# MPF-Optimization-Laboratory/ConicIP.jl

Measured on AMD Instinct MI355X. Metric: KKT solves/sec + wall-clock to converge, dense QP n=8192, 1 GPU, higher is better.
Workload: dtype f64

## Files before the change

conicip.jl_amd/cipkkt/_lib.py:

```python
import ctypes as C
import os

_HERE = os.path.dirname(os.path.abspath(__file__))
LIB_PATH = os.environ.get("CIPKKT_LIB", os.path.join(_HERE, "libcipkkt.so"))

CONE_R, CONE_Q, CONE_S = 0, 1, 2
ROUTE_SCHUR, ROUTE_FULL3X3 = 0, 1
OP_F, OP_FT, OP_FINV, OP_FINVT = 0, 1, 2, 3
MAT_Q, MAT_A, MAT_G = 0, 1, 2
FLAG_DEVICE_PTRS = 1
FLAG_CSR_HOST = 2
FLAG_Q_CSR = 4
E_SINGULAR = -5
E_UNSUPPORTED = -6
E_RETRY = -7

c_double_p = C.POINTER(C.c_double)
c_int_p = C.POINTER(C.c_int)


class CipProblem(C.Structure):
    _fields_ = [("n", C.c_int), ("m", C.c_int), ("p", C.c_int), ("ncones", C.c_int),
                ("cone_type", c_int_p), ("cone_dim", c_int_p),
                ("Q", C.c_void_p), ("ldq", C.c_int),
# ... 24 lines not shown
                             C.c_void_p, C.c_int, C.POINTER(C.c_void_p)]),
    "cip_create_ex": (C.c_int, [C.POINTER(CipProblem), C.POINTER(C.c_void_p)]),
    "cip_update_problem": (C.c_int, [C.c_void_p, C.POINTER(CipProblem)]),
    "cip_destroy": (C.c_int, [C.c_void_p]),
    "cip_last_error": (C.c_char_p, []),
    "cip_set_stream": (C.c_int, [C.c_void_p, C.c_void_p]),
    "cip_scaling_packed_len": (C.c_size_t, [C.c_void_p]),
    "cip_set_scaling_packed": (C.c_int, [C.c_void_p, C.c_void_p]),
    "cip_set_scaling_identity": (C.c_int, [C.c_void_p]),
    "cip_set_scaling_from_iterate_dev": (C.c_int, [C.c_void_p, C.c_void_p, C.c_void_p, C.c_void_p]),
    "cip_get_scaling_packed": (C.c_int, [C.c_void_p, C.c_void_p]),
    "cip_factor": (C.c_int, [C.c_void_p]),
    "cip_check_factor": (C.c_int, [C.c_void_p]),
    "cip_set_regularization": (C.c_int, [C.c_void_p, C.c_double, C.c_int]),
    "cip_get_regularization": (C.c_int, [C.c_void_p, c_double_p, c_int_p]),
    "cip_solve3x3": (C.c_int, [C.c_void_p] + [C.c_void_p] * 6),
    "cip_solve3x3_dev": (C.c_int, [C.c_void_p] + [C.c_void_p] * 6),
    "cip_solve2x2": (C.c_int, [C.c_void_p] + [C.c_void_p] * 4),
    "cip_solve2x2_dev": (C.c_int, [C.c_void_p] + [C.c_void_p] * 4),
    "cip_solve3x3_many": (C.c_int, [C.c_void_p, C.c_int] + [C.c_void_p] * 6),
    "cip_solve3x3_many_dev": (C.c_int, [C.c_void_p, C.c_int] + [C.c_void_p] * 6),
    "cip_solve2x2_many": (C.c_int, [C.c_void_p, C.c_int] + [C.c_void_p] * 4),
    "cip_solve2x2_many_dev": (C.c_int, [C.c_void_p, C.c_int] + [C.c_void_p] * 4),
    "cip_solve4x4_dev": (C.c_int, [C.c_void_p, C.c_void_p, C.c_void_p, C.c_void_p]),
    "cip_apply_F_dev": (C.c_int, [C.c_void_p, C.c_int, C.c_void_p, C.c_void_p]),
    "cip_cone_prod_dev": (C.c_int, [C.c_void_p, C.c_void_p, C.c_void_p, C.c_void_p]),
    "cip_cone_div_dev": (C.c_int, [C.c_void_p, C.c_void_p, C.c_void_p, C.c_void_p]),
    "cip_maxstep_dev": (C.c_int, [C.c_void_p, C.c_void_p, C.c_void_p, C.c_double, c_double_p]),
    "cip_maxstep_pair_dev": (C.c_int, [C.c_void_p, C.c_void_p, C.c_void_p, C.c_void_p, C.c_void_p, C.c_double, c_double_p]),
    "cip_cone_identity_dev": (C.c_int, [C.c_void_p, C.c_void_p]),
    "cip_gemv_dev": (C.c_int, [C.c_void_p, C.c_int, C.c_int, C.c_double, C.c_void_p, C.c_double, C.c_void_p]),
    "cip_dots_dev": (C.c_int, [C.c_void_p, C.c_int, C.POINTER(C.c_void_p), C.POINTER(C.c_void_p), c_int_p,
                               c_double_p]),
    "cip_axpby_dev": (C.c_int, [C.c_void_p, C.c_int, C.c_double, C.c_void_p, C.c_double, C.c_void_p]),
    "cip_conicip": (C.c_int, [C.c_void_p, C.c_void_p, C.c_void_p, C.c_void_p, C.POINTER(CipOptions), C.c_void_p,
                              C.c_void_p, C.c_void_p, C.POINTER(CipResult), C.c_void_p, C.c_int]),
    "cip_batch_create": (C.c_int, [C.c_int, C.POINTER(CipProblem), C.POINTER(C.c_void_p)]),
    "cip_batch_destroy": (C.c_int, [C.c_void_p]),
    "cip_batch_size": (C.c_int, [C.c_void_p]),
    "cip_batch_handle": (C.c_void_p, [C.c_void_p, C.c_int]),
    "cip_batch_conicip": (C.c_int, [C.c_void_p] + [C.POINTER(C.c_void_p)] * 3 + [C.POINTER(CipOptions)] +
                          [C.POINTER(C.c_void_p)] * 3 + [C.POINTER(CipResult), C.c_int]),
    "cip_conicip_problems": (C.c_int, [C.c_int, C.POINTER(CipProblem)] + [C.POINTER(C.c_void_p)] * 3 +
                             [C.POINTER(CipOptions)] + [C.POINTER(C.c_void_p)] * 3 + [C.POINTER(CipResult), C.c_int]),
    "cip_conicip_lockstep": (C.c_int, [C.c_int, C.POINTER(CipProblem)] + [C.POINTER(C.c_void_p)] * 3 +
                             [C.POINTER(CipOptions)] + [C.POINTER(C.c_void_p)] * 3 + [C.POINTER(CipResult)]),
    "cip_conicip_mixed": (C.c_int, [C.c_int, C.POINTER(CipProblem)] + [C.POINTER(C.c_void_p)] * 3 +
                          [C.POINTER(CipOptions)] + [C.POINTER(C.c_void_p)] * 3 + [C.POINTER(CipResult), C.c_int]),
    "cip_release_cached_memory": (C.c_int, []),
    "cip_lockstep_stats": (C.c_int, [c_int_p]),
    "cip_set_lockstep_regularize": (C.c_int, [C.c_int]),
    "cip_set_lockstep_ragged": (C.c_int, [C.c_int]),
    "cip_lockstep_regularized": (C.c_int, [c_int_p]),
    "cip_conicip_many": (C.c_int, [C.POINTER(C.c_void_p), C.c_int] + [C.POINTER(C.c_void_p)] * 3 +
                         [C.POINTER(CipOptions)] + [C.POINTER(C.c_void_p)] * 3 + [C.POINTER(CipResult), C.c_int]),
    "cip_ldlt_workspace_bytes": (C.c_int, [C.c_int, C.POINTER(C.c_size_t)]),
    "cip_ldlt_factor_dev": (C.c_int, [C.c_void_p, C.c_void_p, C.c_int, C.c_int, C.c_void_p, c_int_p]),
    "cip_ldlt_solve_dev": (C.c_int, [C.c_void_p, C.c_void_p, C.c_int, C.c_int, C.c_void_p, C.c_void_p]),
    "cip_ldlt_solve_many_scratch_bytes": (C.c_int, [C.c_int, C.c_int, C.POINTER(C.c_size_t)]),
    "cip_ldlt_solve_many_dev": (C.c_int, [C.c_void_p, C.c_void_p, C.c_int, C.c_int, C.c_void_p, C.c_void_p, C.c_void_p, C.c_int,
                                          C.c_int]),
    "cip_gemm_nt_dev": (C.c_int, [C.c_void_p, C.c_int, C.c_int, C.c_int, C.c_double, C.c_void_p, C.c_int,
                                  C.c_void_p, C.c_int, C.c_void_p, C.c_int, C.c_int]),
    "cip_qrcp_workspace_bytes": (C.c_int, [C.c_int, C.c_int, C.POINTER(C.c_size_t)]),
    "cip_imcols_workspace_bytes": (C.c_int, [C.c_int, C.c_int, C.POINTER(C.c_size_t)]),
    "cip_qrcp_dev": (C.c_int, [C.c_void_p, C.c_void_p, C.c_int, C.c_int, C.c_int, C.c_double, C.c_void_p, C.c_void_p, c_int_p,
                               c_double_p, c_int_p]),
    "cip_imcols_dev": (C.c_int, [C.c_void_p, C.c_void_p, C.c_int, C.c_int, C.c_int, C.c_void_p, C.c_double, C.c_void_p, c_int_p,
                                 c_int_p, c_int_p, c_double_p]),
    "cip_kkt_order": (C.c_int, [C.c_void_p, c_int_p, c_int_p]),
    "cip_get_kkt_matrix": (C.c_int, [C.c_void_p, C.c_void_p]),
    "cip_assemble_only": (C.c_int, [C.c_void_p]),
    "cip_stats": (C.c_int, [C.c_void_p, c_double_p]),
    "cip_set_timing": (C.c_int, [C.c_void_p, C.c_int]),
    "cip_set_ldlt_outer_block": (C.c_int, [C.c_int]),
    "cip_set_solve_block_max": (C.c_int, [C.c_int]),
    "cip_set_solve_fused": (C.c_int, [C.c_int]),
    "cip_lockstep_solve_block_for": (C.c_int, [C.c_int]),
    "cip_profile_trailing_thread": (C.c_int, [C.c_int]),
    "cip_profile_thread_get": (C.c_int, [c_double_p]),
    "cip_profile_kernel_thread": (C.c_int, [C.c_int, C.c_int]),
    "cip_profile_kernel_thread_get": (C.c_int, [C.c_int, c_double_p]),
    "cip_set_lazy_copy": (C.c_int, [C.c_int]),
    "cip_set_sdp_lanczos": (C.c_int, [C.c_int]),
    "cip_set_lockstep_split": (C.c_int, [C.c_int]),
    "cip_debug_chain_giveup": (C.c_int, [C.c_int]),
    "cip_get_chain_fallbacks": (C.c_int, [C.c_void_p]),
    "cip_sdp_lanczos_fallbacks": (C.c_int, [C.c_void_p, c_int_p]),
    "cip_set_ldlt_fused_chain": (C.c_int, [C.c_int]),
    "cip_set_ldlt_side_prep": (C.c_int, [C.c_int]),
    "cip_profile_trailing": (C.c_int, [C.c_void_p, C.c_int]),
    "cip_profile_get": (C.c_int, [C.c_void_p, c_double_p]),
}

_lib = None


class CipError(RuntimeError):
    def __init__(self, code, msg):
        super().__init__("libcipkkt error %d: %s" % (code, msg))
        self.code = code


def load():
    global _lib
    if _lib is not None:
        return _lib
    if not os.path.exists(LIB_PATH):
        raise ImportError("libcipkkt.so not built (%s): run `python -c 'import __graft_entry__ as g; g.build()'` "
                          "-- there is no CPU fallback" % LIB_PATH)
    lib = C.CDLL(LIB_PATH)
    for name, (res, args) in SIGNATURES.items():
        fn = getattr(lib, name)
        fn.restype = res
        fn.argtypes = args
    _lib = lib
    return lib


def check(rc):
    if rc != 0:
        msg = load().cip_last_error()
        raise CipError(rc, msg.decode() if msg else "?")
```

conicip.jl_amd/csrc/api.hip:

```cpp
#include "cip_handle.h"
#include <thread>
#include <stdlib.h>
#include "../../include/cipkkt.h"
#include <stdarg.h>
#include <stdio.h>
#include <string.h>
#include <math.h>
#include <new>

static thread_local char g_err[512] = "";
void cip_set_error(const char *fmt, ...) {
    va_list ap;
    va_start(ap, fmt);
    vsnprintf(g_err, sizeof(g_err), fmt, ap);
    va_end(ap);
}
extern "C" const char *cip_last_error(void) { return g_err; }

int cip_env_int(const char *name, int dflt) { const char *e = getenv(name); return e ? atoi(e) : dflt; }
long cip_env_long(const char *name, long dflt) { const char *e = getenv(name); return e ? atol(e) : dflt; }
double cip_env_double(const char *name, double dflt) { const char *e = getenv(name); return e ? atof(e) : dflt; }
bool cip_env_set(const char *name) { return getenv(name) != nullptr; }

#include <dlfcn.h>
// ... 556 lines not shown
    return 0;
}

extern "C" int cip_set_stream(cip_handle *h, void *stream) {
    if (!h) return CIP_E_INVALID;
    CIP_HIP_CHECK(hipStreamSynchronize(h->stream));
    h->stream = (hipStream_t)stream;
    h->graph_state = 0;
    return 0;
}

extern "C" size_t cip_scaling_packed_len(const cip_handle *h) { return h ? h->cs.scal_len : 0; }

extern "C" int cip_set_scaling_packed(cip_handle *h, const double *packedF) {
    if (!h || !packedF) { cip_set_error("NULL argument"); return CIP_E_INVALID; }
    CIP_HIP_CHECK(hipMemcpyAsync(h->cs.d_scal, packedF, sizeof(double) * h->cs.scal_len, hipMemcpyHostToDevice, h->stream));
    CIP_HIP_CHECK(hipStreamSynchronize(h->stream));
    h->assembled = h->factored = false;
    return cip_sdp_scaling_changed(h->stream, h->cs);
}
extern "C" int cip_get_scaling_packed(cip_handle *h, double *packedF) {
    if (!h || !packedF) { cip_set_error("NULL argument"); return CIP_E_INVALID; }
    CIP_HIP_CHECK(hipMemcpyAsync(packedF, h->cs.d_scal, sizeof(double) * h->cs.scal_len, hipMemcpyDeviceToHost, h->stream));
    CIP_HIP_CHECK(hipStreamSynchronize(h->stream));
    return 0;
}
extern "C" int cip_set_scaling_identity(cip_handle *h) {
    if (!h) return CIP_E_INVALID;
    h->assembled = h->factored = false;
    CIP_TRY(cip_cones_identity_scaling(h->stream, h->cs));
    return cip_sdp_scaling_changed(h->stream, h->cs);
}
extern "C" int cip_set_scaling_from_iterate_dev(cip_handle *h, const double *v, const double *s, double *lambda_out) {
    if (!h || (h->m > 0 && (!v || !s))) { cip_set_error("NULL argument"); return CIP_E_INVALID; }
    h->assembled = h->factored = false;
    CipRange rg("cip:scaling");
    return cip_cones_nt_scaling(h->stream, h->cs, v, s, lambda_out);
}

extern "C" int cip_assemble_only(cip_handle *h) {
    if (!h) return CIP_E_INVALID;
    return cip_assemble(h);
}

bool cip_graph_wanted(cip_handle *h) {
    if (h->graph_state == 0) {
        const int npmax = cip_env_int("CIP_GRAPH_NMAX", 4096);
        h->graph_state = (h->Npad <= npmax && cip_env_int("CIP_GRAPH", 0) == 1 && !h->timing && !h->ws.prof) ? 1 : -1;
    }
    return h->graph_state == 1;
}
thread_local CipGraphBuilder *cip_tl_builder = nullptr;

__global__ void k_publish_info(const int *info, int *host, int seq) {
    if (threadIdx.x == 0) {
        host[0] = info[0]; host[1] = info[1]; host[2] = info[2]; host[3] = info[3];
        __hip_atomic_store(host + 4, seq, __ATOMIC_RELEASE, __HIP_MEMORY_SCOPE_SYSTEM);
    }
}
static int info_landed(cip_handle *h, bool wait, bool *landed) {
    volatile int *seqp = h->info_host + 4;
    *landed = __atomic_load_n(seqp, __ATOMIC_ACQUIRE) == h->info_seq;
    if (*landed || !wait) return 0;
    for (long spin = 0;; ++spin) {
        if (__atomic_load_n(seqp, __ATOMIC_ACQUIRE) == h->info_seq) { *landed = true; return 0; }
        if ((spin & 0xfff) == 0xfff) {
            std::this_thread::yield();
            const hipError_t q = hipStreamQuery(h->stream);
            if (q == hipSuccess) {
                *landed = __atomic_load_n(seqp, __ATOMIC_ACQUIRE) == h->info_seq;
                if (*landed) return 0;
                cip_set_error("LDL': the pivot flags of factorisation %d never arrived", h->info_seq);
                return CIP_E_HIP;
            }
            if (q != hipErrorNotReady) { cip_set_error("hipStreamQuery failed: %s", hipGetErrorString(q)); return CIP_E_HIP; }
        }
    }
}
static int factor_enqueue(cip_handle *h) {
    { CipRange rg("cip:assemble"); CIP_TRY(cip_assemble(h, true)); }
    if (h->timing) CIP_HIP_CHECK(hipEventRecord(h->ev1, h->stream));
    {
        CipRange rg("cip:ldlt");
        if (h->gx_factor && (h->gx_factor_lazyC != h->ws.lazyC || h->gx_factor_unfused != h->ws.unfused)) {
            (void)hipGraphExecDestroy(h->gx_factor); h->gx_factor = nullptr;
        }
        h->gx_factor_lazyC = h->ws.lazyC;
        h->gx_factor_unfused = h->ws.unfused;
        bool replayed = false;
        CIP_TRY(graph_run(h, &h->gx_factor, [&]() {
            const int r = cip_ldlt_factor(h->stream, h->K, h->Npad, h->ldk, h->ws);
            if (cip_tl_builder) h->gx_factor_fused = cip_ldlt_last_factor_fused();
            return r;
        }, &replayed));
        if (replayed) CIP_TRY(cip_ldlt_debug_giveup(h->stream, h->K, h->Npad, h->ldk, h->ws, h->gx_factor_fused));
    }
    h->n_factor += 1;
    if (!h->info_host) {
        CIP_HIP_CHECK(hipHostMalloc((void **)&h->info_host, 8 * sizeof(int), hipHostMallocMapped | hipHostMallocCoherent));
        memset(h->info_host, 0, 8 * sizeof(int));
    }
    {
        int *info_dev = nullptr;
        CIP_HIP_CHECK(hipHostGetDevicePointer((void **)&info_dev, h->info_host, 0));
        h->info_seq = (h->info_seq == 0x7fffffff) ? 1 : h->info_seq + 1;
        hipLaunchKernelGGL(k_publish_info, dim3(1), dim3(64), 0, h->stream, (const int *)h->ws.info, info_dev, h->info_seq);
        CIP_HIP_CHECK(hipGetLastError());
    }
    h->info_pending = true;
    h->spec_solves = 0;
    h->factored = true;
    return 0;
}

static int refactor_and_wait(cip_handle *h) {
    for (;;) {
        CIP_TRY(factor_enqueue(h));
        { bool landed = false; CIP_TRY(info_landed(h, true, &landed)); }
        h->info_pending = false;
        if (h->info_host[3] == 0 || h->info_host[1] != 0 || h->ws.unfused) return 0;
        h->ws.unfused = 1;
        h->n_chain_fallbacks += 1;
    }
}
static int chain_gave_up(cip_handle *h) {
    if (h->info_host[3] == 0 && h->info_host[1] == 0) return 0;
    cip_set_error("LDL': in-launch wait of the panel chain gave up (%d)", h->info_host[3]);
    h->factored = false;
    return CIP_E_HIP;
}
static int solves_to_repeat(int spec, const char *why) {
    if (spec <= 0) return 0;
    cip_set_error("LDL': %d solve(s) were enqueued on a factorisation %s -- repeat them", spec, why);
    return CIP_E_RETRY;
}
int cip_factor_resolve(cip_handle *h, bool wait) {
    if (!h->info_pending) return 0;
    bool landed = false;
    CIP_TRY(info_landed(h, wait, &landed));
    if (!landed) return 0;
    h->info_pending = false;
    const int spec = h->spec_solves;
    bool redone = false;
    if (h->info_host[3] != 0 && h->info_host[1] == 0 && !h->ws.unfused) {
        h->ws.unfused = 1;
        h->n_chain_fallbacks += 1;
        CIP_TRY(refactor_and_wait(h));
        redone = true;
    }
    CIP_TRY(chain_gave_up(h));
    int info = h->info_host[0];
    if (info == 0 || (h->reg_rel > 0.0 && h->info_host[2] == 0)) {
        h->pivots_verified = true;
        return redone ? solves_to_repeat(spec, "whose panel chain gave up an in-launch wait; the handle has switched to the three-launch chain") : 0;
    }
    if (h->reg_rel > 0.0) {
        info = h->info_host[2];
    } else if (h->auto_reg) {
        h->reg_rel = cip_env_double("CIP_AUTO_REG", CIP_AUTO_REG);
        h->n_regularized += 1;
        CIP_TRY(refactor_and_wait(h));
        CIP_TRY(chain_gave_up(h));
        if (h->info_host[2] == 0) {
            h->pivots_verified = true;
            return solves_to_repeat(spec, "that met a bad pivot; the handle has switched to the regularised factorisation");
        }
        info = h->info_host[2];
    }
    h->factored = false;
    h->pivots_verified = false;
// ... 132 lines not shown
    return cip_ldlt_solve((hipStream_t)stream, K, N, ld, ws, rhs);
}
extern "C" int cip_ldlt_solve_many_scratch_bytes(int N, int nrhs, size_t *bytes) {
    if (N <= 0 || N % CIP_NB || nrhs < 0 || !bytes) { cip_set_error("N must be a positive multiple of 128, nrhs >= 0"); return CIP_E_INVALID; }
    *bytes = sizeof(double) * (size_t)cip_ldlt_solve_many_scratch_block(N) * (size_t)(nrhs < 64 ? nrhs : 64);
    return 0;
}
extern "C" int cip_ldlt_solve_many_dev(void *stream, const double *K, int N, int ld, const void *workspace, void *scratch, double *B,
                                       int ldb, int nrhs) {
    if (!ldlt_dims_ok(K, N, ld, workspace) || nrhs < 0 || ldb < N) {
        cip_set_error("cip_ldlt_solve_many_dev: bad argument (K, workspace non-NULL; N > 0 and ld >= N multiples of 128; nrhs >= 0; "
                      "ldb >= N)");
        return CIP_E_INVALID;
    }
    if (nrhs == 0) return 0;
    if (!B || !scratch) { cip_set_error("cip_ldlt_solve_many_dev: B and scratch must be non-NULL"); return CIP_E_INVALID; }
    LdltWorkspace ws{};
    cip_ldlt_ws_carve((void *)workspace, N, &ws, cip_ldlt_fused_for(N));
    return cip_ldlt_solve_many((hipStream_t)stream, K, N, ld, ws, (double *)scratch, B, ldb, nrhs, true);
}
extern "C" int cip_gemm_nt_dev(void *stream, int M, int N, int K, double alpha, const double *A, int lda, const double *B,
                               int ldb, double *C, int ldc, int lower_only) {
    if (!A || !B || !C || M <= 0 || N <= 0 || K <= 0 || M % CIP_NB || N % CIP_NB || K % 16 || lda < M || ldb < N || ldc < M ||
        (lower_only && M != N)) {
        cip_set_error("cip_gemm_nt_dev: bad argument (A, B, C non-NULL; M, N > 0 multiples of 128, K > 0 a multiple of 16, "
                      "lda >= M, ldb >= N, ldc >= M; M == N with lower_only)");
        return CIP_E_INVALID;
    }
    if (lower_only) return cip_gemm_lower((hipStream_t)stream, M, K, alpha, A, lda, B, ldb, C, ldc);
    return cip_gemm_rect((hipStream_t)stream, M, N, K, alpha, A, lda, B, ldb, C, ldc);
}

extern "C" int cip_kkt_order(const cip_handle *h, int *N, int *N_padded) {
    if (!h) return CIP_E_INVALID;
    if (N) *N = h->N;
    if (N_padded) *N_padded = h->Npad;
    return 0;
}
extern "C" int cip_get_kkt_matrix(cip_handle *h, double *K_host) {
    if (!h || !K_host) return CIP_E_INVALID;
    CIP_TRY(cip_ldlt_side_join(h->stream, h->ws, -1));
    CIP_HIP_CHECK(hipStreamSynchronize(h->stream));
    CIP_HIP_CHECK(hipMemcpy(K_host, h->K, sizeof(double) * (size_t)h->ldk * h->Npad, hipMemcpyDeviceToHost));
    return 0;
}
extern "C" int cip_stats(cip_handle *h, double *out8) {
    if (!h || !out8) return CIP_E_INVALID;
    out8[0] = h->n_factor; out8[1] = h->n_solve; out8[2] = h->ms_assemble; out8[3] = h->ms_ldlt; out8[4] = h->flops_ldlt;
    out8[5] = cip_ldlt_outer_block_for(h->Npad); out8[6] = h->N; out8[7] = h->Npad;
    return 0;
}
extern "C" int cip_set_timing(cip_handle *h, int enabled) {
    if (!h) return CIP_E_INVALID;
    h->timing = enabled != 0;
    return 0;
}
extern "C" int cip_profile_trailing(cip_handle *h, int enabled) {
    if (!h) return CIP_E_INVALID;
    if (enabled && !h->ws.prof) h->ws.prof = cip_ldlt_profile_create();
    if (enabled) cip_ldlt_profile_stride(h->ws.prof, enabled);
    if (!enabled && h->ws.prof) { cip_ldlt_profile_destroy(h->ws.prof); h->ws.prof = nullptr; }
    return 0;
}
extern "C" int cip_profile_get(cip_handle *h, double *out3) {
    if (!h || !out3 || !h->ws.prof) { cip_set_error("profiling not enabled"); return CIP_E_INVALID; }
    return cip_ldlt_profile_collect(h->ws.prof, &out3[0], &out3[1], &out3[2]);
}
extern "C" int cip_profile_kernel_thread(int slot, int enabled) {
    if (cip_prof_slot_enable(slot, enabled)) { cip_set_error("cip_profile_kernel_thread: no slot %d", slot); return CIP_E_INVALID; }
    return 0;
}
extern "C" int cip_profile_kernel_thread_get(int slot, double *out3) {
    if (!out3) return CIP_E_INVALID;
    if (cip_prof_slot_collect(slot, &out3[0], &out3[1], &out3[2])) { cip_set_error("slot %d: profiling not enabled", slot); return CIP_E_INVALID; }
    return 0;
}
extern "C" int cip_profile_trailing_thread(int enabled) { return cip_ldlt_profile_thread(enabled); }
extern "C" int cip_profile_thread_get(double *out3) {
    if (!out3) return CIP_E_INVALID;
    if (cip_ldlt_profile_thread_collect(&out3[0], &out3[1], &out3[2])) { cip_set_error("thread profiling not enabled"); return CIP_E_INVALID; }
    return 0;
}
extern "C" int cip_set_lazy_copy(int on) { return cip_lazy_copy_set(on); }
extern "C" int cip_set_sdp_lanczos(int on) { return cip_sdp_large_lanczos(on); }
extern "C" int cip_debug_chain_giveup(int n) { return cip_debug_chain_giveup_set(n); }
extern "C" int cip_get_chain_fallbacks(cip_handle *h) { return h ? h->n_chain_fallbacks : -1; }
extern "C" int cip_sdp_lanczos_fallbacks(cip_handle *h, int *count) {
    if (!h || !count) { cip_set_error("bad argument"); return CIP_E_INVALID; }
    int out2[2] = {0, 0};
    const int rc = cip_sdp_large_cert_stats(h->stream, h->cs.lg, out2);
    *count = out2[0];
    return rc;
}
extern "C" int cip_set_ldlt_fused_chain(int on) { return cip_ldlt_set_fused_chain(on); }
extern "C" int cip_set_ldlt_side_prep(int on) { return cip_ldlt_set_side_prep(on); }
extern "C" int cip_set_solve_block_max(int b) { return cip_solve_block_max_set(b); }
extern "C" int cip_set_solve_fused(int mode) { return cip_solve_fused_set(mode); }
extern "C" int cip_set_ldlt_outer_block(int nbo) { cip_ldlt_set_outer_block(nbo); return cip_ldlt_outer_block(); }
```

conicip.jl_amd/csrc/assemble.hip:

```cpp
#include "cip_handle.h"
#include <atomic>
#include "../../include/cipkkt.h"

__global__ __launch_bounds__(256) void k_fill_rest(double *K, long ldk, int n, int p, int Npad, const double *G, long ldg, CipBatch cb) {
    CIP_BATCH_GUARD(cb);
    CIP_BO2(cb, K, G);
    const int j = blockIdx.x * 256 + threadIdx.x;
    if (j >= Npad) return;
    for (int i = n + blockIdx.y; i < Npad; i += gridDim.y) {
        if (j > i) continue;
        double v;
        if (i < n + p) v = (j < n) ? G[(i - n) + (long)j * ldg] : 0.0;
        else v = (i == j) ? 1.0 : 0.0;
        K[i + (long)j * ldk] = v;
    }
}

__global__ __launch_bounds__(256) void k_copy_block(double *K, long ldk, int r0, int c0, const double *M, long ldm,
                                                     int rows, int cols, double sign, CipBatch cb) {
    CIP_BATCH_GUARD(cb);
    CIP_BO2(cb, K, M);
    const int i = blockIdx.x * 256 + threadIdx.x;
    if (i >= rows) return;
    for (int j = blockIdx.y; j < cols; j += gridDim.y)
// ... 38 lines not shown
        cip_launch_b(k_copy_block_lower, dim3((n + 255) / 256, n < 32768 ? n : 32768), dim3(256), 0, s, K, ldk, r0, M, ldm, n, sign);
    }
}

__global__ __launch_bounds__(256) void k_qcsr_fill_cols(double *K, long ldk, int n, const int *rp, const int *ci, const double *v, int vec,
                                                         CipBatch cb) {
    CIP_BATCH_GUARD(cb);
    CIP_BO4(cb, K, rp, ci, v);
    const int j = blockIdx.x, tid = threadIdx.x;
    if (j >= n) return;
    double *col = K + (long)j * ldk;
    const int z0 = j & ~127;
    if (vec) {
        const int nv = (n - z0) >> 1;
        for (int t = tid; t < nv; t += 256) *(v2d *)(col + z0 + 2 * t) = (v2d){0.0, 0.0};
        if (((n - z0) & 1) && tid == 0) col[n - 1] = 0.0;
    } else {
        for (int i = z0 + tid; i < n; i += 256) col[i] = 0.0;
    }
    __syncthreads();
    const int q1 = rp[j + 1];
    for (int q = rp[j] + tid; q < q1; q += 256) {
        const int i = ci[q];
        if ((i >> 7) >= (j >> 7)) col[i] = v[q];
    }
}
template <bool ADD>
__global__ __launch_bounds__(256) void k_qcsr_scatter(double *K, long ldk, int r0, int n, const int *rp, const int *ci, const double *v,
                                                       int shift, CipBatch cb) {
    CIP_BATCH_GUARD(cb);
    CIP_BO4(cb, K, rp, ci, v);
    const int lane = threadIdx.x & 63;
    const int j = blockIdx.x * 4 + (threadIdx.x >> 6);
    if (j >= n) return;
    double *col = K + r0 + (long)(r0 + j) * ldk;
    const int q1 = rp[j + 1];
    for (int q = rp[j] + lane; q < q1; q += 64) {
        const int i = ci[q];
        if (((r0 + i) >> shift) < ((r0 + j) >> shift)) continue;
        if (ADD) col[i] += v[q];
        else col[i] = v[q];
    }
}

__device__ __forceinline__ double schur_row_weight(const ConeDesc &cd, const double *scal, int r) {
    if (cd.type == CIP_CONE_R) { const double d = scal[cd.soff + (r - cd.off)]; return 1.0 / (d * d); }
    if (cd.type == CIP_CONE_S) return 0.0;
    const double beta = scal[cd.soff];
    return ((r == cd.off) ? -1.0 : 1.0) / (beta * beta);
}
__global__ __launch_bounds__(256) void k_schur_rows(int n, const int *trp, const int *tci, const double *tv, const int *rp,
                                                     const int *ci, const double *av, const int *row_cone,
                                                     const ConeDesc *cones, const double *scal, double *K, long ldk, int base, CipBatch cb) {
    CIP_BATCH_GUARD(cb);
    CIP_BO8(cb, trp, tci, tv, rp, ci, av, scal, K);
    const int lane = threadIdx.x & 63;
    const int i = blockIdx.x * 4 + (threadIdx.x >> 6);
    if (i >= n) return;
    double *Ki = K + (base + i) + (long)base * ldk;
    for (int q = trp[i]; q < trp[i + 1]; ++q) {
        const int r = tci[q];
        const ConeDesc rc = cones[row_cone[r]];
        if (rc.type == CIP_CONE_S) continue;
        const double wa = schur_row_weight(rc, scal, r) * tv[q];
        const int b1 = rp[r + 1];
        bool wrote = false;
        for (int b = rp[r] + lane; b < b1; b += 64) {
            const int j = ci[b];
            if (j <= i) {
                double *kp = Ki + (long)j * ldk;
                double x = __hip_atomic_load(kp, __ATOMIC_RELAXED, __HIP_MEMORY_SCOPE_AGENT);
                x += wa * av[b];
                __hip_atomic_store(kp, x, __ATOMIC_RELAXED, __HIP_MEMORY_SCOPE_AGENT);
                wrote = true;
            }
        }
        (void)wrote;
        asm volatile("s_waitcnt vmcnt(0)" ::: "memory");
    }
}
__global__ __launch_bounds__(256) void k_schur_diag_lazy(int n, int nb0, const int *trp, const int *tci, const double *tv, const int *rp,
                                                          const int *ci, const double *av, const int *row_cone, const ConeDesc *cones,
                                                          const double *scal, const double *Q, long ldq, double *K, long ldk, double *kdiag,
                                                          CipBatch cb) {
    CIP_BATCH_GUARD(cb);
    CIP_BO8(cb, trp, tci, tv, rp, ci, av, scal, Q);
    CIP_BO2(cb, K, kdiag);
    const int i = blockIdx.x * 256 + threadIdx.x;
    if (i >= n) return;
    double d = i < nb0 ? K[i + (long)i * ldk] : Q[i + (long)i * ldq];
    for (int q = trp[i]; q < trp[i + 1]; ++q) {
        const int r = tci[q];
        const double wa = schur_row_weight(cones[row_cone[r]], scal, r) * tv[q];
        for (int b = rp[r]; b < rp[r + 1]; ++b)
            if (ci[b] == i) d += wa * av[b];
    }
    if (i < nb0) K[i + (long)i * ldk] = d;
    else kdiag[i] = d;
}
__global__ __launch_bounds__(256) void k_schur_qcols(int n, const int *trp, const int *tci, const double *tv,
                                                      const int *row_cone, const ConeDesc *cones, const double *scal,
                                                      double *Gm, long ldgm, CipBatch cb) {
    CIP_BATCH_GUARD(cb);
    CIP_BO5(cb, trp, tci, tv, scal, Gm);
    const int i = blockIdx.x * 256 + threadIdx.x;
    if (i >= n) return;
    int cur = -1;
    double acc = 0.0;
    for (int q = trp[i]; q < trp[i + 1]; ++q) {
        const int r = tci[q];
        const ConeDesc cd = cones[row_cone[r]];
        if (cd.type != CIP_CONE_Q) continue;
        if (cd.qidx != cur) {
            if (cur >= 0) Gm[i + (long)cur * ldgm] = acc;
            cur = cd.qidx; acc = 0.0;
        }
        const double beta = scal[cd.soff];
        const double *w = scal + cd.soff + 1;
        const int e = r - cd.off;
        const double jw = (e == 0) ? (w[0] * w[0] / beta - 1.0) : -(w[0] * w[e] / beta);
        acc += (jw * 1.4142135623730951 / beta) * tv[q];
    }
    if (cur >= 0) Gm[i + (long)cur * ldgm] = acc;
}

__global__ __launch_bounds__(256) void k_scatter_AtS(int n, const int *trp, const int *tci, const double *tv, const int *row_cone,
                                                      const ConeDesc *cones, double *AtS, long ld, CipBatch cb) {
    CIP_BATCH_GUARD(cb);
    CIP_BO4(cb, trp, tci, tv, AtS);
    const int i = blockIdx.x * 256 + threadIdx.x;
    if (i >= n) return;
    for (int q = trp[i]; q < trp[i + 1]; ++q) {
        const int r = tci[q];
        const ConeDesc cd = cones[row_cone[r]];
        if (cd.type == CIP_CONE_S) AtS[i + (long)(cd.aoff + (r - cd.off)) * ld] = tv[q];
    }
}
int cip_scatter_AtS(cip_handle *h) {
    if (!h->AtS || h->n == 0) return 0;
    CIP_HIP_CHECK(hipMemsetAsync(h->AtS, 0, sizeof(double) * (size_t)h->npad * h->mSpad, h->stream));
    hipLaunchKernelGGL(k_scatter_AtS, dim3((h->n + 255) / 256), dim3(256), 0, h->stream, h->n, h->T_rp, h->T_ci, h->T_v, h->row_cone,
                       h->cs.d_cones, h->AtS, (long)h->npad, CipBatch{0, 1ull});
    CIP_HIP_CHECK(hipGetLastError());
    return 0;
}

__global__ __launch_bounds__(256) void k_fill_ftf(const ConeDesc *cones, const WorkItem *items, const double *scal,
                                                   double *K, long ldk, CipBatch cb) {
    CIP_BATCH_GUARD(cb);
    CIP_BO2(cb, scal, K);
    const WorkItem it = items[blockIdx.x];
    const ConeDesc cd = cones[it.cone];
    const int tid = threadIdx.x;
    if (cd.type == CIP_CONE_R) {
        for (int e = it.start + tid; e < it.start + it.len; e += 256) {
            const double d = scal[cd.soff + e];
            const long g = cd.off + e;
            K[g + g * ldk] = -d * d;
        }
    } else if (cd.type == CIP_CONE_Q) {
        if (!it.width) return;
        const int ncone = it.len;
        for (int q = 0; q < ncone; ++q) {
            const ConeDesc qc = cones[it.cone + q];
            const int k = qc.dim;
            const double beta = scal[qc.soff];
            const double *w = scal + qc.soff + 1;
            const double b2 = beta * beta, w0 = w[0];
            for (long e = tid; e < (long)k * k; e += 256) {
                const int i = (int)(e % k), j = (int)(e / k);
                if (i < j) continue;
                const double wi = (i == 0) ? (w0 * w0 / beta - 1.0) : (w0 * w[i] / beta);
                const double wj = (j == 0) ? (w0 * w0 / beta - 1.0) : (w0 * w[j] / beta);
                double v = 2.0 * wi * wj;
                if (i == j) v -= (i == 0) ? 1.0 : -1.0;
                K[(qc.off + i) + (long)(qc.off + j) * ldk] = -b2 * v;
            }
        }
    }
}
__global__ __launch_bounds__(256) void k_fill_ftf_qbig(const ConeDesc *cones, const WorkItem *items, const int *bigq, const double *scal,
                                                        double *K, long ldk, CipBatch cb) {
    CIP_BATCH_GUARD(cb);
    CIP_BO2(cb, scal, K);
    const WorkItem it = items[bigq[blockIdx.x]];
    const ConeDesc qc = cones[it.cone];
    const int k = qc.dim;
    const double beta = scal[qc.soff];
    const double *w = scal + qc.soff + 1;
    const double b2 = beta * beta, w0 = w[0];
    for (int j = blockIdx.y; j < k; j += gridDim.y) {
        const double wj = (j == 0) ? (w0 * w0 / beta - 1.0) : (w0 * w[j] / beta);
        for (int i = j + threadIdx.x; i < k; i += 256) {
            const double wi = (i == 0) ? (w0 * w0 / beta - 1.0) : (w0 * w[i] / beta);
            double v = 2.0 * wi * wj;
            if (i == j) v -= (i == 0) ? 1.0 : -1.0;
            K[(qc.off + i) + (long)(qc.off + j) * ldk] = -b2 * v;
        }
    }
}
__global__ __launch_bounds__(256) void k_scatter_negA(int nrowsT, const int *trp, const int *tci, const double *tv,
                                                       double *K, long ldk, int r0, CipBatch cb) {
    CIP_BATCH_GUARD(cb);
    CIP_BO4(cb, trp, tci, tv, K);
    const int i = blockIdx.x * 256 + threadIdx.x;
    if (i >= nrowsT) return;
    for (int q = trp[i]; q < trp[i + 1]; ++q) K[(r0 + i) + (long)tci[q] * ldk] = -tv[q];
}
__global__ __launch_bounds__(256) void k_pad_identity(double *K, long ldk, int N, int Npad, CipBatch cb) {
    CIP_BATCH_GUARD(cb);
    CIP_BO1(cb, K);
    const int i = N + blockIdx.x * 256 + threadIdx.x;
    if (i < Npad) K[i + (long)i * ldk] = 1.0;
}

int cip_ldlt_outer_block_for(int Npad);
static std::atomic<int> g_lazy_copy{-1};
int cip_lazy_copy_set(int on) {
    int prev = g_lazy_copy.load(std::memory_order_relaxed);
    if (prev < 0) {
        const int env = cip_env_int("CIP_LAZY_COPY", 1) != 0;
        int expect = -1;
        g_lazy_copy.compare_exchange_strong(expect, env);
        prev = g_lazy_copy.load(std::memory_order_relaxed);
    }
    if (on == 0 || on == 1) g_lazy_copy.store(on);
    return prev;
}
static int assemble_schur(cip_handle *h, bool lazy_ok) {
    hipStream_t s = h->stream;
    int rc;
    const int n = h->n, p = h->p;
    h->ws.lazyC = nullptr;
    if (!h->A_sparse) {
        if ((rc = cip_cones_scale_At(s, h->cs, n, h->At, h->npad, h->Wt, h->npad))) return rc;
        if ((rc = cip_prof_slot_begin(CIP_PROF_SYRK, s, (double)h->m * (double)n * (double)n * (cip_in_batch() ? (double)__builtin_popcountll(cip_tl_bz.mask) : 1.0)))) return rc;
        if ((rc = cip_syrk_schur(s, h->npad, h->mpad, n, 1.0, h->Wt, h->npad, h->Q, n, h->K, h->ldk, h->syrk_ws, h->syrk_n, h->syrk_len))) return rc;
        if ((rc = cip_prof_slot_end(CIP_PROF_SYRK, s))) return rc;
        if (h->Q_sparse && cip_grp_Q_nonempty(h))
            cip_launch_b(k_qcsr_scatter<true>, dim3((n + 3) / 4), dim3(256), 0, s, h->K, h->ldk, 0, n, h->Q_rp, h->Q_ci, h->Q_v, 6);
    } else {
        const int lazy_now = g_lazy_copy.load(std::memory_order_relaxed);
        const int lazy_on = lazy_now < 0 ? cip_lazy_copy_set(-1) : lazy_now;
        bool all_r = cip_all_r(h);
        const int nb0 = cip_ldlt_outer_block_for(h->Npad);
        if (!h->Q_sparse && lazy_on && lazy_ok && all_r && cip_grp_A_one_per_row(h) && p == 0 && h->Npad == n && n > nb0 && h->reg_rel <= 0.0 && h->kdiag &&
            copy_lower_vectorisable(h->K, h->ldk, 0, h->Q, (long)n, n)) {
            launch_copy_block_lower(s, h->K, h->ldk, 0, h->Q, (long)n, n, 1.0, nb0);
            cip_launch_b(k_schur_diag_lazy, dim3((n + 255) / 256), dim3(256), 0, s, n, nb0, h->T_rp, h->T_ci, h->T_v, h->A_rp, h->A_ci, h->A_v,
                         h->row_cone, h->cs.d_cones, h->cs.d_scal, h->Q, (long)n, h->K, h->ldk, h->kdiag);
            CIP_HIP_CHECK(hipGetLastError());
            h->ws.lazyC = h->Q; h->ws.lazy_ld = n; h->ws.lazy_diag = h->kdiag;
            return 0;
        }
        if (h->Q_sparse) {
            const int vec = !(h->ldk & 1) && !(((uintptr_t)h->K) & 15);
            cip_launch_b(k_qcsr_fill_cols, dim3(n), dim3(256), 0, s, h->K, h->ldk, n, h->Q_rp, h->Q_ci, h->Q_v, vec);
        } else if (n > 0) {
            launch_copy_block_lower(s, h->K, h->ldk, 0, h->Q, (long)n, n, 1.0);
        }
        if (h->m > 0) {
            cip_launch_b(k_schur_rows, dim3((n + 3) / 4), dim3(256), 0, s, n, h->T_rp, h->T_ci, h->T_v, h->A_rp, h->A_ci,
                               h->A_v, h->row_cone, h->cs.d_cones, h->cs.d_scal, h->K, h->ldk, 0);
            if (h->nq > 0) {
                if ((rc = cip_zero(s, (long)h->npad * h->nqpad, h->Gm))) return rc;
                cip_launch_b(k_schur_qcols, dim3((n + 255) / 256), dim3(256), 0, s, n, h->T_rp, h->T_ci, h->T_v,
                                   h->row_cone, h->cs.d_cones, h->cs.d_scal, h->Gm, (long)h->npad);
            }
        }
    }
    if (h->Npad > n) {
        cip_launch_b(k_fill_rest, dim3((h->Npad + 255) / 256, (h->Npad - n) < 32768 ? (h->Npad - n) : 32768), dim3(256), 0, s, h->K, h->ldk, n, p,
                           h->Npad, h->G, (long)p);
    }
    if (h->A_sparse && h->AtS) {
        if ((rc = cip_sdp_scale_At(s, h->cs, n, h->AtS, (long)h->npad, h->WtS, (long)h->npad))) return rc;
        if ((rc = cip_gemm_lower(s, h->npad, h->mSpad, 1.0, h->WtS, h->npad, h->WtS, h->npad, h->K, h->ldk))) return rc;
    }
    if (h->A_sparse && h->nq > 0 && h->m > 0) {
        if ((rc = cip_gemm_lower(s, h->npad, h->nqpad, 1.0, h->Gm, h->npad, h->Gm, h->npad, h->K, h->ldk))) return rc;
    }
    CIP_HIP_CHECK(hipGetLastError());
    return 0;
}

int cip_sdp_fill_ftf(hipStream_t s, const ConeSet &cs, double *K, long ldk);

static int assemble_full(cip_handle *h) {
    hipStream_t s = h->stream;
    const int n = h->n, m = h->m, p = h->p;
    { int rcz = cip_zero(s, (long)h->ldk * h->Npad, h->K); if (rcz) return rcz; }
    if (h->cs.nitems > 0)
        cip_launch_b(k_fill_ftf, dim3(h->cs.nitems), dim3(256), 0, s, h->cs.d_cones, h->cs.d_items, h->cs.d_scal,
                           h->K, h->ldk);
    if (h->cs.nbigq > 0)
        cip_launch_b(k_fill_ftf_qbig, dim3(h->cs.nbigq, 128), dim3(256), 0, s, h->cs.d_cones, h->cs.d_items, (const int *)h->cs.d_bigq, h->cs.d_scal, h->K, h->ldk);
    if (h->cs.has_S) { int rc = cip_sdp_fill_ftf(s, h->cs, h->K, h->ldk); if (rc) return rc; }
    if (m > 0 && n > 0) {
        if (!h->A_sparse)
            cip_launch_b(k_copy_block, dim3((n + 255) / 256, m < 32768 ? m : 32768), dim3(256), 0, s, h->K, h->ldk, m, 0, h->At,
                               (long)h->npad, n, m, -1.0);
        else
            cip_launch_b(k_scatter_negA, dim3((n + 255) / 256), dim3(256), 0, s, n, h->T_rp, h->T_ci, h->T_v,
                               h->K, h->ldk, m);
    }
    if (h->Q_sparse) {
        if (cip_grp_Q_nonempty(h))
            cip_launch_b(k_qcsr_scatter<false>, dim3((n + 3) / 4), dim3(256), 0, s, h->K, h->ldk, m, n, h->Q_rp, h->Q_ci, h->Q_v, 7);
    } else if (n > 0)
        launch_copy_block_lower(s, h->K, h->ldk, m, h->Q, (long)n, n, 1.0);
    if (p > 0)
        cip_launch_b(k_copy_block, dim3((p + 255) / 256, n < 32768 ? n : 32768), dim3(256), 0, s, h->K, h->ldk, m + n, m, h->G,
                           (long)p, p, n, 1.0);
    if (h->Npad > h->N)
        cip_launch_b(k_pad_identity, dim3((h->Npad - h->N + 255) / 256), dim3(256), 0, s, h->K, h->ldk, h->N, h->Npad);
    CIP_HIP_CHECK(hipGetLastError());
    return 0;
}

#define REG_TILE 128
#define REG_COLS 16
__global__ __launch_bounds__(256) void k_regmax_tiles(const double *K, long ldk, int N, double *mx_d, CipBatch cb) {
    CIP_BATCH_GUARD(cb);
    CIP_BO2(cb, K, mx_d);
    unsigned long long *mx = (unsigned long long *)mx_d;
    __shared__ double sh[2][REG_COLS][REG_TILE + 1];
    __shared__ double shrow[REG_TILE];
    const int t = blockIdx.x;
    int ti = (int)((sqrt(8.0 * (double)t + 1.0) - 1.0) * 0.5);
    while ((long)(ti + 1) * (ti + 2) / 2 <= t) ++ti;
    while ((long)ti * (ti + 1) / 2 > t) --ti;
    const int tj = t - (int)((long)ti * (ti + 1) / 2);
    const int r = threadIdx.x & (REG_TILE - 1), hh = threadIdx.x >> 7;
    const int cc = threadIdx.x >> 4, sg = threadIdx.x & 15;
    const int gi = ti * REG_TILE + r;
    double rmx = 0.0;
    for (int q = 0; q < REG_TILE / REG_COLS; ++q) {
        double (*buf)[REG_TILE + 1] = sh[q & 1];
        double a[8];
#pragma unroll
        for (int k = 0; k < 8; ++k) {
            const int gj = tj * REG_TILE + q * REG_COLS + hh * 8 + k;
            a[k] = (gi < N && gj <= gi) ? fmax(0.0, fabs(K[gi + (long)gj * ldk])) : 0.0;
        }
#pragma unroll
        for (int k = 0; k < 8; ++k) {
            const int gj = tj * REG_TILE + q * REG_COLS + hh * 8 + k;
            rmx = fmax(rmx, a[k]);
            buf[hh * 8 + k][r] = gj < gi ? a[k] : 0.0;
        }
        __syncthreads();
        double v = 0.0;
#pragma unroll
        for (int e = 0; e < 8; ++e) v = fmax(v, buf[cc][sg + 16 * e]);
        for (int o = 8; o > 0; o >>= 1) v = fmax(v, __shfl_xor(v, o));
        const int gc = tj * REG_TILE + q * REG_COLS + cc;
        if (sg == 0 && gc < N && v > 0.0) atomicMax(&mx[gc], (unsigned long long)__double_as_longlong(v));
    }
    if (hh == 1) shrow[r] = rmx;
    __syncthreads();
    if (hh == 0) {
        rmx = fmax(rmx, shrow[r]);
        if (gi < N && rmx > 0.0) atomicMax(&mx[gi], (unsigned long long)__double_as_longlong(rmx));
    }
}
__global__ __launch_bounds__(256) void k_regularize_diag(double *K, long ldk, int N, int p0, int p1, double rel, const double *mx, CipBatch cb) {
    CIP_BATCH_GUARD(cb);
    CIP_BO2(cb, K, mx);
    const int i = blockIdx.x * 256 + threadIdx.x;
    if (i >= N) return;
    const double delta = rel * mx[i];
    K[i + (long)i * ldk] += (i >= p0 && i < p1) ? delta : -delta;
}
int cip_regularize(cip_handle *h, double rel) {
    if (h->N <= 0) return 0;
    const int T = (h->N + REG_TILE - 1) / REG_TILE;
    { const int rc = cip_zero(h->stream, h->N, h->rhs); if (rc) return rc; }
    cip_launch_b(k_regmax_tiles, dim3((unsigned)((long)T * (T + 1) / 2)), dim3(256), 0, h->stream, (const double *)h->K, h->ldk, h->N, h->rhs);
    cip_launch_b(k_regularize_diag, dim3((h->N + 255) / 256), dim3(256), 0, h->stream, h->K, h->ldk, h->N, h->ws.signs.p0, h->ws.signs.p1, rel,
                 (const double *)h->rhs);
    CIP_HIP_CHECK(hipGetLastError());
    return 0;
}

int cip_assemble(cip_handle *h, bool lazy_ok) {
    h->ws.lazyC = nullptr;
    { const int rj = cip_ldlt_side_join(h->stream, h->ws, -1); if (rj) return rj; }
    int rc = (h->route == CIP_ROUTE_SCHUR) ? assemble_schur(h, lazy_ok) : assemble_full(h);
    if (rc == 0 && h->reg_rel > 0.0) rc = cip_regularize(h, h->reg_rel);
    if (rc == 0) { h->assembled = true; h->factored = false; }
    return rc;
}
```

conicip.jl_amd/csrc/cip_gemm_tile.h:

```cpp
#pragma once
#include "cip_internal.h"

enum { EPI_ACCUM = 0, EPI_SYRKQ = 2, EPI_STORE = 3, EPI_LAZYC = 4, EPI_SYRK0 = 5 };

struct GemmArgs {
    const double *A; long lda;
    const double *B; long ldb;
    double *C; long ldc;
    int M, N, K;
    double alpha;
    int tiles;
    const double *Qin; long ldq; int nvalid;
    const double *Cdiag;
    int bz;
    long sAy, sAz, sBy, sBz, sCy, sCz;
    double *Ct; long ldct, sCty, sCtz;
    double *ksplit_ws; int ksplit_n, ksplit_len;
};

__device__ __forceinline__ unsigned gemm_batch_prologue(GemmArgs &g, const CipBatch &cb, bool &live) {
    const unsigned gz = g.bz > 0 ? (unsigned)g.bz : 1u;
    const unsigned pz = blockIdx.z / gz;
    live = ((cb.mask >> pz) & 1ull) != 0;
    const long off = (long)pz * cb.stride;
// ... 76 lines not shown
            acc[0][1] = __builtin_amdgcn_mfma_f64_16x16x4f64(fj.y, fi.x, acc[0][1], 0, 0, 0);
            acc[1][1] = __builtin_amdgcn_mfma_f64_16x16x4f64(fj.y, fi.y, acc[1][1], 0, 0, 0);
        }
        if (!GLDS && kt + 1 < KT) lstore(buf ^ 1);
        __syncthreads();
    }
#pragma unroll
    for (int tj = 0; tj < 2; ++tj)
#pragma unroll
        for (int q = 0; q < 4; ++q) {
            const long col = j0 + wn * 32 + 2 * (l4 + 4 * q) + tj;
            const long row = i0 + wm * 32 + 2 * l15;
            double *cp = g.C + row + col * g.ldc;
            const v2d val = (v2d){acc[0][tj][q], acc[1][tj][q]};
            if (EPI == EPI_ACCUM) {
                v2d c = *(v2d *)cp;
                c += g.alpha * val;
                *(v2d *)cp = c;
            } else if (EPI == EPI_LAZYC) {
                v2d c = *(const v2d *)(g.Qin + row + col * g.ldq);
                if (row == col) c.x = g.Cdiag[row];
                if (row + 1 == col) c.y = g.Cdiag[col];
                c += g.alpha * val;
                *(v2d *)cp = c;
            } else if (EPI == EPI_STORE) {
                const v2d c = g.alpha * val;
                *(v2d *)cp = c;
                if (g.Ct) { g.Ct[col + row * g.ldct] = c.x; g.Ct[col + (row + 1) * g.ldct] = c.y; }
            } else if (EPI == EPI_SYRK0) {
                if (col < g.nvalid) {
                    if (row + 1 < g.nvalid) *(v2d *)cp = g.alpha * val;
                    else if (row < g.nvalid) *cp = g.alpha * val.x;
                }
            } else if (col < g.nvalid) {
                if (row + 1 < g.nvalid) {
                    const double *qp = g.Qin + row + col * g.ldq;
                    *(v2d *)cp = (v2d){qp[0], qp[1]} + g.alpha * val;
                } else if (row < g.nvalid) {
                    *cp = g.Qin[row + col * g.ldq] + g.alpha * val.x;
                }
            }
        }
}

template <class FetchB, class Store>
__device__ __forceinline__ void gemm_tile_16_splitk(const double *a, long lda, int K, FetchB fetch_b, Store store) {
    __shared__ double red[3][4][64];
    const int lane = threadIdx.x & 63, wave = threadIdx.x >> 6;
    const int kq = K >> 2;
    v4d acc0 = (v4d){0.0, 0.0, 0.0, 0.0}, acc1 = acc0;
    for (int k = 0; k < kq; k += 32) {
        double av[8], bv[8];
#pragma unroll
        for (int u = 0; u < 8; ++u) {
            av[u] = a[(long)(k + 4 * u) * lda];
            bv[u] = fetch_b(k + 4 * u);
        }
#pragma unroll
        for (int u = 0; u < 8; u += 2) {
            acc0 = __builtin_amdgcn_mfma_f64_16x16x4f64(bv[u], av[u], acc0, 0, 0, 0);
            acc1 = __builtin_amdgcn_mfma_f64_16x16x4f64(bv[u + 1], av[u + 1], acc1, 0, 0, 0);
        }
    }
    acc0 += acc1;
    if (wave > 0) {
#pragma unroll
        for (int q = 0; q < 4; ++q) red[wave - 1][q][lane] = acc0[q];
    }
    __syncthreads();
    if (wave == 0) {
#pragma unroll
        for (int q = 0; q < 4; ++q) store(q, ((acc0[q] + red[0][q][lane]) + red[1][q][lane]) + red[2][q][lane]);
    }
}

struct GrpBar { unsigned *ctr; unsigned gen; };
__device__ __forceinline__ void grp_barrier(GrpBar &b) {
    b.gen += 4u;
    asm volatile("s_waitcnt lgkmcnt(0)" ::: "memory");
    if ((threadIdx.x & 63) == 0) __hip_atomic_fetch_add(b.ctr, 1u, __ATOMIC_RELAXED, __HIP_MEMORY_SCOPE_WORKGROUP);
    while (__hip_atomic_load(b.ctr, __ATOMIC_RELAXED, __HIP_MEMORY_SCOPE_WORKGROUP) < b.gen) __builtin_amdgcn_s_sleep(1);
    asm volatile("" ::: "memory");
}
template <bool QUEUE>
__device__ __forceinline__ unsigned gemm_tile_64_k128_grp(const GemmArgs &g, double *lds, long i0, long j0, int gt, GrpBar &bar,
                                                          unsigned *tileq, unsigned *slot) {
    const int lane = gt & 63;
    const int wave = gt >> 6;
    const int wm = wave & 1, wn = wave >> 1;
    const int l15 = lane & 15, l4 = lane >> 4;
    const int k_ld = gt >> 5, rp = gt & 31;
    const double *Ap = g.A + i0 + 2 * rp;
    const double *Bp = g.B + j0 + 2 * rp;
    const long rowo = i0 + wm * 32 + 2 * l15;
    v2d cpre[2][4];
    v2d ra[16], rb[16];
#pragma unroll
    for (int q = 0; q < 16; ++q) {
        const long k = q * 8 + k_ld;
        ra[q] = *(const v2d *)(Ap + k * g.lda);
        rb[q] = *(const v2d *)(Bp + k * g.ldb);
    }
    unsigned nxt = 0u;
    if (QUEUE && gt == 0) nxt = __hip_atomic_fetch_add(tileq, 1u, __ATOMIC_RELAXED, __HIP_MEMORY_SCOPE_AGENT);
    v4d acc[2][2];
#pragma unroll
    for (int a = 0; a < 2; ++a)
#pragma unroll
        for (int b = 0; b < 2; ++b) acc[a][b] = (v4d){0.0, 0.0, 0.0, 0.0};
#pragma unroll
    for (int qt = 0; qt < 4; ++qt) {
        double *la = lds + (qt & 1) * (64 * SB), *lb = la + 32 * SB;
        if (qt == 0) {
#pragma unroll
            for (int q = 0; q < 4; ++q) {
                *(v2d *)(la + (q * 8 + k_ld) * SB + 2 * rp) = ra[q];
                *(v2d *)(lb + (q * 8 + k_ld) * SB + 2 * rp) = rb[q];
            }
        }
        if (QUEUE && qt == 3 && gt == 0) *(volatile unsigned *)slot = nxt;
        grp_barrier(bar);
        if (qt == 1) {
#pragma unroll
            for (int tj = 0; tj < 2; ++tj)
#pragma unroll
                for (int q = 0; q < 4; ++q) cpre[tj][q] = *(const v2d *)(g.C + rowo + (j0 + wn * 32 + 2 * (l4 + 4 * q) + tj) * g.ldc);
        }
        if (qt < 3) {
            double *na = lds + ((qt + 1) & 1) * (64 * SB), *nb = na + 32 * SB;
#pragma unroll
            for (int q = 0; q < 4; ++q) {
                *(v2d *)(na + (q * 8 + k_ld) * SB + 2 * rp) = ra[4 * (qt + 1) + q];
                *(v2d *)(nb + (q * 8 + k_ld) * SB + 2 * rp) = rb[4 * (qt + 1) + q];
            }
        }
        const double *pa = la + wm * 32 + 2 * l15, *pb = lb + wn * 32 + 2 * l15;
#pragma unroll
        for (int ks = 0; ks < 8; ++ks) {
            const int kk = ks * 4 + l4;
            const v2d fi = *(const v2d *)(pa + kk * SB);
            const v2d fj = *(const v2d *)(pb + kk * SB);
            acc[0][0] = __builtin_amdgcn_mfma_f64_16x16x4f64(fj.x, fi.x, acc[0][0], 0, 0, 0);
            acc[1][0] = __builtin_amdgcn_mfma_f64_16x16x4f64(fj.x, fi.y, acc[1][0], 0, 0, 0);
            acc[0][1] = __builtin_amdgcn_mfma_f64_16x16x4f64(fj.y, fi.x, acc[0][1], 0, 0, 0);
            acc[1][1] = __builtin_amdgcn_mfma_f64_16x16x4f64(fj.y, fi.y, acc[1][1], 0, 0, 0);
        }
    }
#pragma unroll
    for (int tj = 0; tj < 2; ++tj)
#pragma unroll
        for (int q = 0; q < 4; ++q) {
            double *cp = g.C + rowo + (j0 + wn * 32 + 2 * (l4 + 4 * q) + tj) * g.ldc;
            v2d c = cpre[tj][q];
            c += g.alpha * (v2d){acc[0][tj][q], acc[1][tj][q]};
            *(v2d *)cp = c;
        }
    if (QUEUE) nxt = *(volatile unsigned *)slot;
    return nxt;
}
```

conicip.jl_amd/csrc/cip_handle.h:

```cpp
#pragma once
#include "cip_internal.h"
#include <vector>

struct cip_handle {
    int n = 0, m = 0, p = 0, ncones = 0, route = 0;
    int N = 0, Npad = 0;
    int npad = 0, mpad = 0;
    int nq = 0, nqpad = 0;
    hipStream_t stream = nullptr;
    int device = 0;
    std::vector<void *> owned;
    bool in_slab = false;
    int ldlt_fused = 0;

    double *Q = nullptr;
    bool Q_sparse = false;
    int Q_nnz = 0, Q_wave = 0;
    int *Q_rp = nullptr, *Q_ci = nullptr; double *Q_v = nullptr;
    double *symv_ws = nullptr;
    bool A_sparse = false;
    bool A_one_per_row = false;
    double *kdiag = nullptr;
    int s4_fused = -1;
    double *A = nullptr;
    double *At = nullptr;
    int A_nnz = 0;
    int *A_rp = nullptr, *A_ci = nullptr; double *A_v = nullptr;
    int *T_rp = nullptr, *T_ci = nullptr; double *T_v = nullptr;
    int *row_cone = nullptr;
    double *AtS = nullptr, *WtS = nullptr; int mS = 0, mSpad = 0;
    double *G = nullptr;
    double *Gt = nullptr;

    std::vector<int> st_rp, st_ci, st_trp, st_tci, st_rowcone, st_sidx, st_small, st_bigq, st_ritems, st_packq;
    std::vector<double> st_av, st_tv;
    std::vector<int> st_qrp, st_qci; std::vector<double> st_qv;
    bool staging_live = false;

    std::vector<ConeDesc> h_cones;
    std::vector<WorkItem> h_items;
    ConeSet cs = {};

    double *K = nullptr; long ldk = 0;
    double *Wt = nullptr;
    double *syrk_ws = nullptr; int syrk_n = 1, syrk_len = 0;
    double *Gm = nullptr;
    void *ws_base = nullptr; LdltWorkspace ws = {};
    struct LdltSide *ldlt_side = nullptr;
    bool assembled = false, factored = false;
    double reg_rel = 0.0;
    bool auto_reg = true;
    int n_regularized = 0;
    int n_chain_fallbacks = 0;
    int x_zeroed = 0;
    int *info_host = nullptr;
    int info_seq = 0;
    bool info_pending = false;
    int spec_solves = 0;
    bool pivots_verified = false;

    double *rhs = nullptr;
    double *mt1 = nullptr, *mt2 = nullptr, *mt3 = nullptr;
    double *nt1 = nullptr;
    double *pt1 = nullptr;
    double *dot_scratch = nullptr;
    double *stage = nullptr;
    double *ref = nullptr;
    double *c2x2 = nullptr;
    double *many = nullptr, *many_stage = nullptr;
    double *drv = nullptr;

    hipGraphExec_t gx_factor = nullptr, gx_solve = nullptr;
    const double *gx_factor_lazyC = nullptr;
    int gx_factor_unfused = 0;
    bool gx_factor_fused = false;
    int graph_state = 0;

    double n_factor = 0, n_solve = 0, ms_assemble = 0, ms_ldlt = 0, flops_ldlt = 0;
    bool timing = false;
    hipEvent_t ev0 = nullptr, ev1 = nullptr, ev2 = nullptr;
};

int cip_lazy_copy_set(int on);
int cip_scatter_AtS(cip_handle *h);
int cip_assemble(cip_handle *h, bool lazy_ok = false);
#define CIP_AUTO_REG 1e-13

int cip_regularize(cip_handle *h, double rel);
int cip_mul_Q(cip_handle *h, double alpha, const double *x, double beta, double *y, bool symv = true);
int cip_mul_A(cip_handle *h, double alpha, const double *x, double beta, double *y);
int cip_mul_At(cip_handle *h, double alpha, const double *x, double beta, double *y);
inline bool cip_all_r(const cip_handle *h) { return h->m > 0 && h->nq == 0 && !h->cs.has_S; }
int cip_handle_alloc(cip_handle *h, void **out, size_t bytes);
#define CIP_EXTRA_DRIVER 1u
#define CIP_EXTRA_REFINE 2u
int cip_plan(const struct cip_problem *pr, hipStream_t stream, cip_handle **out);
struct CipCsrCap { size_t A_nnz, Q_nnz; };
size_t cip_handle_layout(CipLayout L, cip_handle *h, unsigned extras, const CipCsrCap *cap = nullptr);
int cip_create_in_slab(cip_handle *h, const struct cip_problem *pr, char *slab, size_t cap, unsigned extras, const CipCsrCap *csr_cap = nullptr);
inline bool cip_grp_A_one_per_row(const cip_handle *h) {
    return cip_in_batch() ? (cip_tl_bz.mask & ~cip_tl_bz.a_one_per_row) == 0 : h->A_one_per_row;
}
inline bool cip_grp_Q_nonempty(const cip_handle *h) {
    return cip_in_batch() ? (cip_tl_bz.mask & cip_tl_bz.q_nonempty) != 0 : h->Q_nnz > 0;
}
size_t cip_driver_bytes(const cip_handle *h);
int cip_factor_resolve(cip_handle *h, bool wait);

void cip_range_push(const char *name);
void cip_range_pop(void);
struct CipRange { explicit CipRange(const char *n) { cip_range_push(n); } ~CipRange() { cip_range_pop(); } };

#define CIP_MANY_CHUNK 64
struct Vec3 { double *x, *y, *z; };
inline Vec3 cip_take3(CipLayout &L, const cip_handle *h, size_t k = 1, size_t g = 8) { return Vec3{L.take<double>(h->n * k, g), L.take<double>(h->p * k, g), L.take<double>(h->m * k, g)}; }
struct StageView { Vec3 in, out; };
inline size_t stage_layout(CipLayout L, const cip_handle *h, size_t cap, StageView *v) {
    v->in = cip_take3(L, h, cap, 16);
    v->out = cip_take3(L, h, cap, 16);
    return L.bytes();
}
struct RefView { Vec3 rhs, res, cor; };
inline size_t ref_layout(CipLayout L, const cip_handle *h, RefView *v) {
    for (Vec3 *b : {&v->rhs, &v->res, &v->cor}) { *b = cip_take3(L, h); L.take<double>(8, 8); }
    return L.bytes();
}
struct ManyView { double *R, *T, *U, *S; };
inline size_t many_layout(CipLayout L, const cip_handle *h, ManyView *v) {
    const size_t c = CIP_MANY_CHUNK;
    *v = ManyView{L.take<double>(c * h->Npad, 8), L.take<double>(c * h->m, 8), L.take<double>(c * h->m, 8), L.take<double>(c * h->ws.Bs, 8)};
    return L.bytes();
}

bool cip_graph_wanted(cip_handle *h);
template <class F>
static int graph_run(cip_handle *h, hipGraphExec_t *exec, F &&enqueue, bool *replayed = nullptr) {
    if (cip_in_batch() || !cip_graph_wanted(h) || h->timing || h->ws.prof) return enqueue();
    if (!*exec) {
        CipGraphBuilder b = {nullptr, nullptr, false, true};
        if (hipGraphCreate(&b.graph, 0) != hipSuccess) { (void)hipGetLastError(); h->graph_state = -1; return enqueue(); }
        cip_tl_builder = &b;
        const int rc = enqueue();
        cip_tl_builder = nullptr;
        hipError_t ei = hipErrorUnknown;
        if (rc == 0 && b.ok && b.have_last) ei = hipGraphInstantiate(exec, b.graph, nullptr, nullptr, 0);
        (void)hipGraphDestroy(b.graph);
        if (ei != hipSuccess) { (void)hipGetLastError(); *exec = nullptr; h->graph_state = -1; return enqueue(); }
    }
    CIP_HIP_CHECK(hipGraphLaunch(*exec, h->stream));
    if (replayed) *replayed = true;
    return 0;
}
```

conicip.jl_amd/csrc/cip_internal.h:

```cpp
#pragma once
#include <hip/hip_runtime.h>
#include <stddef.h>
#include <stdint.h>

typedef double v4d __attribute__((ext_vector_type(4)));
typedef double v2d __attribute__((ext_vector_type(2)));

#define CIP_NB 128
#define CIP_KT 16

void cip_set_error(const char *fmt, ...);
#define CIP_HIP_CHECK(expr)                                                       \
    do {                                                                          \
        hipError_t e__ = (expr);                                                  \
        if (e__ != hipSuccess) {                                                  \
            cip_set_error("%s failed: %s (%s:%d)", #expr, hipGetErrorString(e__), \
                          __FILE__, __LINE__);                                    \
            return -3;                                                            \
        }                                                                         \
    } while (0)
#define CIP_TRY(expr)                                                             \
    do {                                                                          \
        const int rc__ = (expr);                                                  \
        if (rc__) return rc__;                                                    \
// ... 46 lines not shown
#define CIP_BATCH_MAX 64
struct CipScal64 { double v[CIP_BATCH_MAX]; };
extern thread_local CipBatchCtx cip_tl_bz;
inline bool cip_in_batch() { return cip_tl_bz.B > 1; }
struct CipMaskScope {
    const unsigned long long saved = cip_tl_bz.mask;
    ~CipMaskScope() { cip_tl_bz.mask = saved; }
    void set(unsigned long long mask) { cip_tl_bz.mask = mask; }
};
template <typename T>
__device__ __forceinline__ T *cip_bo(T *p, const CipBatch &cb) { return p ? (T *)((char *)p + (long)blockIdx.z * cb.stride) : p; }
#define CIP_BATCH_GUARD(cb) do { if (!(((cb).mask >> blockIdx.z) & 1ull)) return; } while (0)
#define CIP_BO1(cb, a) a = cip_bo(a, cb)
#define CIP_BO2(cb, a, b) CIP_BO1(cb, a); CIP_BO1(cb, b)
#define CIP_BO3(cb, a, b, c) CIP_BO2(cb, a, b); CIP_BO1(cb, c)
#define CIP_BO4(cb, a, b, c, d) CIP_BO2(cb, a, b); CIP_BO2(cb, c, d)
#define CIP_BO5(cb, a, b, c, d, e) CIP_BO4(cb, a, b, c, d); CIP_BO1(cb, e)
#define CIP_BO6(cb, a, b, c, d, e, f) CIP_BO4(cb, a, b, c, d); CIP_BO2(cb, e, f)
#define CIP_BO7(cb, a, b, c, d, e, f, g) CIP_BO4(cb, a, b, c, d); CIP_BO3(cb, e, f, g)
#define CIP_BO8(cb, a, b, c, d, e, f, g, h) CIP_BO4(cb, a, b, c, d); CIP_BO4(cb, e, f, g, h)
template <typename... KArgs, typename... Args>
inline void cip_launch_b(void (*kernel)(KArgs...), dim3 grid, dim3 block, size_t shmem, hipStream_t s, Args... args) {
    const CipBatchCtx &c = cip_tl_bz;
    CipBatch cb{c.B > 1 ? c.stride : 0, c.B > 1 ? c.mask : 1ull};
    if (c.B > 1) grid.z *= (unsigned)c.B;
    cip_launch(kernel, grid, block, shmem, s, args..., cb);
}

int cip_gemm_lower(hipStream_t s, int M, int K, double alpha, const double *A, long lda, const double *B, long ldb, double *C, long ldc);
int cip_gemm_lower_lazyc(hipStream_t s, int M, int K, double alpha, const double *A, long lda, const double *B, long ldb, double *C, long ldc,
                         const double *Qin, long ldq, const double *Cdiag);
int cip_gemm_rect(hipStream_t s, int M, int N, int K, double alpha, const double *A, long lda, const double *B, long ldb, double *C, long ldc);
int cip_syrk_schur(hipStream_t s, int M, int K, int nvalid, double alpha, const double *W, long ldw, const double *Qin, long ldq, double *C, long ldc,
                   double *split_ws, int split_n, int split_len);
int cip_syrk_split(int M, int K, int *len);
struct GemmBatchIn { const double *p; long ld, sy, sz; };
struct GemmBatchOut { double *p; long ld, sy, sz; };
enum { GEMM_TILES_ALL = 0, GEMM_TILES_TOUCH_UPPER = 1, GEMM_TILES_TOUCH_LOWER = 2 };
int cip_gemm_batched_64(hipStream_t s, int M, int N, int K, double alpha, const GemmBatchIn &A, const GemmBatchIn &B, const GemmBatchOut &C,
                        const GemmBatchOut &Ct, int by, int bz, int tiles);
int cip_gemm_batched_16(hipStream_t s, int M, int N, int K, double alpha, const GemmBatchIn &A, const GemmBatchIn &B, const GemmBatchOut &C,
                        const GemmBatchOut &Ct, int by, int bz);

struct CipHostScratch { double *host; double *dev; };
int cip_host_scratch(CipHostScratch *out);
int cip_wait(hipStream_t s);

struct LdltProfile;
LdltProfile *cip_ldlt_profile_create(void);
void cip_ldlt_profile_destroy(LdltProfile *p);
void cip_ldlt_profile_stride(LdltProfile *p, int stride);
int cip_ldlt_profile_collect(LdltProfile *p, double *launches, double *ms, double *flops);
int cip_ldlt_profile_thread(int enabled);
int cip_ldlt_profile_thread_collect(double *launches, double *ms, double *flops);
#define CIP_PROF_SLOTS 3
#define CIP_PROF_SYRK 1
#define CIP_PROF_JACOBI 2
int cip_prof_slot_enable(int slot, int enabled);
int cip_prof_slot_collect(int slot, double *launches, double *ms, double *work);
int cip_prof_slot_begin(int slot, hipStream_t s, double work);
int cip_prof_slot_end(int slot, hipStream_t s);

struct PivotSigns { int p0, p1, N; };

struct LdltWorkspace {
    double *Wbuf;
    double *Linv;
    double *LinvT;
    double *Xm;
    int Bs;
    double *X, *XT;
    double *Tt;
    double *MT, *PT;
    int fused;
    double *zbuf;
    int *x_zeroed;
    double *dinv;
    double *dvec;
    double *tmp;
    int *info;
    PivotSigns signs;
    LdltProfile *prof;
    const double *lazyC; long lazy_ld; const double *lazy_diag;
    struct LdltSide **side;
    int no_prep;
    int unfused;
};
struct LdltSide;
void cip_ldlt_side_destroy(struct LdltSide *sd);
int cip_ldlt_side_join(hipStream_t s, const struct LdltWorkspace &ws, int J);
int cip_kernels_init(void);
int cip_ldlt_set_side_prep(int on);
int cip_debug_chain_giveup_set(int n);
int cip_ldlt_debug_giveup(hipStream_t s, double *K, int Npad, long ld, const struct LdltWorkspace &ws, bool fused);
bool cip_ldlt_last_factor_fused(void);
int cip_ldlt_set_fused_chain(int on);
int cip_solve_block(int Npad);
int cip_solve_block_max_set(int b);
int cip_solve_fused_set(int mode);
extern thread_local int cip_tl_solve_block_max;
int cip_ldlt_fused_for(int Npad);
size_t cip_ldlt_ws_bytes(int Npad, int fused);
void cip_ldlt_ws_carve(void *base, int Npad, LdltWorkspace *ws, int fused);
int cip_ldlt_factor(hipStream_t s, double *K, int Npad, long ld, const LdltWorkspace &ws);
int cip_ldlt_solve(hipStream_t s, const double *K, int Npad, long ld, const LdltWorkspace &ws, double *rhs);
int cip_ldlt_solve_many_scratch_block(int Npad);
int cip_ldlt_solve_many(hipStream_t s, const double *K, int Npad, long ld, const LdltWorkspace &ws, double *scratch, double *B, long ldb,
                        int k, bool one_is_single);
int cip_gemm_tn(hipStream_t s, int M, int k, int Kr, double alpha, const double *A, long lda, const double *B, long ldb,
                double beta, double *C, long ldc);
int cip_block_copy(hipStream_t s, int rows, int cols, double alpha, const double *src, long lds, const double *d, double *dst, long ldd);
int cip_ldlt_outer_block(void);
int cip_ldlt_outer_block_for(int Npad);
void cip_ldlt_set_outer_block(int nbo);

struct ConeDesc {
    int type;
    int off;
    int dim;
    int soff;
    int r;
    int qidx;
    int item;
    int aoff;
};
struct WorkItem {
    int cone;
    int start;
    int len;
    int slot;
    int width;
};
struct ConeSet {
    int ncones, nitems, nslots, m;
    ConeDesc *d_cones;
    WorkItem *d_items;
    double *d_scal;
    size_t scal_len;
    double *d_partial;
    double *d_scalar;
    int has_S;
    int nbigq;
    int nritems; int *d_ritems;
    int *d_bigq;
    int npackq; int *d_packq;
    int ns, rmax, kmax;
    int *d_sidx;
    int sdp_slots;
    double *d_sdpws;
    double *d_sdpvec;
    int *d_sdpflag;
    int ns_small;
    int rmax_small;
    int *d_sidx_small;
    int nlarge;
    int large_cone[1024];
    const ConeDesc *h_cones;
    struct LargeWs *lg;
};
#define CIP_MAX_LARGE_S 1024
#define CIP_LARGE_S_MIN 133
#define CIP_SDP_WS_MATS 6
struct LargeWs;
int cip_sdp_large_create(int rmax_large, int nlarge, int ncols, LargeWs **out);
void cip_sdp_large_invalidate(LargeWs *w);
void cip_sdp_large_destroy(LargeWs *w);
int cip_sdp_large_nt(hipStream_t s, LargeWs *w, const ConeDesc &cd, int li, const double *v, const double *sv, double *scal,
                     double *lambda, int *flag);
int cip_sdp_large_refresh(hipStream_t s, LargeWs *w, const ConeDesc &cd, int li, const double *scal);
int cip_sdp_large_apply(hipStream_t s, LargeWs *w, const ConeDesc &cd, int li, int mode, const double *x, double *out);
int cip_sdp_large_prod(hipStream_t s, LargeWs *w, const ConeDesc &cd, const double *x, const double *y, double *out);
int cip_sdp_large_div(hipStream_t s, LargeWs *w, const ConeDesc &cd, const double *x, const double *y, double *out, int *flag);
int cip_sdp_large_lanczos(int on);
int cip_sdp_large_cert_stats(hipStream_t s, struct LargeWs *w, int *out2);
int cip_sdp_large_maxstep(hipStream_t s, LargeWs *w, const ConeDesc &cd, const double *x, const double *d, double scale,
                          double *partial, int side = 0);
bool cip_sdp_large_pairable(const LargeWs *w);
int cip_sdp_large_fork(hipStream_t s, LargeWs *w, hipStream_t *s2);
int cip_sdp_large_join(hipStream_t s, LargeWs *w);
int cip_sdp_large_scale_At(hipStream_t s, LargeWs *w, const ConeDesc &cd, int li, int n, const double *At, long ldat, double *Wt,
                           long ldwt);
int cip_cones_nt_scaling(hipStream_t s, const ConeSet &cs, const double *v, const double *sv, double *lambda);
int cip_cones_identity_scaling(hipStream_t s, const ConeSet &cs);
int cip_sdp_scaling_changed(hipStream_t s, const ConeSet &cs);
// ... 83 lines not shown
```

conicip.jl_amd/csrc/diag.hip:

```cpp
#include "cip_internal.h"
#include "cip_gemm_tile.h"
#include <stdlib.h>

#define DP 144
#define PANEL_WAVES 8
#define XM_OFF (CIP_NB * DP)
#define DIAG2_LDS_BYTES ((CIP_NB * DP + 8 * 256) * 8)

__device__ __forceinline__ double fast_rcp(double d) {
    double r = __builtin_amdgcn_rcp(d);
    double e = fma(-d, r, 1.0);
    r = fma(r, e, r);
    e = fma(-d, r, 1.0);
    r = fma(r, e, r);
    return r;
}
#define MFMA(a, b, c) __builtin_amdgcn_mfma_f64_16x16x4f64((a), (b), (c), 0, 0, 0)

__host__ __device__ constexpr int diag_perm(int x) { return 4 * (x & 3) + (x >> 2); }
template <int N>
__device__ __forceinline__ double row_bcast_t(double x) {
    return __builtin_amdgcn_update_dpp(0.0, x, 0x150 + N, 0xf, 0xf, true);
}
template <int N>
// ... 192 lines not shown
#pragma unroll
                    for (int s = 0; s < 4; ++s) acc = MFMA(lp[4 * s], XT[kt][s], acc);
                }
            }
            const double *xp = xm + jt * (16 * XR) + l15 * XR + g;
            v4d r = (v4d){0.0, 0.0, 0.0, 0.0};
#pragma unroll
            for (int s = 0; s < 4; ++s) r = MFMA(xp[4 * s], acc[s], r);
#pragma unroll
            for (int s = 0; s < 4; ++s) XT[jt][s] = -r[s];
        }
    }
#pragma unroll
    for (int t = 0; t < 8; ++t)
        if (t < it) {
#pragma unroll
            for (int s = 0; s < 4; ++s) a[(t * 16 + g + 4 * s) + (it * 16 + l15) * P] = XT[t][s];
        }
}

template <int P = DP>
__device__ __forceinline__ void diag_load_block(double *a, const double *Kb, long ld, int tid) {
    v2d tmp[32];
#pragma unroll
    for (int q = 0; q < 32; ++q) {
        const int e = q * 256 + tid;
        tmp[q] = *(const v2d *)(Kb + 2 * (e & 63) + (long)(e >> 6) * ld);
    }
#pragma unroll
    for (int q = 0; q < 32; ++q) {
        const int e = q * 256 + tid;
        const int i = 2 * (e & 63), j = e >> 6;
        v2d v = tmp[q];
        if (i < j) v.x = 0.0;
        if (i + 1 < j) v.y = 0.0;
        *(v2d *)(a + i + j * P) = v;
    }
}

#define PANEL_STAGE_LAST 0x10000u
__device__ __forceinline__ void st_pub(double *p, double v) { __hip_atomic_store(p, v, __ATOMIC_RELAXED, __HIP_MEMORY_SCOPE_AGENT); }
__device__ __forceinline__ double ld_pub(const double *p) { return __hip_atomic_load(p, __ATOMIC_RELAXED, __HIP_MEMORY_SCOPE_AGENT); }
template <bool PUB = false>
__device__ __forceinline__ void diag_store_panel(const double *a, double *Kb, long ld, int c, int t, int nt) {
    typedef int v4i_t __attribute__((ext_vector_type(4)));
    const __amdgpu_buffer_rsrc_t rs = __builtin_amdgcn_make_buffer_rsrc((void *)Kb, 0, 0x7fffffff, 0x00020000);
    for (int e = t; e < 16 * 64; e += nt) {
        const int i = 2 * (e & 63), j = c + (e >> 6);
        if (i >= j) {
            const v2d v = *(const v2d *)(a + i + j * DP);
            if (PUB) __builtin_amdgcn_raw_buffer_store_b128(__builtin_bit_cast(v4i_t, v), rs, (int)((i + (long)j * ld) * 8), 0, 16);
            else *(v2d *)(Kb + i + (long)j * ld) = v;
        } else if (i + 1 == j) {
            if (PUB) st_pub(Kb + i + 1 + (long)j * ld, a[i + 1 + j * DP]);
            else Kb[i + 1 + (long)j * ld] = a[i + 1 + j * DP];
        }
    }
}
__device__ __forceinline__ void wave_store_T(double *scr, const double (&v)[4], double *dst, long ld, int lane) {
    const int l15 = lane & 15, g = lane >> 4;
#pragma unroll
    for (int q = 0; q < 4; ++q) scr[l15 * 17 + 4 * q + g] = v[q];
    __builtin_amdgcn_fence(__ATOMIC_RELEASE, "wavefront");
    __builtin_amdgcn_wave_barrier();
    __builtin_amdgcn_fence(__ATOMIC_ACQUIRE, "wavefront");
    const int r = lane >> 2, cq = lane & 3;
    const double *sp = scr + r * 17 + 4 * cq;
    const double t0 = sp[0], t1 = sp[1], t2 = sp[2], t3 = sp[3];
    double *d = dst + 4 * cq + (long)r * ld;
    *(v2d *)d = (v2d){t0, t1};
    *(v2d *)(d + 2) = (v2d){t2, t3};
    __builtin_amdgcn_fence(__ATOMIC_RELEASE, "wavefront");
    __builtin_amdgcn_wave_barrier();
}
__device__ __forceinline__ void diag_publish_micro(const double *a, const double *xm, double *xm_out, double *dvec, double *dinv,
                                                   int kb, int t, int nt) {
    for (int i = t; i < 256; i += nt) st_pub(xm_out + kb * 256 + i, xm[kb * 256 + i]);
    if (t < 16) {
        st_pub(dvec + kb * 16 + t, a[128 + (kb * 16 + t) * DP]);
        st_pub(dinv + kb * 16 + t, a[129 + (kb * 16 + t) * DP]);
    }
}

template <bool WAIT, bool PUB = false>
__device__ __forceinline__ void diag_body(double *sm, double *Kb, long ld, double *xm_out, double *dvec, double *dinv,
                                          int *info, int col0, PivotSigns sg, const unsigned *ready, unsigned *stage,
                                          unsigned ready_target) {
    double *a = sm;
    double *xm = sm + XM_OFF;
    const int tid = threadIdx.x, lane = tid & 63, wave = __builtin_amdgcn_readfirstlane(tid >> 6);
    const int l15 = lane & 15, g = lane >> 4;

    constexpr int NW = PANEL_WAVES, NH = NW - NW / 4;
    const bool idle = wave != 0 && (wave & 3) == 0;
    const int hid = wave - 1 - (wave >> 2);
    __builtin_amdgcn_s_setprio(3);
    if (WAIT) {
        if (tid == 0) {
            cip_bounded_wait<1>([&] { return __hip_atomic_load(ready, __ATOMIC_RELAXED, __HIP_MEMORY_SCOPE_AGENT) >= ready_target; },
                                info + 3, CIP_GIVEUP_XWG);
            __builtin_amdgcn_fence(__ATOMIC_ACQUIRE, "wavefront");
        }
        __syncthreads();
        typedef int v4i_t __attribute__((ext_vector_type(4)));
        const __amdgpu_buffer_rsrc_t rs = __builtin_amdgcn_make_buffer_rsrc((void *)Kb, 0, 0x7fffffff, 0x00020000);
        auto put = [&](int e, v4i_t t) {
            const int i = 2 * (e & 63), j = e >> 6;
            v2d v = __builtin_bit_cast(v2d, t);
            if (i < j) v.x = 0.0;
            if (i + 1 < j) v.y = 0.0;
            *(v2d *)(a + i + j * DP) = v;
        };
        auto get = [&](int e) -> v4i_t {
            const int i = 2 * (e & 63), j = e >> 6;
            if (i + 1 >= j) return __builtin_amdgcn_raw_buffer_load_b128(rs, (int)((i + (long)j * ld) * 8), 0, 16);
            return (v4i_t){0, 0, 0, 0};
        };
        {
            v4i_t t0 = get(tid), t1 = get(512 + tid);
            put(tid, t0); put(512 + tid, t1);
        }
        if (tid < 3) *(unsigned *)(a + 130 + tid) = 0u;
        __syncthreads();
        if (wave != 0) {
            constexpr int REST = 64 * (NW - 1), PER = (8192 - 1024 + REST - 1) / REST;
            v4i_t t[PER];
#pragma unroll
            for (int q = 0; q < PER; ++q) { const int e = 1024 + q * REST + (tid - 64); t[q] = e < 8192 ? get(e) : (v4i_t){0, 0, 0, 0}; }
#pragma unroll
            for (int q = 0; q < PER; ++q) { const int e = 1024 + q * REST + (tid - 64); if (e < 8192) put(e, t[q]); }
        }
    } else {
        auto put = [&](int e, v2d v) {
            const int i = 2 * (e & 63), j = e >> 6;
            if (i < j) v.x = 0.0;
            if (i + 1 < j) v.y = 0.0;
            *(v2d *)(a + i + j * DP) = v;
        };
        auto get = [&](int e) -> v2d {
            const int i = 2 * (e & 63), j = e >> 6;
            return (i + 1 >= j) ? *(const v2d *)(Kb + i + (long)j * ld) : (v2d){0.0, 0.0};
        };
        {
            v2d t0 = get(tid), t1 = get(512 + tid);
            put(tid, t0); put(512 + tid, t1);
        }
        if (tid < 3) *(unsigned *)(a + 130 + tid) = 0u;
        __syncthreads();
        if (wave != 0) {
            constexpr int REST = 64 * (NW - 1), PER = (8192 - 1024 + REST - 1) / REST;
            v2d t[PER];
#pragma unroll
            for (int q = 0; q < PER; ++q) { const int e = 1024 + q * REST + (tid - 64); t[q] = e < 8192 ? get(e) : (v2d){0.0, 0.0}; }
#pragma unroll
            for (int q = 0; q < PER; ++q) { const int e = 1024 + q * REST + (tid - 64); if (e < 8192) put(e, t[q]); }
        }
    }

    if (wave == 0) diag_step_a(a, xm, 0, lane, info, col0, sg);
    __syncthreads();
    unsigned *bflag = (unsigned *)(a + 130), *tflag = (unsigned *)(a + 131), *aflag = (unsigned *)(a + 132);
    auto count = [&](unsigned *f) {
        __builtin_amdgcn_fence(__ATOMIC_RELEASE, "wavefront");
        if (lane == 0) __hip_atomic_fetch_add(f, 1u, __ATOMIC_RELAXED, __HIP_MEMORY_SCOPE_WORKGROUP);
    };
    auto wait_for = [&](unsigned *f, unsigned want) {
        if (__hip_atomic_load(f, __ATOMIC_RELAXED, __HIP_MEMORY_SCOPE_WORKGROUP) < want)
            cip_bounded_wait<1>([&] { return __hip_atomic_load(f, __ATOMIC_RELAXED, __HIP_MEMORY_SCOPE_WORKGROUP) >= want; },
                                info + 3, CIP_GIVEUP_INWG);
        __builtin_amdgcn_fence(__ATOMIC_ACQUIRE, "wavefront");
    };
    if (!idle) {
        for (int kb = 0; kb < 7; ++kb) {
            const int c = kb * 16;
            double xa[4], di4[4], d4[4];
            if (wave == 0) {
                const unsigned tf = __hip_atomic_load(tflag, __ATOMIC_RELAXED, __HIP_MEMORY_SCOPE_WORKGROUP);
                asm volatile("" ::: "memory");
#pragma unroll
                for (int s = 0; s < 4; ++s) {
                    xa[s] = xm[kb * 256 + (g + 4 * s) * 16 + l15];
                    di4[s] = a[129 + (c + g + 4 * s) * DP];
                    d4[s] = a[128 + (c + g + 4 * s) * DP];
                }
                BcOperands bo = diag_step_bc_load(a, kb, l15, g);
                if (tf < (unsigned)(kb * NH)) {
                    wait_for(tflag, (unsigned)(kb * NH));
                    bo = diag_step_bc_load(a, kb, l15, g);
                } else __builtin_amdgcn_fence(__ATOMIC_ACQUIRE, "wavefront");
                const v4d U1 = diag_step_bc_perm(a, kb, l15, g, bo, xa, di4, d4);
                count(bflag);
                diag_step_a<true>(a, xm, kb + 1, lane, info, col0, sg, U1);
                count(aflag);
                if (PUB && kb == 6) {
#pragma unroll
                    for (int q = 0; q < 4; ++q) st_pub(xm_out + 7 * 256 + lane + 64 * q, xm[7 * 256 + lane + 64 * q]);
                    if (lane < 16) {
                        st_pub(dvec + 112 + lane, a[128 + (112 + lane) * DP]);
                        st_pub(dinv + 112 + lane, a[129 + (112 + lane) * DP]);
                    }
                    asm volatile("s_waitcnt vmcnt(0)" ::: "memory");
                    if (lane == 0) atomicAdd(stage, PANEL_STAGE_LAST);
                }
            } else {
                wait_for(aflag, (unsigned)kb);
                wait_for(tflag, (unsigned)(kb * NH));
#pragma unroll
                for (int s = 0; s < 4; ++s) {
                    xa[s] = xm[kb * 256 + (g + 4 * s) * 16 + l15];
                    di4[s] = a[129 + (c + g + 4 * s) * DP];
                    d4[s] = a[128 + (c + g + 4 * s) * DP];
                }
                for (int it = kb + 2 + hid; it < 8; it += NH) diag_step_b(a, it, c, l15, g, xa, di4);
                count(bflag);
                if (PUB && kb > 0) {
                    asm volatile("s_waitcnt vmcnt(0)" ::: "memory");
                    if (lane == 0) atomicAdd(stage, 1u);
                }
                wait_for(bflag, (unsigned)((kb + 1) * (NH + 1)));
                const int ncol = 6 - kb;
                const int ntl = ncol + (kb + 2 <= 7 ? 1 : 0);
                for (int t = hid; t < ntl; t += NH) {
                    const int it = t < ncol ? kb + 2 + t : kb + 2, jt = t < ncol ? kb + 1 : kb + 2;
                    diag_tile_left(a, it, jt, kb + 1, l15, g);
                }
                count(tflag);
#ifdef DIAG_DEBUG_SLOW_HELPERS
                if (PUB && kb == 6) { const long t0 = __builtin_amdgcn_s_memtime(); while (__builtin_amdgcn_s_memtime() - t0 < (long)(DIAG_DEBUG_SLOW_HELPERS)) __builtin_amdgcn_s_sleep(8); }
#endif
                diag_store_panel<PUB>(a, Kb, ld, c, hid * 64 + lane, 64 * NH);
                if (PUB) diag_publish_micro(a, xm, xm_out, dvec, dinv, kb, hid * 64 + lane, 64 * NH);
            }
        }
        if (PUB && wave != 0) {
            wait_for(tflag, 7u * NH);
            asm volatile("s_waitcnt vmcnt(0)" ::: "memory");
            if (lane == 0) atomicAdd(stage, 1u);
        }
    }
    __syncthreads();
    if (PUB) {
        diag_store_panel<true>(a, Kb, ld, 112, tid, 64 * NW);
        return;
    }

    diag_store_panel(a, Kb, ld, 112, tid, 64 * NW);
    if (tid < CIP_NB) {
        dvec[tid] = a[128 + tid * DP];
        dinv[tid] = a[129 + tid * DP];
    }
#pragma unroll
    for (int q = 0; q < 8; ++q)
        if (tid < 256) xm_out[q * 256 + tid] = xm[q * 256 + tid];
}

__global__ __launch_bounds__(64 * PANEL_WAVES) void k_ldlt_diag128_v2(double *Kb, long ld, double *xm_out, double *dvec, double *dinv,
                                                                      int *info, int col0, PivotSigns sg, CipBatch cb) {
    CIP_BATCH_GUARD(cb);
    CIP_BO5(cb, Kb, xm_out, dvec, dinv, info);
    extern __shared__ __attribute__((aligned(16))) double sm[];
    diag_body<false>(sm, Kb, ld, xm_out, dvec, dinv, info, col0, sg, nullptr, nullptr, 0u);
}

#define PANEL_NH (PANEL_WAVES - PANEL_WAVES / 4)
struct TrsmStrips {
    double *Ap; long ld;
    const double *L11;
    const double *xm, *dinv;
    double *W; long ldw;
    int strips;
    int nprod;
};
__device__ __forceinline__ bool stage_reached(unsigned x, int kb) {
    return kb < 7 ? (x & 0xffffu) >= (unsigned)PANEL_NH * (unsigned)(kb + 1) : (x >> 16) != 0u;
}
__device__ __forceinline__ unsigned strip_wait(unsigned v, int kb, const unsigned *stage, unsigned *slot, int *info) {
    if (stage_reached(v, kb)) return v;
    if (threadIdx.x == 0) {
        unsigned x;
        if (!cip_bounded_wait<2>([&] { return stage_reached(x = __hip_atomic_load(stage, __ATOMIC_RELAXED, __HIP_MEMORY_SCOPE_AGENT), kb); },
                                 info + 3, CIP_GIVEUP_XWG))
            x = 0xffffffffu;
        *slot = x;
    }
    __syncthreads();
    const unsigned r = *slot;
    __syncthreads();
    return r;
}
__device__ __forceinline__ unsigned strip_wait_wave(unsigned v, int kb, const unsigned *stage, int *info) {
    if (stage_reached(v, kb)) return v;
    unsigned x = 0u;
    if ((threadIdx.x & 63) == 0 &&
        !cip_bounded_wait<2>([&] { return stage_reached(x = __hip_atomic_load(stage, __ATOMIC_RELAXED, __HIP_MEMORY_SCOPE_AGENT), kb); },
                             info + 3, CIP_GIVEUP_XWG))
        x = 0xffffffffu;
    return (unsigned)__builtin_amdgcn_readfirstlane((int)x);
}
template <bool WAVEWAIT>
__device__ __forceinline__ void trsm_strip_pipelined(const TrsmStrips &tr, int strip, const unsigned *stage, unsigned *slot, int *info, double *tscr) {
    const int tid = threadIdx.x & 255, lane = tid & 63, wave = tid >> 6;
    const int l15 = lane & 15, g = lane >> 4;
    const long row = (long)strip * 64 + wave * 16 + l15;
    double *scr = tscr + wave * 272;
    double *ut = const_cast<double *>(tr.L11) + (long)(CIP_NB + strip * 64 + wave * 16) * tr.ld;
    double *ap = tr.Ap + row + (long)g * tr.ld;
    double *wp = tr.W + row + (long)g * tr.ldw;
    v4d T[8];
    unsigned v = 0;
#pragma unroll
    for (int r = 0; r < 8; ++r)
#pragma unroll
        for (int q = 0; q < 4; ++q) T[r][q] = ap[(long)(r * 16 + 4 * q) * tr.ld];
#pragma unroll
    for (int kb = 0; kb < 8; ++kb) {
        v = WAVEWAIT ? strip_wait_wave(v, kb, stage, info) : strip_wait(v, kb, stage, slot, info);
        double xo[4], dv[4], lo[7][4];
#pragma unroll
        for (int s = 0; s < 4; ++s) {
            xo[s] = ld_pub(tr.xm + kb * 256 + (g + 4 * s) * 16 + l15);
            dv[s] = ld_pub(tr.dinv + kb * 16 + 4 * s + g);
        }
#pragma unroll
        for (int r = 1; r < 8; ++r)
            if (r > kb) {
#pragma unroll
                for (int s = 0; s < 4; ++s) lo[r - 1][s] = ld_pub(tr.L11 + r * 16 + l15 + (long)(kb * 16 + 4 * s + g) * tr.ld);
            }
        v4d w = (v4d){0.0, 0.0, 0.0, 0.0};
#pragma unroll
        for (int s = 0; s < 4; ++s) w = MFMA(xo[s], T[kb][s], w);
        double wneg[4], lq[4];
#pragma unroll
        for (int q = 0; q < 4; ++q) {
            const long col = kb * 16 + 4 * q;
            wneg[q] = -w[q];
            lq[q] = w[q] * dv[q];
            wp[col * tr.ldw] = w[q];
            ap[col * tr.ld] = lq[q];
        }
#pragma unroll
        for (int s = 0; s < 4; ++s)
#pragma unroll
            for (int r = 1; r < 8; ++r)
                if (r > kb) T[r] = MFMA(lo[r - 1][s], wneg[s], T[r]);
        wave_store_T(scr, lq, ut + kb * 16, tr.ld, lane);
    }
}
__device__ __forceinline__ void diag_block_producer(const GemmArgs &g, int tile, unsigned *ready, int col0 = 0) {
    const int lane = threadIdx.x & 63, l15 = lane & 15, l4 = lane >> 4;
    int it = 0;
    while ((it + 1) * (it + 2) / 2 <= tile) ++it;
    const int jt = tile - it * (it + 1) / 2;
    const double *ap = g.A + it * 16 + l15 + (long)l4 * g.lda;
    const double *bp = g.B + jt * 16 + l15 + (long)l4 * g.ldb;
    double *cp = g.C + (it * 16 + l15) + (long)(jt * 16 + l4) * g.ldc;
    double wa[32], lb[32], cpre[4];
#pragma unroll
    for (int q = 0; q < 4; ++q) cpre[q] = cp[(long)(4 * q) * g.ldc];
#pragma unroll
    for (int ks = 0; ks < 32; ++ks) {
        wa[ks] = ap[(long)(4 * ks) * g.lda];
        lb[ks] = bp[(long)(4 * ks) * g.ldb];
    }
    v4d acc = (v4d){0.0, 0.0, 0.0, 0.0};
#pragma unroll
    for (int ks = 0; ks < 32; ++ks) acc = MFMA(lb[ks], wa[ks], acc);
#pragma unroll
    for (int q = 0; q < 4; ++q) st_pub(cp + (long)(4 * q) * g.ldc, cpre[q] + g.alpha * acc[q]);
    asm volatile("s_waitcnt vmcnt(0)" ::: "memory");
    if (lane == 0) atomicAdd(ready, 1u);
}
#define PANEL_PRODUCERS 36
#define PANEL_PRODUCER_CUS 9
#define PANEL_GRP_DOUBLES 8192
#define PANEL_NONE 0xffffffffu
__device__ __forceinline__ void panel_tile_jobs(const GemmArgs &g, double *lds, int gt, GrpBar &bar, unsigned *tileq, unsigned *slot,
                                                unsigned first_tile, unsigned nstatic) {
    const int tm = g.M / SB, tn = g.N / SB;
    const unsigned ntiles = (unsigned)(tm * (tn - 2) - (tn * (tn - 1) / 2 - 1));
    unsigned t = first_tile;
    if (t == PANEL_NONE) {
        if (gt == 0) *(volatile unsigned *)slot = __hip_atomic_fetch_add(tileq, 1u, __ATOMIC_RELAXED, __HIP_MEMORY_SCOPE_AGENT);
        grp_barrier(bar);
        t = nstatic + *(volatile unsigned *)slot;
    }
    while (t < ntiles) {
        const int npair = (tn - 2) / 2;
        int r = (int)t, ti = 0, tj = 0, p = 0;
        for (; p < npair; ++p) {
            const int j = 2 + 2 * p, n = 2 * (tm - j - 1);
            if (r < n) { ti = j + 1 + (r >> 1); tj = j + (r & 1); break; }
            r -= n;
        }
        if (p == npair) { tj = 2 + 2 * r; ti = tj; }
        t = nstatic + gemm_tile_64_k128_grp<true>(g, lds, (long)ti * SB, (long)tj * SB, gt, bar, tileq, slot);
    }
}
template <bool UPD>
__global__ __launch_bounds__(64 * PANEL_WAVES) void k_ldlt_panel(double *Kb, long ld, double *xm_out, double *dvec, double *dinv,
                                                                  int *info, int col0, PivotSigns sg, unsigned *ready, unsigned *stage,
                                                                  unsigned *tileq, GemmArgs g, TrsmStrips tr, int bt, CipBatch cb) {
    extern __shared__ __attribute__((aligned(16))) double sm[];
    const unsigned bz = bt > 0 ? blockIdx.x % (unsigned)bt : blockIdx.z;
    if (!((cb.mask >> bz) & 1ull)) return;
    {
        const long off = (long)bz * cb.stride;
        Kb = (double *)((char *)Kb + off); xm_out = (double *)((char *)xm_out + off); dvec = (double *)((char *)dvec + off);
        dinv = (double *)((char *)dinv + off); info = (int *)((char *)info + off); ready = (unsigned *)((char *)ready + off);
        stage = (unsigned *)((char *)stage + off); if (tileq) tileq = (unsigned *)((char *)tileq + off);
        g.A = (const double *)((const char *)g.A + off); g.B = (const double *)((const char *)g.B + off); g.C = (double *)((char *)g.C + off);
        tr.Ap = (double *)((char *)tr.Ap + off); tr.L11 = (const double *)((const char *)tr.L11 + off);
        tr.xm = (const double *)((const char *)tr.xm + off); tr.dinv = (const double *)((const char *)tr.dinv + off);
        tr.W = (double *)((char *)tr.W + off);
    }
    const int b = bt > 0 ? (int)(blockIdx.x / (unsigned)bt) : (int)blockIdx.x;
    const int nblocks = bt > 0 ? (int)(gridDim.x / (unsigned)bt) : (int)gridDim.x;
    if (b == 0) {
        diag_body<UPD, true>(sm, Kb, ld, xm_out, dvec, dinv, info, col0, sg, ready, stage, 36u);
        return;
    }
    if (!UPD) {
        __builtin_amdgcn_s_setprio(3);
        if (threadIdx.x >= 256) return;
        trsm_strip_pipelined<false>(tr, b - 1, stage, (unsigned *)sm, info, sm + 64);
        return;
    }
    if (b <= tr.nprod) {
        __builtin_amdgcn_s_setprio(3);
        const int pw = 36 / tr.nprod;
        if ((int)threadIdx.x < 64 * pw) diag_block_producer(g, (b - 1) * pw + (int)(threadIdx.x >> 6), ready, col0);
        return;
    }
    const int first = 1 + tr.nprod;
    const int grp = (int)(threadIdx.x >> 8), gt = (int)(threadIdx.x & 255);
    unsigned *ctl = (unsigned *)(sm + 2 * PANEL_GRP_DOUBLES);
    if (threadIdx.x < 5) ctl[threadIdx.x] = 0u;
    __syncthreads();
    GrpBar bar = {ctl + grp, 0u};
    double *lds = sm + grp * PANEL_GRP_DOUBLES;
    const int w = b - first - tr.strips, nworkers = nblocks - first - tr.strips;
    const unsigned first_tile = w >= 0 ? (unsigned)(2 * w + grp) : PANEL_NONE;
    if (w < 0) {
        const int strip = b - first;
        __builtin_amdgcn_s_setprio(3);
        gemm_tile_64_k128_grp<false>(g, lds, (long)(2 + strip) * SB, (long)grp * SB, gt, bar, nullptr, nullptr);
        asm volatile("s_waitcnt vmcnt(0)" ::: "memory");
        grp_barrier(bar);
        if (gt == 0) __hip_atomic_fetch_add(ctl + 4, 1u, __ATOMIC_RELAXED, __HIP_MEMORY_SCOPE_WORKGROUP);
        if (grp == 0) {
            while (__hip_atomic_load(ctl + 4, __ATOMIC_RELAXED, __HIP_MEMORY_SCOPE_WORKGROUP) < 2u) __builtin_amdgcn_s_sleep(1);
            asm volatile("" ::: "memory");
            trsm_strip_pipelined<true>(tr, strip, stage, nullptr, info, lds);
        }
        __builtin_amdgcn_s_setprio(0);
    }
    panel_tile_jobs(g, lds, gt, bar, tileq, ctl + 2 + grp, first_tile, (unsigned)(2 * nworkers));
}

__global__ __launch_bounds__(256) void k_diag_inverse_batched(const double *K, long ld, const double *xm_all, double *Linv,
                                                               double *LinvT, int Bs, CipBatch cb) {
    CIP_BATCH_GUARD(cb);
    CIP_BO4(cb, K, xm_all, Linv, LinvT);
    extern __shared__ __attribute__((aligned(16))) double sm[];
    constexpr int P = 130, XR = 17;
    static_assert((CIP_NB * P + 8 * 16 * XR) * 8 <= DIAG2_LDS_BYTES, "the re-pitched images must fit the launch's LDS");
    double *a = sm;
    double *xm = sm + CIP_NB * P;
    const int tid = threadIdx.x, lane = tid & 63, wave = tid >> 6;
    const int l15 = lane & 15, g = lane >> 4;
    const int jb = blockIdx.x;
    diag_load_block<P>(a, K + (long)jb * CIP_NB * (ld + 1), ld, tid);
#pragma unroll
    for (int q = 0; q < 8; ++q) xm[q * (16 * XR) + (tid >> 4) * XR + (tid & 15)] = xm_all[(size_t)jb * 2048 + q * 256 + tid];
    __syncthreads();
    diag_inverse_row<P, XR>(a, xm, wave, l15, g);
    diag_inverse_row<P, XR>(a, xm, 7 - wave, l15, g);
    __syncthreads();
    const int per = Bs / CIP_NB;
    const size_t ob = (size_t)(jb / per) * Bs * Bs + (size_t)(jb % per) * CIP_NB * (Bs + 1);
    double *Li = Linv + ob, *Lt = LinvT + ob;
    for (int e = tid; e < CIP_NB * CIP_NB; e += 256) {
        const int r = e & 127, cc = e >> 7;
        const int tr = r >> 4, tc = cc >> 4;
        double x, xt;
        if (tr == tc) {
            x = xm[tr * (16 * XR) + (cc & 15) * XR + (r & 15)];
            xt = xm[tr * (16 * XR) + (r & 15) * XR + (cc & 15)];
        } else {
            x = (tr > tc) ? a[cc + r * P] : 0.0;
            xt = (tc > tr) ? a[r + cc * P] : 0.0;
        }
        Li[r + (size_t)cc * Bs] = x;
        Lt[r + (size_t)cc * Bs] = xt;
    }
}

#define TRSM_LDS_DOUBLES (28 * 256 + 8 * 256 + 128)
__device__ __forceinline__ int trsm_tile_index(int kb, int qq) { return kb * (kb - 1) / 2 + qq; }
__global__ __launch_bounds__(256) void k_trsm_subst(double *__restrict__ Ap, long ld, const double *__restrict__ L11,
                                                        const double *__restrict__ xm, const double *__restrict__ dinv,
                                                        double *__restrict__ W, long ldw, CipBatch cb) {
    CIP_BATCH_GUARD(cb);
    CIP_BO5(cb, Ap, L11, xm, dinv, W);
    extern __shared__ __attribute__((aligned(16))) double sm[];
    double *lt = sm, *xs = sm + 28 * 256, *ds = xs + 8 * 256;
    __builtin_amdgcn_s_setprio(3);
    const int tid = threadIdx.x, lane = tid & 63, wave = tid >> 6;
    const int l15 = lane & 15, g = lane >> 4;
    const long row = (long)blockIdx.x * 64 + wave * 16 + l15;
    double *ap = Ap + row + (long)g * ld;
    double *wp = W + row + (long)g * ldw;
    double areg[8][4];
#pragma unroll
    for (int kb = 0; kb < 8; ++kb)
#pragma unroll
        for (int q = 0; q < 4; ++q) areg[kb][q] = ap[(long)(kb * 16 + 4 * q) * ld];
    {
        const int r = tid & 15, c = tid >> 4;
        double tl[28];
#pragma unroll
        for (int kb = 1; kb < 8; ++kb)
#pragma unroll
            for (int qq = 0; qq < kb; ++qq) tl[trsm_tile_index(kb, qq)] = L11[kb * 16 + r + (long)(qq * 16 + c) * ld];
        double xv[8];
#pragma unroll
        for (int kb = 0; kb < 8; ++kb) xv[kb] = xm[kb * 256 + tid];
        const double dv = tid < CIP_NB ? dinv[tid] : 0.0;
#pragma unroll
        for (int t = 0; t < 28; ++t) lt[t * 256 + c * 16 + r] = tl[t];
#pragma unroll
        for (int kb = 0; kb < 8; ++kb) xs[kb * 256 + tid] = xv[kb];
        if (tid < CIP_NB) ds[tid] = dv;
    }
    __syncthreads();
    double wneg[8][4];
    double lreg[8][4];
#pragma unroll
    for (int kb = 0; kb < 8; ++kb) {
        v4d acc = (v4d){areg[kb][0], areg[kb][1], areg[kb][2], areg[kb][3]};
#pragma unroll
        for (int qq = 0; qq < kb; ++qq) {
            const double *t = lt + trsm_tile_index(kb, qq) * 256 + g * 16 + l15;
#pragma unroll
            for (int s = 0; s < 4; ++s) acc = MFMA(t[64 * s], wneg[qq][s], acc);
        }
        v4d w = (v4d){0.0, 0.0, 0.0, 0.0};
#pragma unroll
        for (int s = 0; s < 4; ++s) w = MFMA(xs[kb * 256 + (g + 4 * s) * 16 + l15], acc[s], w);
#pragma unroll
        for (int q = 0; q < 4; ++q) {
            const long col = kb * 16 + 4 * q;
            wneg[kb][q] = -w[q];
            lreg[kb][q] = w[q] * ds[col + g];
            wp[col * ldw] = w[q];
            ap[col * ld] = lreg[kb][q];
        }
    }
    __syncthreads();
    {
        double *scr = lt + wave * 272;
        double *ut = const_cast<double *>(L11) + (long)(CIP_NB + blockIdx.x * 64 + wave * 16) * ld;
#pragma unroll
        for (int kb = 0; kb < 8; ++kb) wave_store_T(scr, lreg[kb], ut + kb * 16, ld, lane);
    }
}

#include <mutex>
static std::once_flag g_attr_once;
static hipError_t g_attr_err = hipSuccess;
static void diag_attr_init(void) {
    hipError_t e = hipFuncSetAttribute((const void *)k_ldlt_diag128_v2, hipFuncAttributeMaxDynamicSharedMemorySize, DIAG2_LDS_BYTES);
    if (e == hipSuccess) e = hipFuncSetAttribute((const void *)k_ldlt_panel<true>, hipFuncAttributeMaxDynamicSharedMemorySize, DIAG2_LDS_BYTES);
    if (e == hipSuccess) e = hipFuncSetAttribute((const void *)k_ldlt_panel<false>, hipFuncAttributeMaxDynamicSharedMemorySize, DIAG2_LDS_BYTES);
    if (e == hipSuccess) e = hipFuncSetAttribute((const void *)k_diag_inverse_batched, hipFuncAttributeMaxDynamicSharedMemorySize, DIAG2_LDS_BYTES);
    if (e == hipSuccess) e = hipFuncSetAttribute((const void *)k_trsm_subst, hipFuncAttributeMaxDynamicSharedMemorySize, (int)(TRSM_LDS_DOUBLES * sizeof(double)));
    g_attr_err = e;
}
int cip_kernels_init(void) {
    std::call_once(g_attr_once, diag_attr_init);
    if (g_attr_err != hipSuccess) { cip_set_error("hipFuncSetAttribute failed: %s", hipGetErrorString(g_attr_err)); return -3; }
    return 0;
}
int cip_launch_diag_v2(hipStream_t s, double *Kb, long ld, double *xm_out, double *dvec, double *dinv, int *info, int col0,
                       PivotSigns sg) {
    if (cip_kernels_init()) return -3;
    cip_launch_b(k_ldlt_diag128_v2, dim3(1), dim3(64 * PANEL_WAVES), DIAG2_LDS_BYTES, s, Kb, ld, xm_out, dvec, dinv, info, col0, sg);
    CIP_HIP_CHECK(hipGetLastError());
    return 0;
}
int cip_launch_panel(hipStream_t s, double *Kb, long ld, double *xm_out, double *dvec, double *dinv, int *info, int col0,
                     PivotSigns sg, unsigned *ready, unsigned *stage, unsigned *tileq, const GemmArgs *g, int rows, double *W, long ldw) {
    if (cip_kernels_init()) return -3;
    TrsmStrips tr = {Kb + CIP_NB, ld, Kb, xm_out, dinv, W, ldw, rows / 64, PANEL_PRODUCER_CUS};
    const int Bn = cip_in_batch() ? cip_tl_bz.B : 1;
    const bool transposed = Bn > 1;
    if (g) {
        const int tm = g->M / SB, tn = g->N / SB;
        if (tm != tr.strips + 2 || tn < 2) { cip_set_error("panel launch: update / TRSM shapes disagree"); return -1; }
        static const int ncu = [] {
            int dev = 0, cus = 256;
            if (hipGetDevice(&dev) == hipSuccess) (void)hipDeviceGetAttribute(&cus, hipDeviceAttributeMultiprocessorCount, dev);
            return cus;
        }();
        const long ntiles = (long)tm * (tn - 2) - ((long)tn * (tn - 1) / 2 - 1);
        long workers = ncu / Bn - 1 - PANEL_PRODUCER_CUS - tr.strips;
        if (workers > (ntiles + 1) / 2) workers = (ntiles + 1) / 2;
        if (workers < 1 && ntiles > 0 && tr.strips == 0) workers = 1;
        if (workers < 0) workers = 0;
        tr.nprod = Bn > 1 ? PANEL_PRODUCER_CUS : PANEL_PRODUCERS;
        const long grid = 1 + tr.nprod + tr.strips + workers;
        if (transposed) cip_launch(k_ldlt_panel<true>, dim3((unsigned)(grid * Bn)), dim3(64 * PANEL_WAVES), DIAG2_LDS_BYTES, s, Kb, ld, xm_out, dvec, dinv, info,
                                   col0, sg, ready, stage, tileq, *g, tr, Bn, CipBatch{cip_tl_bz.stride, cip_tl_bz.mask});
        else cip_launch_b(k_ldlt_panel<true>, dim3((unsigned)grid), dim3(64 * PANEL_WAVES), DIAG2_LDS_BYTES, s, Kb, ld, xm_out, dvec, dinv, info, col0, sg,
                          ready, stage, tileq, *g, tr, 0);
    } else {
        if (transposed) cip_launch(k_ldlt_panel<false>, dim3((unsigned)((1 + tr.strips) * Bn)), dim3(64 * PANEL_WAVES), DIAG2_LDS_BYTES, s, Kb, ld, xm_out, dvec,
                                   dinv, info, col0, sg, ready, stage, tileq, GemmArgs{}, tr, Bn, CipBatch{cip_tl_bz.stride, cip_tl_bz.mask});
        else cip_launch_b(k_ldlt_panel<false>, dim3((unsigned)(1 + tr.strips)), dim3(64 * PANEL_WAVES), DIAG2_LDS_BYTES, s, Kb, ld, xm_out, dvec, dinv,
                          info, col0, sg, ready, stage, tileq, GemmArgs{}, tr, 0);
    }
    CIP_HIP_CHECK(hipGetLastError());
    return 0;
}
int cip_launch_diag_inverse(hipStream_t s, const double *K, long ld, int nblk, const double *xm_all, double *Linv,
                            double *LinvT, int Bs) {
    if (cip_kernels_init()) return -3;
    cip_launch_b(k_diag_inverse_batched, dim3(nblk), dim3(256), DIAG2_LDS_BYTES, s, K, ld, xm_all, Linv, LinvT, Bs);
    CIP_HIP_CHECK(hipGetLastError());
    return 0;
}
int cip_launch_trsm_subst(hipStream_t s, double *Ap, long ld, int rows, const double *L11, const double *xm,
                          const double *dinv, double *W, long ldw) {
    if (rows <= 0) return 0;
    if (cip_kernels_init()) return -3;
    cip_launch_b(k_trsm_subst, dim3(rows / 64), dim3(256), TRSM_LDS_DOUBLES * sizeof(double), s, Ap, ld, L11, xm, dinv, W, ldw);
    CIP_HIP_CHECK(hipGetLastError());
    return 0;
}
```

conicip.jl_amd/csrc/ldlt.hip:

```cpp
#include "cip_internal.h"
#include "cip_gemm_tile.h"
#include <stdlib.h>
#include <string.h>

#include <atomic>
#include <mutex>
#include <vector>
static std::atomic<int> g_nbo{0};
static std::atomic<int> g_fuse_diag{-1};
static std::once_flag g_fuse_once;
static void fuse_env(void) {
    std::call_once(g_fuse_once, [] {
        g_fuse_diag = cip_env_int("CIP_FUSE_DIAG", 3) == 0 ? 0 : 3;
    });
}
int cip_ldlt_outer_block_for(int Npad) {
    { const int v = g_nbo.load(std::memory_order_relaxed); if (v > 0) return v; }
    fuse_env();
    static const int nbo_auto = [] { const int v = cip_env_int("CIP_LDLT_NBO_AUTO", 896); return (v >= 256 && v <= 1024 && v % CIP_NB == 0) ? v : 896; }();
    return (Npad >= 4096 && g_fuse_diag) ? nbo_auto : 512;
}
#define CIP_NBO_MAX 1024
#define CIP_TAIL_MAX 3072
static size_t wbuf_cols(int Npad) { return Npad >= 4096 ? (Npad < CIP_TAIL_MAX ? Npad : CIP_TAIL_MAX) : CIP_NBO_MAX; }
// ... 39 lines not shown
    if (!p) return -1;
    if (p->used) CIP_HIP_CHECK(hipEventSynchronize(p->pool[p->used - 1]));
    for (size_t i = 0; i + 1 < p->used; i += 2) {
        float t = 0;
        CIP_HIP_CHECK(hipEventElapsedTime(&t, p->pool[i], p->pool[i + 1]));
        p->tot_ms += t;
        p->tot_flops += p->flops[i / 2];
        p->tot_launches += 1;
    }
    p->used = 0;
    p->flops.clear();
    if (launches) *launches = p->tot_launches;
    if (ms) *ms = p->tot_ms;
    if (flops) *flops = p->tot_flops;
    return 0;
}

static thread_local LdltProfile *g_tl_prof = nullptr;
int cip_ldlt_profile_thread(int enabled) {
    if (enabled && !g_tl_prof) g_tl_prof = cip_ldlt_profile_create();
    if (!enabled && g_tl_prof) { cip_ldlt_profile_destroy(g_tl_prof); g_tl_prof = nullptr; }
    return 0;
}
int cip_ldlt_profile_thread_collect(double *launches, double *ms, double *flops) {
    return cip_ldlt_profile_collect(g_tl_prof, launches, ms, flops);
}

static thread_local LdltProfile *g_tl_aux[CIP_PROF_SLOTS] = {nullptr, nullptr, nullptr};
int cip_prof_slot_enable(int slot, int enabled) {
    if (slot == 0) return cip_ldlt_profile_thread(enabled);
    if (slot < 0 || slot >= CIP_PROF_SLOTS) return -1;
    if (enabled && !g_tl_aux[slot]) g_tl_aux[slot] = cip_ldlt_profile_create();
    if (!enabled && g_tl_aux[slot]) { cip_ldlt_profile_destroy(g_tl_aux[slot]); g_tl_aux[slot] = nullptr; }
    return 0;
}
int cip_prof_slot_collect(int slot, double *launches, double *ms, double *flops) {
    if (slot == 0) return cip_ldlt_profile_thread_collect(launches, ms, flops);
    if (slot < 0 || slot >= CIP_PROF_SLOTS) return -1;
    return cip_ldlt_profile_collect(g_tl_aux[slot], launches, ms, flops);
}
int cip_prof_slot_begin(int slot, hipStream_t s, double work) {
    LdltProfile *p = (slot > 0 && slot < CIP_PROF_SLOTS && !cip_tl_builder) ? g_tl_aux[slot] : nullptr;
    if (!p) return 0;
    int rc = prof_event(p, s);
    if (rc) return rc;
    p->flops.push_back(work);
    return 0;
}
int cip_prof_slot_end(int slot, hipStream_t s) {
    LdltProfile *p = (slot > 0 && slot < CIP_PROF_SLOTS && !cip_tl_builder) ? g_tl_aux[slot] : nullptr;
    return p ? prof_event(p, s) : 0;
}

static std::atomic<int> g_solve_block_max{-1};
thread_local int cip_tl_solve_block_max = 0;
int cip_solve_block_max_set(int b) {
    if (g_solve_block_max.load() < 0) { int v = -1; g_solve_block_max.compare_exchange_strong(v, cip_env_int("CIP_SOLVE_BLOCK", 1024)); }
    const int prev = g_solve_block_max.load();
    if (b == 128 || b == 256 || b == 512 || b == 1024) g_solve_block_max.store(b);
    return prev;
}
int cip_solve_block(int Npad) {
    int mx = cip_tl_solve_block_max > 0 ? cip_tl_solve_block_max : cip_solve_block_max_set(0);
    if (mx < CIP_NB) mx = CIP_NB;
    for (int b = 2048; b > CIP_NB; b >>= 1)
        if (b <= mx && Npad % b == 0) return b;
    return CIP_NB;
}

static std::atomic<int> g_solve_fused{-1};
int cip_solve_fused_set(int mode) {
    if (g_solve_fused.load() < 0) { int v = -1; g_solve_fused.compare_exchange_strong(v, cip_env_int("CIP_SOLVE_FUSED", 0)); }
    const int prev = g_solve_fused.load();
    if (mode == 0 || mode == 1 || mode == 2) g_solve_fused.store(mode);
    return prev;
}
static int solve_fused_for(int Npad, int Bs) {
    const int mode = cip_solve_fused_set(-1);
    if (Npad / Bs < 2) return 0;
    return mode == 2 || (mode == 1 && Bs <= 512);
}

int cip_ldlt_fused_for(int Npad) { return solve_fused_for(Npad, cip_solve_block(Npad)); }
static size_t ldlt_ws_layout(CipLayout L, int Npad, LdltWorkspace *ws, int fused) {
    const size_t nblk = Npad / CIP_NB;
    ws->Bs = cip_solve_block(Npad);
    const size_t nbk = Npad / ws->Bs, blk = nbk * (size_t)ws->Bs * ws->Bs, half = ws->Bs / 2;
    ws->Wbuf = L.take<double>((size_t)Npad * wbuf_cols(Npad));
    ws->Linv = L.take<double>(nblk * CIP_NB * CIP_NB); ws->LinvT = L.take<double>(nblk * CIP_NB * CIP_NB);
    ws->Xm = L.take<double>(nblk * 2048);
    ws->X = L.take<double>(blk); ws->XT = L.take<double>(blk);
    ws->Tt = L.take<double>(nbk * half * half + 32);
    ws->zbuf = L.take<double>(Npad); ws->dinv = L.take<double>(Npad); ws->dvec = L.take<double>(Npad); ws->tmp = L.take<double>(Npad);
    ws->info = L.take<int>(16 + 3 * nblk);
    ws->fused = (fused != 0 && nbk >= 2) ? 1 : 0;
    ws->MT = ws->fused ? L.take<double>(blk) : nullptr; ws->PT = ws->fused ? L.take<double>(blk) : nullptr;
    return L.bytes();
}
size_t cip_ldlt_ws_bytes(int Npad, int fused) { LdltWorkspace ws; return ldlt_ws_layout(nullptr, Npad, &ws, fused); }
void cip_ldlt_ws_carve(void *base, int Npad, LdltWorkspace *ws, int fused) {
    ldlt_ws_layout(base, Npad, ws, fused);
    ws->prof = nullptr;
    ws->lazyC = nullptr; ws->lazy_ld = 0; ws->lazy_diag = nullptr;
    ws->signs = PivotSigns{-1, 0, 0};
    ws->x_zeroed = nullptr;
    ws->side = nullptr;
    ws->no_prep = 0;
    ws->unfused = 0;
}

int cip_launch_diag_v2(hipStream_t s, double *Kb, long ld, double *xm_out, double *dvec, double *dinv, int *info, int col0,
                       PivotSigns sg);
int cip_launch_diag_inverse(hipStream_t s, const double *K, long ld, int nblk, const double *xm_all, double *Linv,
                            double *LinvT, int Bs);
int cip_launch_panel(hipStream_t s, double *Kb, long ld, double *xm_out, double *dvec, double *dinv, int *info, int col0,
                     PivotSigns sg, unsigned *ready, unsigned *stage, unsigned *tileq, const GemmArgs *g, int rows, double *W, long ldw);
int cip_launch_trsm_subst(hipStream_t s, double *Ap, long ld, int rows, const double *L11, const double *xm,
                          const double *dinv, double *W, long ldw);

struct RestOfBlock { int M, N; const double *A, *B; double *C; };
static bool rest_of_block(double *K, int Npad, long ld, double *Wb, int C0, int wblk, int t, RestOfBlock &r) {
    const int c1 = C0 + (t + 1) * CIP_NB;
    const int ncols = C0 + wblk - c1;
    if (ncols <= 0 || c1 >= Npad) return false;
    r = RestOfBlock{Npad - c1, ncols, Wb + c1 + (long)(t * CIP_NB) * Npad, K + c1 + (long)(c1 - CIP_NB) * ld, K + c1 + (long)c1 * ld};
    return true;
}
static int update_rest_of_block(hipStream_t s, double *K, int Npad, long ld, double *Wb, int C0, int wblk, int t) {
    RestOfBlock r;
    if (!rest_of_block(K, Npad, ld, Wb, C0, wblk, t, r)) return 0;
    return cip_gemm_rect(s, r.M, r.N, CIP_NB, -1.0, r.A, Npad, r.B, ld, r.C, ld);
}
int cip_ldlt_set_fused_chain(int on) { fuse_env(); const int prev = g_fuse_diag; if (on == 0 || on == 3) g_fuse_diag = on; return prev; }

static thread_local bool tl_ran_fused = false;

static int factor_outer_panels(hipStream_t s, double *K, int Npad, long ld, const LdltWorkspace &ws, double *Wb, int C0,
                               int wblk, int t0 = 0, int t1 = -1) {
    int rc;
    const int T = t1 < 0 ? wblk / CIP_NB : t1;
    for (int t = t0; t < T; ++t) {
        const int c0 = C0 + t * CIP_NB;
        const int jb = c0 / CIP_NB;
        const int r = Npad - c0 - CIP_NB;
        GemmArgs gu;
        fuse_env();
        static const int lsmax = cip_env_int("CIP_LOCKSTEP_PANEL_MAX", 32);
        static const int lscus = [] {
            if (cip_env_set("CIP_LOCKSTEP_PANEL_CUS")) return cip_env_int("CIP_LOCKSTEP_PANEL_CUS", 0);
            int dev = 0, cus = 256;
            if (hipGetDevice(&dev) == hipSuccess) (void)hipDeviceGetAttribute(&cus, hipDeviceAttributeMultiprocessorCount, dev);
            return 4 * cus;
        }();
        const bool small_group = cip_in_batch() && cip_tl_bz.B <= lsmax && (long)cip_tl_bz.B * (10 + Npad / 64) <= lscus;
        const bool fuse = g_fuse_diag && !ws.unfused && (!cip_in_batch() || small_group);
        if (fuse) {
            tl_ran_fused = true;
            RestOfBlock rb;
            const bool upd = t > 0 && rest_of_block(K, Npad, ld, Wb, C0, wblk, t - 1, rb);
            if (upd) gu = GemmArgs{rb.A, Npad, rb.B, ld, rb.C, ld, rb.M, rb.N, CIP_NB, -1.0};
            unsigned *ctr = (unsigned *)(ws.info + 16);
            if ((rc = cip_launch_panel(s, K + c0 + (long)c0 * ld, ld, ws.Xm + (size_t)jb * 2048, ws.dvec + c0, ws.dinv + c0, ws.info, c0,
                                       ws.signs, ctr + jb, ctr + Npad / CIP_NB + jb, ctr + 2 * (Npad / CIP_NB) + jb, upd ? &gu : nullptr, r,
                                       Wb + (c0 + CIP_NB) + (long)(t * CIP_NB) * Npad, Npad)))
                return rc;
            continue;
        }
        if ((rc = cip_launch_diag_v2(s, K + c0 + (long)c0 * ld, ld, ws.Xm + (size_t)jb * 2048, ws.dvec + c0,
                                     ws.dinv + c0, ws.info, c0, ws.signs)))
            return rc;
        if ((rc = cip_launch_trsm_subst(s, K + (c0 + CIP_NB) + (long)c0 * ld, ld, r, K + c0 + (long)c0 * ld,
                                        ws.Xm + (size_t)jb * 2048, ws.dinv + c0,
                                        Wb + (c0 + CIP_NB) + (long)(t * CIP_NB) * Npad, Npad)))
            return rc;
        if ((rc = update_rest_of_block(s, K, Npad, ld, Wb, C0, wblk, t))) return rc;
    }
    return 0;
}

__global__ __launch_bounds__(256) void k_zero_words(unsigned *p, size_t nwords, CipBatch cb) {
    CIP_BATCH_GUARD(cb);
    CIP_BO1(cb, p);
    for (size_t i = (size_t)blockIdx.x * 256 + threadIdx.x; i < nwords; i += (size_t)gridDim.x * 256) p[i] = 0u;
}
static int zero_fill(hipStream_t s, void *p, size_t bytes) {
    const size_t nw = bytes / 4;
    size_t nb = (nw + 255) / 256;
    if (nb > 2048) nb = 2048;
    if (nb == 0) return 0;
    cip_launch_b(k_zero_words, dim3((unsigned)nb), dim3(256), 0, s, (unsigned *)p, nw);
    CIP_HIP_CHECK(hipGetLastError());
    return 0;
}

static int ensure_x_zeroed(hipStream_t s, int Npad, const LdltWorkspace &ws) {
    const int Bs = ws.Bs;
    if (Bs == CIP_NB || (ws.x_zeroed && *ws.x_zeroed)) return 0;
    int rc;
    const int nall = Npad / Bs;
    if ((rc = zero_fill(s, ws.X, sizeof(double) * (size_t)nall * Bs * Bs))) return rc;
    if ((rc = zero_fill(s, ws.XT, sizeof(double) * (size_t)nall * Bs * Bs))) return rc;
    if (ws.x_zeroed && (!cip_in_batch() || cip_tl_bz.mask == (cip_tl_bz.B >= 64 ? ~0ull : ((1ull << cip_tl_bz.B) - 1)))) *ws.x_zeroed = 1;
    return 0;
}
__global__ __launch_bounds__(256, 4) void k_solve_premul(const double *K, long ld, const double *X, const double *XT, double *MT,
                                                         double *PT, int Bs, int jm0, int nm, int jp0, CipBatch cb) {
    __shared__ __attribute__((aligned(16))) double lds[2 * 2 * CIP_KT * SB];
    CIP_BATCH_GUARD(cb);
    CIP_BO5(cb, K, X, XT, MT, PT);
    const int tm = Bs / SB;
    const long i0 = (long)(blockIdx.x % tm) * SB, j0 = (long)(blockIdx.x / tm) * SB;
    const long bs2 = (long)Bs * Bs;
    GemmArgs g = {};
    g.alpha = 1.0; g.ldb = Bs; g.ldc = Bs; g.lda = ld;
    if ((int)blockIdx.y < nm) {
        const long J = jm0 + blockIdx.y;
        g.A = K + (J - 1) * Bs + J * Bs * ld;
        g.B = X + J * bs2;
        g.C = MT + J * bs2;
        g.K = (int)(j0 + SB);
    } else {
        const long J = jp0 + ((int)blockIdx.y - nm);
        g.A = K + (J + 1) * Bs + J * Bs * ld + j0 * ld;
        g.B = XT + J * bs2 + j0 * Bs;
        g.C = PT + J * bs2;
        g.K = (int)(Bs - j0);
    }
    gemm_tile_64<EPI_STORE>(g, lds, i0, j0);
}
static int doubling_tiny(int Bs, int J0, int nbk_all) {
    return Bs == 1024 && J0 == nbk_all - 1;
}
static int build_solve_premul(hipStream_t s, double *K, long ld, const LdltWorkspace &ws, int nbk_all, int J0, int J1) {
    if (!ws.fused) return 0;
    const int Bs = ws.Bs;
    const double *X = (Bs == CIP_NB) ? ws.Linv : ws.X, *XT = (Bs == CIP_NB) ? ws.LinvT : ws.XT;
    const int jm0 = J0 > 1 ? J0 : 1, nm = J1 - jm0 > 0 ? J1 - jm0 : 0;
    const int jp1 = J1 < nbk_all - 1 ? J1 : nbk_all - 1, np = jp1 - J0 > 0 ? jp1 - J0 : 0;
    if (nm + np == 0) return 0;
    const int tm = Bs / SB;
    cip_launch_b(k_solve_premul, dim3((unsigned)(tm * tm), (unsigned)(nm + np)), dim3(256), 0, s, (const double *)K, ld, X, XT, ws.MT, ws.PT, Bs, jm0, nm, J0);
    CIP_HIP_CHECK(hipGetLastError());
    return 0;
}

static int build_solve_blocks(hipStream_t s, double *K, int Npad, long ld, const LdltWorkspace &ws, int J0 = 0, int J1 = -1) {
    const int Bs = ws.Bs;
    if (J1 < 0) J1 = Npad / Bs;
    if (J1 - J0 > 1 && J1 == Npad / Bs && doubling_tiny(Bs, J1 - 1, Npad / Bs)) {
        const int rc0 = build_solve_blocks(s, K, Npad, ld, ws, J0, J1 - 1);
// ... 74 lines not shown
    if (sd->nfork >= 16) return build_solve_blocks(s, K, Npad, ld, ws, J0, J1);
    const int g = sd->nfork++;
    sd->j0[g] = J0;
    hipStream_t t = sd->s2;
    CIP_HIP_CHECK(hipEventRecord(sd->fork[g], s));
    CIP_HIP_CHECK(hipStreamWaitEvent(t, sd->fork[g], 0));
    static const long delay_us = cip_env_long("CIP_DEBUG_SIDE_DELAY_US", 0L);
    if (delay_us > 0) { hipLaunchKernelGGL(k_debug_spin, dim3(1), dim3(64), 0, t, delay_us * 100); CIP_HIP_CHECK(hipGetLastError()); }
    const int rc = build_solve_blocks(t, K, Npad, ld, ws, J0, J1);
    CIP_HIP_CHECK(hipEventRecord(sd->done[g], t));
    return rc;
}
int cip_ldlt_side_join(hipStream_t s, const LdltWorkspace &ws, int J) {
    LdltSide *sd = ws.side ? *ws.side : nullptr;
    if (!sd) return 0;
    while (sd->waited < sd->nfork && (J < 0 || sd->j0[sd->waited] <= J)) {
        CIP_HIP_CHECK(hipStreamWaitEvent(s, sd->done[sd->waited], 0));
        sd->waited += 1;
    }
    return 0;
}

static std::atomic<int> g_debug_giveup{0}, g_debug_giveup_skip{0}, g_debug_giveup_kind{0}, g_debug_redo_pivot{0}, g_debug_redo_armed{0};
int cip_debug_chain_giveup_set(int n) {
    const int prev = g_debug_giveup.load();
    if (n >= 0) {
        g_debug_giveup_kind.store((n >> 28) & 3);
        g_debug_redo_pivot.store((n >> 30) & 1);
        g_debug_redo_armed.store(0);
        g_debug_giveup_skip.store((n >> 16) & 0xfff);
        g_debug_giveup.store(n & 0xffff);
    }
    return prev;
}
__global__ void k_debug_set_word(int *p, int v, CipBatch cb) {
    CIP_BATCH_GUARD(cb);
    CIP_BO1(cb, p);
    if (threadIdx.x == 0) *p = v;
}
__global__ __launch_bounds__(256) void k_debug_poison_strip(double *K, long ld, CipBatch cb) {
    CIP_BATCH_GUARD(cb);
    CIP_BO1(cb, K);
    const int i = 64 + (threadIdx.x & 63);
    for (int j = threadIdx.x >> 6; j < 64; j += 4) K[i + (long)j * ld] *= 1.0 + 0x1p-20;
}
int cip_ldlt_debug_giveup(hipStream_t s, double *K, int Npad, long ld, const LdltWorkspace &ws, bool fused) {
    if (!fused) {
        int armed = 1;
        if (g_debug_redo_armed.load() > 0 && g_debug_redo_armed.compare_exchange_strong(armed, 0)) {
            cip_launch_b(k_debug_set_word, dim3(1), dim3(64), 0, s, ws.info + 0, 1);
            CIP_HIP_CHECK(hipGetLastError());
        }
        return 0;
    }
    if (g_debug_giveup.load() <= 0 || g_debug_giveup_skip.fetch_sub(1) > 0 || g_debug_giveup.fetch_sub(1) <= 0) return 0;
    const int kind = g_debug_giveup_kind.load();
    if (kind & 1) {
        cip_launch_b(k_debug_set_word, dim3(1), dim3(64), 0, s, ws.info + 0, 1);
    } else {
        cip_launch_b(k_debug_set_word, dim3(1), dim3(64), 0, s, ws.info + 3, CIP_GIVEUP_XWG);
        if (g_debug_redo_pivot.load()) g_debug_redo_armed.store(1);
    }
    CIP_HIP_CHECK(hipGetLastError());
    if ((kind & 2) && !(kind & 1)) {
        int rc;
        if ((rc = cip_ldlt_side_join(s, ws, -1))) return rc;
        cip_launch_b(k_debug_poison_strip, dim3(1), dim3(256), 0, s, K, ld);
        CIP_HIP_CHECK(hipGetLastError());
        if (!ws.no_prep && (rc = build_solve_blocks(s, K, Npad, ld, ws, 0, 1))) return rc;
    }
    return 0;
}
bool cip_ldlt_last_factor_fused(void) { return tl_ran_fused; }
static int ldlt_factor_body(hipStream_t s, double *K, int Npad, long ld, const LdltWorkspace &ws);
int cip_ldlt_factor(hipStream_t s, double *K, int Npad, long ld, const LdltWorkspace &ws) {
    tl_ran_fused = false;
    const int rc = ldlt_factor_body(s, K, Npad, ld, ws);
    if (rc == 0 && !cip_tl_builder) return cip_ldlt_debug_giveup(s, K, Npad, ld, ws, tl_ran_fused);
    return rc;
}
static int ldlt_factor_body(hipStream_t s, double *K, int Npad, long ld, const LdltWorkspace &ws) {
    if (Npad % CIP_NB) { cip_set_error("ldlt: N must be a multiple of 128"); return -1; }
    int rc;
    if ((rc = zero_fill(s, ws.info, 64 + 12 * (size_t)(Npad / CIP_NB)))) return rc;
    if ((rc = ensure_x_zeroed(s, Npad, ws))) return rc;
    const int Bs = ws.Bs;
    LdltProfile *prof_this = ws.prof ? ws.prof : (cip_tl_builder ? nullptr : g_tl_prof);
    if (prof_this && (prof_this->nfact++ % prof_this->stride) != 0) prof_this = nullptr;
    LdltSide *sd = nullptr;
    int Jdone = 0;
    for (int C0 = 0, wblk = 0; C0 < Npad; C0 += wblk) {
        wblk = outer_block_width(Npad, C0);
        const bool last = C0 + wblk >= Npad;
        if (last && side_prep_mode() && !cip_in_batch() && !cip_tl_builder && Bs > CIP_NB && Npad / Bs >= 2 &&
            wblk >= 2 * cip_ldlt_outer_block_for(Npad) && wblk > Bs && (sd = side_get(ws))) {
            if ((rc = cip_ldlt_side_join(s, ws, -1))) return rc;
            sd->nfork = 0; sd->waited = 0;
            fuse_env();
            static const int side_from = cip_env_int("CIP_SIDE_PREP_FROM", 2048);
            for (int c = C0; c < Npad; ) {
                if (c % (Bs > 1024 ? Bs : 1024) == 0 && Npad - c <= side_from && c / Bs > Jdone) {
                    if ((rc = side_fork(sd, s, K, Npad, ld, ws, Jdone, c / Bs))) return rc;
                    Jdone = c / Bs;
                }
                int cend = (c / Bs + 1) * Bs;
                if (cend > Npad) cend = Npad;
                if ((rc = factor_outer_panels(s, K, Npad, ld, ws, ws.Wbuf, C0, wblk, (c - C0) / CIP_NB, (cend - C0) / CIP_NB))) return rc;
                c = cend;
            }
            continue;
        }
        if ((rc = factor_outer_panels(s, K, Npad, ld, ws, ws.Wbuf, C0, wblk))) return rc;
        const int r0 = C0 + wblk;
        if (r0 < Npad) {
            const double *Wr = ws.Wbuf + r0, *Lr = K + r0 + (long)C0 * ld;
            double *Cr = K + r0 + (long)r0 * ld;
            const bool lazy = C0 == 0 && ws.lazyC;
            LdltProfile *prof = prof_this;
            if (prof) {
                if ((rc = prof_event(prof, s))) return rc;
                const double r = (double)(Npad - r0);
                const double live = cip_in_batch() ? (double)__builtin_popcountll(cip_tl_bz.mask) : 1.0;
                prof->flops.push_back(live * r * (r + 1.0) * (double)wblk);
            }
            if ((rc = lazy ? cip_gemm_lower_lazyc(s, Npad - r0, wblk, -1.0, Wr, Npad, Lr, ld, Cr, ld, ws.lazyC + r0 + (long)r0 * ws.lazy_ld, ws.lazy_ld,
                                                  ws.lazy_diag + r0)
                           : cip_gemm_lower(s, Npad - r0, wblk, -1.0, Wr, Npad, Lr, ld, Cr, ld))) return rc;
            if (prof && (rc = prof_event(prof, s))) return rc;
        }
    }
    if (sd && sd->nfork > 0) {
        return side_fork(sd, s, K, Npad, ld, ws, Jdone, Npad / Bs);
    }
    if (ws.no_prep) return 0;
    return build_solve_blocks(s, K, Npad, ld, ws, Jdone, Npad / Bs);
}

__global__ __launch_bounds__(256) void k_scale_vec(int n, const double *x, const double *d, double *y, CipBatch cb) {
    CIP_BATCH_GUARD(cb);
    CIP_BO3(cb, x, d, y);
    const int i = blockIdx.x * 256 + threadIdx.x;
    if (i < n) y[i] = x[i] * d[i];
}

struct SolveStepArgs {
    const double *T, *M, *v, *u;
    double *out, *out2; const double *dsc;
    int Bs, tri;
    const double *Bm; long ldb; double *tgt; int ncols;
};
__device__ __forceinline__ double lane_dot(const double *a, const double *x, int r0, int r1, int lane) {
    double s0 = 0, s1 = 0, s2 = 0, s3 = 0;
    int i = r0 + lane * 2;
    for (; i + 384 < r1; i += 512) {
        const v2d a0 = *(const v2d *)(a + i), a1 = *(const v2d *)(a + i + 128), a2 = *(const v2d *)(a + i + 256), a3 = *(const v2d *)(a + i + 384);
        const v2d x0 = *(const v2d *)(x + i), x1 = *(const v2d *)(x + i + 128), x2 = *(const v2d *)(x + i + 256), x3 = *(const v2d *)(x + i + 384);
        s0 = fma(a0.x, x0.x, s0); s1 = fma(a0.y, x0.y, s1);
        s2 = fma(a1.x, x1.x, s2); s3 = fma(a1.y, x1.y, s3);
        s0 = fma(a2.x, x2.x, s0); s1 = fma(a2.y, x2.y, s1);
        s2 = fma(a3.x, x3.x, s2); s3 = fma(a3.y, x3.y, s3);
    }
    for (; i < r1; i += 128) {
        const v2d av = *(const v2d *)(a + i), xv = *(const v2d *)(x + i);
        s0 = fma(av.x, xv.x, s0); s1 = fma(av.y, xv.y, s1);
    }
    return (s0 + s1) + (s2 + s3);
}
// ... 82 lines not shown
```

conicip.jl_amd/csrc/sdp_large.hip:

```cpp
#include "cip_handle.h"
#include "cip_gemm_tile.h"
#include "cip_sdp_numerics.h"
#include "../../include/cipkkt.h"
#include <atomic>
#include <stdio.h>
#include <string.h>
#include <thread>

#define LG_T 1024

__device__ int g_lz_hist[40];
#define LG_NPAD 4
enum {
    LG_V_LAM = 0,
    LG_V_DG = 1, LG_V_OF = 2,
    LG_V_XBUF = 3, LG_V_PBUF = 5,
    LG_V_SCAL = 7,
    LG_V_DG1 = 9, LG_V_OF1 = 10,
    LG_V_CERT = 11, LG_V_SLOTS = 12
};
enum {
    LG_C_BARRIER = 0,
    LG_C_SWEEP = 8,
    LG_C_GIVEUP = 128,
// ... 1146 lines not shown
        hipLaunchKernelGGL(k_lg_vok, dim3(1), dim3(256), 0, s, (const double *)lam, rp, (const int *)w->wz.info, (const int *)w->ws.info, vst);
        w->have_v[li] = left_cone ? 0 : 1;
    }
    hipLaunchKernelGGL(k_lg_build, lg_grid(n2), dim3(256), 0, s, w->G, lam, w->wz.dvec, w->Kz, w->M1, w->M2, w->M3, rp);
    const double *XTz = (w->wz.Bs == CIP_NB) ? w->wz.LinvT : w->wz.XT;
    if ((rc = lg_gemm(s, w->Tz, 0, XTz, 0, w->M1, 0, rp, 1))) return rc;
    if ((rc = lg_gemm(s, w->Ts, 0, w->M2, 0, w->M3, 0, rp, 1))) return rc;
    double *R = scal + cd.soff, *Ri = R + (size_t)r * r;
    hipLaunchKernelGGL(k_lg_store, lg_grid(n2 > cd.dim ? n2 : cd.dim), dim3(256), 0, s, w->Tz, w->Ts, R, Ri, w->Rip + LG_NPAD * (size_t)li * n2,
                       lam, lambda ? lambda + cd.off : nullptr, r, rp, cd.dim);
    if (lambda) hipLaunchKernelGGL(k_lg_lambda_diag, lg_grid(r), dim3(256), 0, s, lam, lambda + cd.off, r);
    CIP_HIP_CHECK(hipGetLastError());
    return 0;
}

int cip_sdp_large_refresh(hipStream_t s, LargeWs *w, const ConeDesc &cd, int li, const double *scal) {
    const int r = cd.r, rp = w->rp;
    w->have_v[li] = 0;
    hipLaunchKernelGGL(k_lg_pad, lg_grid((long)rp * rp), dim3(256), 0, s, scal + cd.soff, scal + cd.soff + (size_t)r * r,
                       w->Rip + LG_NPAD * (size_t)li * rp * rp, r, rp);
    CIP_HIP_CHECK(hipGetLastError());
    return 0;
}

static int lz_reorth(void) {
    static const int on = cip_env_int("CIP_LG_LANCZOS_REORTH", 0);
    return on;
}
int cip_sdp_large_lanczos(int on) {
    static std::atomic<int> mode{[] { const int v = cip_env_int("CIP_LG_LANCZOS", 2); return (v >= 0 && v <= 3) ? v : 2; }()};
    const int prev = mode.load();
    if (on >= 0 && on <= 3) mode.store(on);
    return prev;
}
bool cip_sdp_large_pairable(const LargeWs *w) { return w && w->rp <= 256 && cip_sdp_large_lanczos(-1); }
int cip_sdp_large_fork(hipStream_t s, LargeWs *w, hipStream_t *s2) {
    if (!w->s2) {
        CIP_HIP_CHECK(hipStreamCreateWithFlags(&w->s2, hipStreamNonBlocking));
        CIP_HIP_CHECK(hipEventCreateWithFlags(&w->efork, hipEventDisableTiming));
        CIP_HIP_CHECK(hipEventCreateWithFlags(&w->ejoin, hipEventDisableTiming));
    }
    CIP_HIP_CHECK(hipEventRecord(w->efork, s));
    CIP_HIP_CHECK(hipStreamWaitEvent(w->s2, w->efork, 0));
    *s2 = w->s2;
    return 0;
}
int cip_sdp_large_join(hipStream_t s, LargeWs *w) {
    CIP_HIP_CHECK(hipEventRecord(w->ejoin, w->s2));
    CIP_HIP_CHECK(hipStreamWaitEvent(s, w->ejoin, 0));
    return 0;
}
__global__ __launch_bounds__(256) void k_lg_cert_build(const double *M, int ldm, const double *dscale, int r, int rp, int want_max,
                                                        const double *cert, double *B, double *Asym) {
    const long e = (long)blockIdx.x * 256 + threadIdx.x;
    if (e >= (long)rp * rp) return;
    const int i = (int)(e % rp), j = (int)(e / rp);
    double a = 0.0, b = (i == j) ? 1.0 : 0.0;
    if (i < r && j < r) {
        a = sd_scaled_sym_entry(M, ldm, dscale, j, i);
        if (cert[1] == 0.0) {
            const double th = (i == j) ? cert[0] : 0.0;
            b = want_max ? th - a : a - th;
        }
    }
    B[e] = b;
    Asym[e] = a;
}
__global__ void k_lg_cert_check(const int *info, int *gate, unsigned *count) {
    if (threadIdx.x == 0) {
        const int up = (info[0] != 0 || info[2] != 0) ? 1 : 0;
        gate[0] = up;
        if (up) atomicAdd(count, 1u);
    }
}
static int lg_certify(hipStream_t s, LargeWs *w, const double *M3, const double *dscale, int r, int want_max, double scale,
                      double *M1, double *M2, const LdltWorkspace &wx, double *partial, int item, int side) {
    const int rp = w->rp;
    const long n2 = (long)rp * rp;
    int rc;
    const double *cert = w->cert(side);
    int *gate = (int *)(w->ctr + LG_C_GATE + side);
    hipLaunchKernelGGL(k_lg_cert_build, lg_grid(n2), dim3(256), 0, s, M3, rp, dscale, r, rp, want_max, cert, M2, M1);
    LdltWorkspace wc = wx;
    wc.no_prep = 1; wc.lazyC = nullptr; wc.prof = nullptr;
    if ((rc = cip_ldlt_factor(s, M2, rp, rp, wc))) return rc;
    hipLaunchKernelGGL(k_lg_cert_check, dim3(1), dim3(64), 0, s, (const int *)wc.info, gate, w->fallbacks());
    double *dg = w->dg(side), *of = w->of(side);
    const size_t shm1 = T1_LDS_DOUBLES * sizeof(double);
    if ((rc = lg_set_attr((const void *)k_lg_tridiag1, shm1))) return rc;
    hipLaunchKernelGGL(k_lg_tridiag1, dim3(1), dim3(512), shm1, s, (const double *)M1, rp, (const double *)nullptr, r, dg, of, (const int *)gate);
    hipLaunchKernelGGL(k_lg_sturm, dim3(1), dim3(LG_T), 0, s, dg, of, r, want_max, scale, (const int *)nullptr, partial, item, (const int *)gate);
    CIP_HIP_CHECK(hipGetLastError());
    return 0;
}
int cip_sdp_large_cert_stats(hipStream_t s, LargeWs *w, int *out2) {
    unsigned c = 0;
    if (w) { CIP_HIP_CHECK(hipMemcpyAsync(&c, w->fallbacks(), sizeof(c), hipMemcpyDeviceToHost, s)); CIP_HIP_CHECK(hipStreamSynchronize(s)); }
    out2[0] = (int)c; out2[1] = 0;
    return 0;
}

int cip_sdp_large_maxstep(hipStream_t s, LargeWs *w, const ConeDesc &cd, const double *x, const double *d, double scale,
                          double *partial, int side) {
    const int r = cd.r, rp = w->rp;
    const long n2 = (long)rp * rp;
    int rc;
    double *dg = w->dg(), *of = w->of();
    double *const Kx = side ? w->Ks : w->Kz, *const M1 = side ? w->Tz : w->M1, *const M2 = side ? w->Ts : w->M2, *const M3 = side ? w->G : w->M3;
    LdltWorkspace &wx = side ? w->ws : w->wz;
    int *const stat = (int *)(w->ctr + LG_C_STAT + side);
    const int lzmode = cip_sdp_large_lanczos(-1);
    const bool lz = lzmode && r <= 256;
    double *const cert = (lz && lzmode >= 2) ? w->cert(side) : nullptr;
    const double cert_tol = lzmode == 3 ? -1e-3 : 1e-9;
    if (lz && (rc = lg_set_attr((const void *)k_lg_lanczos1, LZ_LDS_DOUBLES * sizeof(double)))) return rc;
    if (!d) {
        hipLaunchKernelGGL(k_lg_mat, lg_grid(n2), dim3(256), 0, s, x + cd.off, 1L, 0L, M3, r, rp, 0.0);
        if (lz) {
            hipLaunchKernelGGL(k_lg_lanczos1, dim3(1), dim3(512), LZ_LDS_DOUBLES * sizeof(double), s, M3, rp, (const double *)nullptr, r, 0,
                               1.0, (const int *)nullptr, partial, cd.item, M1, stat, cert, cert_tol, lz_reorth());
            CIP_HIP_CHECK(hipGetLastError());
            if (cert) return lg_certify(s, w, M3, nullptr, r, 0, 1.0, M1, M2, wx, partial, cd.item, side);
            return 0;
        }
        if ((rc = lg_tridiag(s, w, M3, nullptr, r, M2))) return rc;
        hipLaunchKernelGGL(k_lg_sturm, dim3(1), dim3(LG_T), 0, s, dg, of, r, 0, 1.0, (const int *)nullptr, partial, cd.item);
        CIP_HIP_CHECK(hipGetLastError());
        return 0;
    }
    hipLaunchKernelGGL(k_lg_mat, lg_grid(n2), dim3(256), 0, s, x + cd.off, 1L, 0L, Kx, r, rp, 1.0);
    if ((rc = cip_ldlt_factor(s, Kx, rp, rp, wx))) return rc;
    const double *Xi = (wx.Bs == CIP_NB) ? wx.Linv : wx.X;
    if (rp <= 256) {
        hipLaunchKernelGGL((k_gemm_nt_small<true, false>), dim3(rp / 16, rp / 16), dim3(256), 0, s, Xi, (long)rp, d + cd.off, 0L, M2, (long)rp, rp, r);
    } else {
        hipLaunchKernelGGL(k_lg_mat, lg_grid(n2), dim3(256), 0, s, d + cd.off, 1L, 0L, M1, r, rp, 0.0);
        if ((rc = lg_gemm(s, M2, 0, Xi, 0, M1, 0, rp, 1))) return rc;
    }
    if ((rc = lg_gemm(s, M3, 0, M2, 0, Xi, 0, rp, 1))) return rc;
    if (lz) {
        hipLaunchKernelGGL(k_lg_lanczos1, dim3(1), dim3(512), LZ_LDS_DOUBLES * sizeof(double), s, M3, rp, (const double *)wx.dvec, r, 1,
                           scale, (const int *)wx.info, partial, cd.item, M1, stat, cert, cert_tol, lz_reorth());
        CIP_HIP_CHECK(hipGetLastError());
        if (cert) return lg_certify(s, w, M3, wx.dvec, r, 1, scale, M1, M2, wx, partial, cd.item, side);
        return 0;
    }
    if ((rc = lg_tridiag(s, w, M3, wx.dvec, r, M2))) return rc;
    hipLaunchKernelGGL(k_lg_sturm, dim3(1), dim3(LG_T), 0, s, dg, of, r, 1, scale, (const int *)wx.info, partial, cd.item);
    CIP_HIP_CHECK(hipGetLastError());
    return 0;
}

void cip_sdp_large_invalidate(LargeWs *w) {
    if (w) for (auto &p : w->amat_src) p = nullptr;
}
int cip_sdp_large_scale_At(hipStream_t s, LargeWs *w, const ConeDesc &cd, int li, int n, const double *At, long ldat, double *Wt,
                           long ldwt) {
    const int r = cd.r, rp = w->rp;
    const long n2 = (long)rp * rp;
    const double *Rip = w->Rip + LG_NPAD * (size_t)li * n2;
    const long dim = (long)r * (r + 1) / 2;
    int rc;
    const bool cached = w->amat && n == w->ncols && n <= w->chunk;
    double *amat = cached ? w->amat + (size_t)li * n * n2 : nullptr;
    if (cached && w->amat_src[li] != At) {
        dim3 gm((unsigned)((n2 + 255) / 256), n);
        hipLaunchKernelGGL(k_lg_mat, gm, dim3(256), 0, s, At + (long)cd.aoff * ldat, ldat, 1L, amat, r, rp, 0.0);
// ... 74 lines not shown
```

include/cipkkt.h:

```cpp
#ifndef CIPKKT_H
#define CIPKKT_H

#include <stddef.h>

#ifdef __cplusplus
extern "C" {
#endif

typedef struct cip_handle cip_handle;

#define CIP_CONE_R 0
#define CIP_CONE_Q 1
#define CIP_CONE_S 2

#define CIP_ROUTE_SCHUR   0
#define CIP_ROUTE_FULL3X3 1

#define CIP_OP_F      0
#define CIP_OP_FT     1
#define CIP_OP_FINV   2
#define CIP_OP_FINVT  3

#define CIP_MAT_Q 0
#define CIP_MAT_A 1
// ... 71 lines not shown

int cip_gemv_dev(cip_handle *h, int which, int trans, double alpha, const double *x, double beta, double *y);
int cip_dots_dev(cip_handle *h, int count, const double *const *x, const double *const *y,
                 const int *len, double *out_host);
int cip_axpby_dev(cip_handle *h, int len, double alpha, const double *x, double beta, double *y);

#define CIP_STATUS_NONE       0
#define CIP_STATUS_OPTIMAL    1
#define CIP_STATUS_INFEASIBLE 2
#define CIP_STATUS_UNBOUNDED  3
#define CIP_STATUS_ABANDONED  4
#define CIP_STATUS_ERROR      5
#define CIP_TRACE_COLS 9
typedef struct cip_options {
    double optTol, DTB, infeasTol, refinementThreshold;
    int maxRefinementSteps, maxIters, verbose;
} cip_options;
typedef struct cip_result {
    int status, iter;
    double mu, prFeas, duFeas, muFeas, pobj, dobj;
    int n_factor, n_solve, trace_rows;
    double wall_s;
} cip_result;
int cip_conicip(cip_handle *h, const double *c, const double *b, const double *d, const cip_options *opt,
                double *y, double *w, double *v, cip_result *res, double *trace, int trace_cap);

typedef struct cip_batch cip_batch;
int cip_batch_create(int count, const cip_problem *probs, cip_batch **out);
int cip_batch_destroy(cip_batch *b);
int cip_batch_size(const cip_batch *b);
cip_handle *cip_batch_handle(cip_batch *b, int i);
int cip_batch_conicip(cip_batch *b, const double *const *c, const double *const *bvec, const double *const *d,
                      const cip_options *opt, double *const *y, double *const *w, double *const *v, cip_result *res,
                      int in_flight);
int cip_conicip_problems(int count, const cip_problem *probs, const double *const *c, const double *const *bvec,
                         const double *const *d, const cip_options *opt, double *const *y, double *const *w,
                         double *const *v, cip_result *res, int in_flight);
int cip_conicip_lockstep(int count, const cip_problem *probs, const double *const *c, const double *const *bvec,
                         const double *const *d, const cip_options *opt, double *const *y, double *const *w,
                         double *const *v, cip_result *res);
int cip_conicip_mixed(int count, const cip_problem *probs, const double *const *c, const double *const *bvec,
                      const double *const *d, const cip_options *opt, double *const *y, double *const *w,
                      double *const *v, cip_result *res, int in_flight);
int cip_release_cached_memory(void);
int cip_lockstep_stats(int *out3);
int cip_set_lockstep_regularize(int on);
int cip_set_lockstep_ragged(int on);
int cip_lockstep_regularized(int *count);
int cip_set_lockstep_split(int k);
int cip_conicip_many(cip_handle *const *handles, int count, const double *const *c, const double *const *bvec,
                     const double *const *d, const cip_options *opt, double *const *y, double *const *w,
                     double *const *v, cip_result *res, int in_flight);

int cip_ldlt_workspace_bytes(int N, size_t *bytes);
int cip_ldlt_factor_dev(void *hip_stream, double *K, int N, int ld, void *workspace, int *info_host);
int cip_ldlt_solve_dev(void *hip_stream, const double *K, int N, int ld, const void *workspace, double *rhs);
int cip_ldlt_solve_many_scratch_bytes(int N, int nrhs, size_t *bytes);
int cip_ldlt_solve_many_dev(void *hip_stream, const double *K, int N, int ld, const void *workspace,
                            void *scratch, double *B, int ldb, int nrhs);
int cip_gemm_nt_dev(void *hip_stream, int M, int N, int K, double alpha,
                    const double *A, int lda, const double *B, int ldb, double *C, int ldc, int lower_only);

int cip_qrcp_workspace_bytes(int len, int cnt, size_t *bytes);
int cip_imcols_workspace_bytes(int len, int cnt, size_t *bytes);
int cip_qrcp_dev(void *hip_stream, double *M, int len, int cnt, int ld, double stop, void *workspace,
                 double *tau_dev, int *piv_host, double *rdiag_host, int *k_host);
int cip_imcols_dev(void *hip_stream, const double *M, int len, int cnt, int ld, const double *b, double eps,
                   void *workspace, int *rows_host, int *nrows_host, int *consistent_host, double *resid_host);

int cip_kkt_order(const cip_handle *h, int *N, int *N_padded);
int cip_get_kkt_matrix(cip_handle *h, double *K_host );
int cip_assemble_only(cip_handle *h);
int cip_stats(cip_handle *h, double *out8);
int cip_set_timing(cip_handle *h, int enabled);
int cip_set_ldlt_outer_block(int nbo);
int cip_set_solve_block_max(int b);
int cip_set_solve_fused(int mode);
int cip_lockstep_solve_block_for(int B);
int cip_set_ldlt_fused_chain(int on);
int cip_debug_chain_giveup(int n);
int cip_get_chain_fallbacks(cip_handle *h);
int cip_set_ldlt_side_prep(int on);
int cip_set_lazy_copy(int on);
int cip_set_sdp_lanczos(int on);
int cip_sdp_lanczos_fallbacks(cip_handle *h, int *count);
int cip_profile_trailing(cip_handle *h, int enabled);
int cip_profile_get(cip_handle *h, double *out3);
int cip_profile_trailing_thread(int enabled);
int cip_profile_thread_get(double *out3);
#define CIP_PROFILE_TRAILING 0
#define CIP_PROFILE_SYRK     1
#define CIP_PROFILE_JACOBI   2
int cip_profile_kernel_thread(int slot, int enabled);
int cip_profile_kernel_thread_get(int slot, double *out3);

#ifdef __cplusplus
}
#endif
#endif
```

Before: 203.0.

## Read first outer block lazily from Q in fused panel chain, skip copy

When the lazy Schur assembly path applies and the fused panel chain is used, the first outer block of K is no longer copied from Q. The diag, TRSM strip, diag-producer and GEMM tile kernels instead read it directly from Q, with the diagonal taken from the precomputed kdiag. The diagonal assembly kernel also zeroes the LDLT info/flag words, so the factor can skip a separate memset launch. This removes a copy kernel and a fill per factorisation. In exchange it adds more template variants, extra branches in hot loads, and a graph-invalidation condition keyed on the new flag.

Result: slower. 200.4 (-1.3%).

```diff
diff --git a/conicip.jl_amd/cipkkt/_lib.py b/conicip.jl_amd/cipkkt/_lib.py
--- a/conicip.jl_amd/cipkkt/_lib.py
+++ b/conicip.jl_amd/cipkkt/_lib.py
@@ -130,6 +130,7 @@
     "cip_profile_kernel_thread": (C.c_int, [C.c_int, C.c_int]),
     "cip_profile_kernel_thread_get": (C.c_int, [C.c_int, c_double_p]),
     "cip_set_lazy_copy": (C.c_int, [C.c_int]),
+    "cip_set_lazy_first": (C.c_int, [C.c_int]),
     "cip_set_sdp_lanczos": (C.c_int, [C.c_int]),
     "cip_set_lockstep_split": (C.c_int, [C.c_int]),
     "cip_debug_chain_giveup": (C.c_int, [C.c_int]),
diff --git a/conicip.jl_amd/csrc/api.hip b/conicip.jl_amd/csrc/api.hip
--- a/conicip.jl_amd/csrc/api.hip
+++ b/conicip.jl_amd/csrc/api.hip
@@ -662,10 +662,11 @@
     if (h->timing) CIP_HIP_CHECK(hipEventRecord(h->ev1, h->stream));
     {
         CipRange rg("cip:ldlt");
-        if (h->gx_factor && (h->gx_factor_lazyC != h->ws.lazyC || h->gx_factor_unfused != h->ws.unfused)) {
+        if (h->gx_factor && (h->gx_factor_lazyC != h->ws.lazyC || h->gx_factor_lazy_first != h->ws.lazy_first || h->gx_factor_unfused != h->ws.unfused)) {
             (void)hipGraphExecDestroy(h->gx_factor); h->gx_factor = nullptr;
         }
         h->gx_factor_lazyC = h->ws.lazyC;
+        h->gx_factor_lazy_first = h->ws.lazy_first;
         h->gx_factor_unfused = h->ws.unfused;
         bool replayed = false;
         CIP_TRY(graph_run(h, &h->gx_factor, [&]() {
@@ -964,6 +965,7 @@
     return 0;
 }
 extern "C" int cip_set_lazy_copy(int on) { return cip_lazy_copy_set(on); }
+extern "C" int cip_set_lazy_first(int on) { return cip_lazy_first_set(on); }
 extern "C" int cip_set_sdp_lanczos(int on) { return cip_sdp_large_lanczos(on); }
 extern "C" int cip_debug_chain_giveup(int n) { return cip_debug_chain_giveup_set(n); }
 extern "C" int cip_get_chain_fallbacks(cip_handle *h) { return h ? h->n_chain_fallbacks : -1; }
diff --git a/conicip.jl_amd/csrc/assemble.hip b/conicip.jl_amd/csrc/assemble.hip
--- a/conicip.jl_amd/csrc/assemble.hip
+++ b/conicip.jl_amd/csrc/assemble.hip
@@ -144,11 +144,12 @@
 __global__ __launch_bounds__(256) void k_schur_diag_lazy(int n, int nb0, const int *trp, const int *tci, const double *tv, const int *rp,
                                                           const int *ci, const double *av, const int *row_cone, const ConeDesc *cones,
                                                           const double *scal, const double *Q, long ldq, double *K, long ldk, double *kdiag,
-                                                          CipBatch cb) {
+                                                          int *info, int ninfo, CipBatch cb) {
     CIP_BATCH_GUARD(cb);
     CIP_BO8(cb, trp, tci, tv, rp, ci, av, scal, Q);
-    CIP_BO2(cb, K, kdiag);
-    const int i = blockIdx.x * 256 + threadIdx.x;
+    CIP_BO3(cb, K, kdiag, info);
+    const int i = blockIdx.x * 256 + threadIdx.x;
+    if (info && i < ninfo) info[i] = 0;
     if (i >= n) return;
     double d = i < nb0 ? K[i + (long)i * ldk] : Q[i + (long)i * ldq];
     for (int q = trp[i]; q < trp[i + 1]; ++q) {
@@ -289,11 +290,23 @@
     if (on == 0 || on == 1) g_lazy_copy.store(on);
     return prev;
 }
+static std::atomic<int> g_lazy_first{-1};
+int cip_lazy_first_set(int on) {
+    int prev = g_lazy_first.load(std::memory_order_relaxed);
+    if (prev < 0) {
+        const int env = cip_env_int("CIP_LAZY_FIRST", 1) != 0;
+        int expect = -1;
+        g_lazy_first.compare_exchange_strong(expect, env);
+        prev = g_lazy_first.load(std::memory_order_relaxed);
+    }
+    if (on == 0 || on == 1) g_lazy_first.store(on);
+    return prev;
+}
 static int assemble_schur(cip_handle *h, bool lazy_ok) {
     hipStream_t s = h->stream;
     int rc;
     const int n = h->n, p = h->p;
-    h->ws.lazyC = nullptr;
+    h->ws.lazyC = nullptr; h->ws.info_zeroed = 0; h->ws.lazy_first = 0;
     if (!h->A_sparse) {
         if ((rc = cip_cones_scale_At(s, h->cs, n, h->At, h->npad, h->Wt, h->npad))) return rc;
         if ((rc = cip_prof_slot_begin(CIP_PROF_SYRK, s, (double)h->m * (double)n * (double)n * (cip_in_batch() ? (double)__builtin_popcountll(cip_tl_bz.mask) : 1.0)))) return rc;
@@ -308,11 +321,15 @@
         const int nb0 = cip_ldlt_outer_block_for(h->Npad);
         if (!h->Q_sparse && lazy_on && lazy_ok && all_r && cip_grp_A_one_per_row(h) && p == 0 && h->Npad == n && n > nb0 && h->reg_rel <= 0.0 && h->kdiag &&
             copy_lower_vectorisable(h->K, h->ldk, 0, h->Q, (long)n, n)) {
-            launch_copy_block_lower(s, h->K, h->ldk, 0, h->Q, (long)n, n, 1.0, nb0);
-            cip_launch_b(k_schur_diag_lazy, dim3((n + 255) / 256), dim3(256), 0, s, n, nb0, h->T_rp, h->T_ci, h->T_v, h->A_rp, h->A_ci, h->A_v,
-                         h->row_cone, h->cs.d_cones, h->cs.d_scal, h->Q, (long)n, h->K, h->ldk, h->kdiag);
+            const int lazy_first = cip_lazy_first_set(-1) && cip_ldlt_lazy_first_for(h->ws, h->Npad);
+            if (!lazy_first) launch_copy_block_lower(s, h->K, h->ldk, 0, h->Q, (long)n, n, 1.0, nb0);
+            const int ninfo = cip_ldlt_info_words(h->Npad);
+            if (ninfo > n) { cip_set_error("assemble: the flag words outnumber the diagonal launch's threads"); return -1; }
+            cip_launch_b(k_schur_diag_lazy, dim3((n + 255) / 256), dim3(256), 0, s, n, lazy_first ? 0 : nb0, h->T_rp, h->T_ci, h->T_v, h->A_rp, h->A_ci, h->A_v,
+                         h->row_cone, h->cs.d_cones, h->cs.d_scal, h->Q, (long)n, h->K, h->ldk, h->kdiag, h->ws.info, ninfo);
             CIP_HIP_CHECK(hipGetLastError());
             h->ws.lazyC = h->Q; h->ws.lazy_ld = n; h->ws.lazy_diag = h->kdiag;
+            h->ws.info_zeroed = 1; h->ws.lazy_first = lazy_first;
             return 0;
         }
         if (h->Q_sparse) {
@@ -446,7 +463,7 @@
 }
 
 int cip_assemble(cip_handle *h, bool lazy_ok) {
-    h->ws.lazyC = nullptr;
+    h->ws.lazyC = nullptr; h->ws.info_zeroed = 0; h->ws.lazy_first = 0;
     { const int rj = cip_ldlt_side_join(h->stream, h->ws, -1); if (rj) return rj; }
     int rc = (h->route == CIP_ROUTE_SCHUR) ? assemble_schur(h, lazy_ok) : assemble_full(h);
     if (rc == 0 && h->reg_rel > 0.0) rc = cip_regularize(h, h->reg_rel);
diff --git a/conicip.jl_amd/csrc/cip_gemm_tile.h b/conicip.jl_amd/csrc/cip_gemm_tile.h
--- a/conicip.jl_amd/csrc/cip_gemm_tile.h
+++ b/conicip.jl_amd/csrc/cip_gemm_tile.h
@@ -182,7 +182,7 @@
     while (__hip_atomic_load(b.ctr, __ATOMIC_RELAXED, __HIP_MEMORY_SCOPE_WORKGROUP) < b.gen) __builtin_amdgcn_s_sleep(1);
     asm volatile("" ::: "memory");
 }
-template <bool QUEUE>
+template <bool QUEUE, bool LAZY = false>
 __device__ __forceinline__ unsigned gemm_tile_64_k128_grp(const GemmArgs &g, double *lds, long i0, long j0, int gt, GrpBar &bar,
                                                           unsigned *tileq, unsigned *slot) {
     const int lane = gt & 63;
@@ -224,7 +224,17 @@
 #pragma unroll
             for (int tj = 0; tj < 2; ++tj)
 #pragma unroll
-                for (int q = 0; q < 4; ++q) cpre[tj][q] = *(const v2d *)(g.C + rowo + (j0 + wn * 32 + 2 * (l4 + 4 * q) + tj) * g.ldc);
+                for (int q = 0; q < 4; ++q) {
+                    const long col = j0 + wn * 32 + 2 * (l4 + 4 * q) + tj;
+                    if (LAZY) {
+                        v2d c = *(const v2d *)(g.Qin + rowo + col * g.ldq);
+                        if (rowo == col) c.x = g.Cdiag[rowo];
+                        if (rowo + 1 == col) c.y = g.Cdiag[col];
+                        cpre[tj][q] = c;
+                    } else {
+                        cpre[tj][q] = *(const v2d *)(g.C + rowo + col * g.ldc);
+                    }
+                }
         }
         if (qt < 3) {
             double *na = lds + ((qt + 1) & 1) * (64 * SB), *nb = na + 32 * SB;
diff --git a/conicip.jl_amd/csrc/cip_handle.h b/conicip.jl_amd/csrc/cip_handle.h
--- a/conicip.jl_amd/csrc/cip_handle.h
+++ b/conicip.jl_amd/csrc/cip_handle.h
@@ -72,6 +72,7 @@
 
     hipGraphExec_t gx_factor = nullptr, gx_solve = nullptr;
     const double *gx_factor_lazyC = nullptr;
+    int gx_factor_lazy_first = 0;
     int gx_factor_unfused = 0;
     bool gx_factor_fused = false;
     int graph_state = 0;
@@ -82,6 +83,7 @@
 };
 
 int cip_lazy_copy_set(int on);
+int cip_lazy_first_set(int on);
 int cip_scatter_AtS(cip_handle *h);
 int cip_assemble(cip_handle *h, bool lazy_ok = false);
 #define CIP_AUTO_REG 1e-13
diff --git a/conicip.jl_amd/csrc/cip_internal.h b/conicip.jl_amd/csrc/cip_internal.h
--- a/conicip.jl_amd/csrc/cip_internal.h
+++ b/conicip.jl_amd/csrc/cip_internal.h
@@ -152,6 +152,8 @@
     PivotSigns signs;
     LdltProfile *prof;
     const double *lazyC; long lazy_ld; const double *lazy_diag;
+    int lazy_first;
+    int info_zeroed;
     struct LdltSide **side;
     int no_prep;
     int unfused;
@@ -170,6 +172,9 @@
 int cip_solve_fused_set(int mode);
 extern thread_local int cip_tl_solve_block_max;
 int cip_ldlt_fused_for(int Npad);
+bool cip_ldlt_chain_fused(const struct LdltWorkspace &ws, int Npad);
+bool cip_ldlt_lazy_first_for(const struct LdltWorkspace &ws, int Npad);
+int cip_ldlt_info_words(int Npad);
 size_t cip_ldlt_ws_bytes(int Npad, int fused);
 void cip_ldlt_ws_carve(void *base, int Npad, LdltWorkspace *ws, int fused);
 int cip_ldlt_factor(hipStream_t s, double *K, int Npad, long ld, const LdltWorkspace &ws);
diff --git a/conicip.jl_amd/csrc/diag.hip b/conicip.jl_amd/csrc/diag.hip
--- a/conicip.jl_amd/csrc/diag.hip
+++ b/conicip.jl_amd/csrc/diag.hip
@@ -298,10 +298,11 @@
     }
 }
 
-template <bool WAIT, bool PUB = false>
+template <bool WAIT, bool PUB = false, bool LAZY = false>
 __device__ __forceinline__ void diag_body(double *sm, double *Kb, long ld, double *xm_out, double *dvec, double *dinv,
                                           int *info, int col0, PivotSigns sg, const unsigned *ready, unsigned *stage,
-                                          unsigned ready_target) {
+                                          unsigned ready_target, const double *Cin = nullptr, long ldcin = 0, const double *Cdiag = nullptr) {
+    static_assert(!(WAIT && LAZY), "a block that other workgroups of the launch update is read from K");
     double *a = sm;
     double *xm = sm + XM_OFF;
     const int tid = threadIdx.x, lane = tid & 63, wave = __builtin_amdgcn_readfirstlane(tid >> 6);
@@ -355,6 +356,13 @@
         };
         auto get = [&](int e) -> v2d {
             const int i = 2 * (e & 63), j = e >> 6;
+            if (LAZY) {
+                if (i + 1 < j) return (v2d){0.0, 0.0};
+                v2d v = *(const v2d *)(Cin + i + (long)j * ldcin);
+                if (i == j) v.x = Cdiag[i];
+                if (i + 1 == j) v.y = Cdiag[j];
+                return v;
+            }
             return (i + 1 >= j) ? *(const v2d *)(Kb + i + (long)j * ld) : (v2d){0.0, 0.0};
         };
         {
@@ -513,8 +521,9 @@
         x = 0xffffffffu;
     return (unsigned)__builtin_amdgcn_readfirstlane((int)x);
 }
-template <bool WAVEWAIT>
-__device__ __forceinline__ void trsm_strip_pipelined(const TrsmStrips &tr, int strip, const unsigned *stage, unsigned *slot, int *info, double *tscr) {
+template <bool WAVEWAIT, bool LAZY = false>
+__device__ __forceinline__ void trsm_strip_pipelined(const TrsmStrips &tr, int strip, const unsigned *stage, unsigned *slot, int *info, double *tscr,
+                                                     const double *Tin = nullptr, long ldtin = 0) {
     const int tid = threadIdx.x & 255, lane = tid & 63, wave = tid >> 6;
     const int l15 = lane & 15, g = lane >> 4;
     const long row = (long)strip * 64 + wave * 16 + l15;
@@ -527,7 +536,7 @@
 #pragma unroll
     for (int r = 0; r < 8; ++r)
 #pragma unroll
-        for (int q = 0; q < 4; ++q) T[r][q] = ap[(long)(r * 16 + 4 * q) * tr.ld];
+        for (int q = 0; q < 4; ++q) T[r][q] = LAZY ? Tin[row + (long)(g + r * 16 + 4 * q) * ldtin] : ap[(long)(r * 16 + 4 * q) * tr.ld];
 #pragma unroll
     for (int kb = 0; kb < 8; ++kb) {
         v = WAVEWAIT ? strip_wait_wave(v, kb, stage, info) : strip_wait(v, kb, stage, slot, info);
@@ -563,6 +572,7 @@
         wave_store_T(scr, lq, ut + kb * 16, tr.ld, lane);
     }
 }
+template <bool LAZY = false>
 __device__ __forceinline__ void diag_block_producer(const GemmArgs &g, int tile, unsigned *ready, int col0 = 0) {
     const int lane = threadIdx.x & 63, l15 = lane & 15, l4 = lane >> 4;
     int it = 0;
@@ -573,7 +583,14 @@
     double *cp = g.C + (it * 16 + l15) + (long)(jt * 16 + l4) * g.ldc;
     double wa[32], lb[32], cpre[4];
 #pragma unroll
-    for (int q = 0; q < 4; ++q) cpre[q] = cp[(long)(4 * q) * g.ldc];
+    for (int q = 0; q < 4; ++q) {
+        if (LAZY) {
+            const int row = it * 16 + l15, col = jt * 16 + l4 + 4 * q;
+            cpre[q] = row == col ? g.Cdiag[row] : g.Qin[row + (long)col * g.ldq];
+        } else {
+            cpre[q] = cp[(long)(4 * q) * g.ldc];
+        }
+    }
 #pragma unroll
     for (int ks = 0; ks < 32; ++ks) {
         wa[ks] = ap[(long)(4 * ks) * g.lda];
@@ -591,6 +608,7 @@
 #define PANEL_PRODUCER_CUS 9
 #define PANEL_GRP_DOUBLES 8192
 #define PANEL_NONE 0xffffffffu
+template <bool LAZY = false>
 __device__ __forceinline__ void panel_tile_jobs(const GemmArgs &g, double *lds, int gt, GrpBar &bar, unsigned *tileq, unsigned *slot,
                                                 unsigned first_tile, unsigned nstatic) {
     const int tm = g.M / SB, tn = g.N / SB;
@@ -610,10 +628,10 @@
             r -= n;
         }
         if (p == npair) { tj = 2 + 2 * r; ti = tj; }
-        t = nstatic + gemm_tile_64_k128_grp<true>(g, lds, (long)ti * SB, (long)tj * SB, gt, bar, tileq, slot);
-    }
-}
-template <bool UPD>
+        t = nstatic + gemm_tile_64_k128_grp<true, LAZY>(g, lds, (long)ti * SB, (long)tj * SB, gt, bar, tileq, slot);
+    }
+}
+template <bool UPD, bool LAZY = false>
 __global__ __launch_bounds__(64 * PANEL_WAVES) void k_ldlt_panel(double *Kb, long ld, double *xm_out, double *dvec, double *dinv,
                                                                   int *info, int col0, PivotSigns sg, unsigned *ready, unsigned *stage,
                                                                   unsigned *tileq, GemmArgs g, TrsmStrips tr, int bt, CipBatch cb) {
@@ -629,23 +647,24 @@
         tr.Ap = (double *)((char *)tr.Ap + off); tr.L11 = (const double *)((const char *)tr.L11 + off);
         tr.xm = (const double *)((const char *)tr.xm + off); tr.dinv = (const double *)((const char *)tr.dinv + off);
         tr.W = (double *)((char *)tr.W + off);
+        if (LAZY) { g.Qin = (const double *)((const char *)g.Qin + off); g.Cdiag = (const double *)((const char *)g.Cdiag + off); }
     }
     const int b = bt > 0 ? (int)(blockIdx.x / (unsigned)bt) : (int)blockIdx.x;
     const int nblocks = bt > 0 ? (int)(gridDim.x / (unsigned)bt) : (int)gridDim.x;
     if (b == 0) {
-        diag_body<UPD, true>(sm, Kb, ld, xm_out, dvec, dinv, info, col0, sg, ready, stage, 36u);
+        diag_body<UPD, true, LAZY && !UPD>(sm, Kb, ld, xm_out, dvec, dinv, info, col0, sg, ready, stage, 36u, g.Qin, g.ldq, g.Cdiag);
         return;
     }
     if (!UPD) {
         __builtin_amdgcn_s_setprio(3);
         if (threadIdx.x >= 256) return;
-        trsm_strip_pipelined<false>(tr, b - 1, stage, (unsigned *)sm, info, sm + 64);
+        trsm_strip_pipelined<false, LAZY>(tr, b - 1, stage, (unsigned *)sm, info, sm + 64, LAZY ? g.Qin + CIP_NB : nullptr, g.ldq);
         return;
     }
     if (b <= tr.nprod) {
         __builtin_amdgcn_s_setprio(3);
         const int pw = 36 / tr.nprod;
-        if ((int)threadIdx.x < 64 * pw) diag_block_producer(g, (b - 1) * pw + (int)(threadIdx.x >> 6), ready, col0);
+        if ((int)threadIdx.x < 64 * pw) diag_block_producer<LAZY>(g, (b - 1) * pw + (int)(threadIdx.x >> 6), ready, col0);
         return;
     }
     const int first = 1 + tr.nprod;
@@ -660,7 +679,7 @@
     if (w < 0) {
         const int strip = b - first;
         __builtin_amdgcn_s_setprio(3);
-        gemm_tile_64_k128_grp<false>(g, lds, (long)(2 + strip) * SB, (long)grp * SB, gt, bar, nullptr, nullptr);
+        gemm_tile_64_k128_grp<false, LAZY>(g, lds, (long)(2 + strip) * SB, (long)grp * SB, gt, bar, nullptr, nullptr);
         asm volatile("s_waitcnt vmcnt(0)" ::: "memory");
         grp_barrier(bar);
         if (gt == 0) __hip_atomic_fetch_add(ctl + 4, 1u, __ATOMIC_RELAXED, __HIP_MEMORY_SCOPE_WORKGROUP);
@@ -671,7 +690,7 @@
         }
         __builtin_amdgcn_s_setprio(0);
     }
-    panel_tile_jobs(g, lds, gt, bar, tileq, ctl + 2 + grp, first_tile, (unsigned)(2 * nworkers));
+    panel_tile_jobs<LAZY>(g, lds, gt, bar, tileq, ctl + 2 + grp, first_tile, (unsigned)(2 * nworkers));
 }
 
 __global__ __launch_bounds__(256) void k_diag_inverse_batched(const double *K, long ld, const double *xm_all, double *Linv,
@@ -789,6 +808,8 @@
     hipError_t e = hipFuncSetAttribute((const void *)k_ldlt_diag128_v2, hipFuncAttributeMaxDynamicSharedMemorySize, DIAG2_LDS_BYTES);
     if (e == hipSuccess) e = hipFuncSetAttribute((const void *)k_ldlt_panel<true>, hipFuncAttributeMaxDynamicSharedMemorySize, DIAG2_LDS_BYTES);
     if (e == hipSuccess) e = hipFuncSetAttribute((const void *)k_ldlt_panel<false>, hipFuncAttributeMaxDynamicSharedMemorySize, DIAG2_LDS_BYTES);
+    if (e == hipSuccess) e = hipFuncSetAttribute((const void *)k_ldlt_panel<true, true>, hipFuncAttributeMaxDynamicSharedMemorySize, DIAG2_LDS_BYTES);
+    if (e == hipSuccess) e = hipFuncSetAttribute((const void *)k_ldlt_panel<false, true>, hipFuncAttributeMaxDynamicSharedMemorySize, DIAG2_LDS_BYTES);
     if (e == hipSuccess) e = hipFuncSetAttribute((const void *)k_diag_inverse_batched, hipFuncAttributeMaxDynamicSharedMemorySize, DIAG2_LDS_BYTES);
     if (e == hipSuccess) e = hipFuncSetAttribute((const void *)k_trsm_subst, hipFuncAttributeMaxDynamicSharedMemorySize, (int)(TRSM_LDS_DOUBLES * sizeof(double)));
     g_attr_err = e;
@@ -806,8 +827,12 @@
     return 0;
 }
 int cip_launch_panel(hipStream_t s, double *Kb, long ld, double *xm_out, double *dvec, double *dinv, int *info, int col0,
-                     PivotSigns sg, unsigned *ready, unsigned *stage, unsigned *tileq, const GemmArgs *g, int rows, double *W, long ldw) {
+                     PivotSigns sg, unsigned *ready, unsigned *stage, unsigned *tileq, const GemmArgs *g, int rows, double *W, long ldw,
+                     const double *Cin, long ldcin, const double *Cdiag) {
     if (cip_kernels_init()) return -3;
+    if (Cin && (!Cdiag || (ldcin & 1) || (((uintptr_t)Cin) & 15))) { cip_set_error("panel launch: the lazy operand must be 16-byte aligned"); return -1; }
+    GemmArgs gl = g ? *g : GemmArgs{};
+    gl.Qin = Cin; gl.ldq = ldcin; gl.Cdiag = Cdiag;
     TrsmStrips tr = {Kb + CIP_NB, ld, Kb, xm_out, dinv, W, ldw, rows / 64, PANEL_PRODUCER_CUS};
     const int Bn = cip_in_batch() ? cip_tl_bz.B : 1;
     const bool transposed = Bn > 1;
@@ -826,15 +851,17 @@
         if (workers < 0) workers = 0;
         tr.nprod = Bn > 1 ? PANEL_PRODUCER_CUS : PANEL_PRODUCERS;
         const long grid = 1 + tr.nprod + tr.strips + workers;
-        if (transposed) cip_launch(k_ldlt_panel<true>, dim3((unsigned)(grid * Bn)), dim3(64 * PANEL_WAVES), DIAG2_LDS_BYTES, s, Kb, ld, xm_out, dvec, dinv, info,
-                                   col0, sg, ready, stage, tileq, *g, tr, Bn, CipBatch{cip_tl_bz.stride, cip_tl_bz.mask});
-        else cip_launch_b(k_ldlt_panel<true>, dim3((unsigned)grid), dim3(64 * PANEL_WAVES), DIAG2_LDS_BYTES, s, Kb, ld, xm_out, dvec, dinv, info, col0, sg,
-                          ready, stage, tileq, *g, tr, 0);
+        auto kern = Cin ? k_ldlt_panel<true, true> : k_ldlt_panel<true, false>;
+        if (transposed) cip_launch(kern, dim3((unsigned)(grid * Bn)), dim3(64 * PANEL_WAVES), DIAG2_LDS_BYTES, s, Kb, ld, xm_out, dvec, dinv, info,
+                                   col0, sg, ready, stage, tileq, gl, tr, Bn, CipBatch{cip_tl_bz.stride, cip_tl_bz.mask});
+        else cip_launch_b(kern, dim3((unsigned)grid), dim3(64 * PANEL_WAVES), DIAG2_LDS_BYTES, s, Kb, ld, xm_out, dvec, dinv, info, col0, sg,
+                          ready, stage, tileq, gl, tr, 0);
     } else {
-        if (transposed) cip_launch(k_ldlt_panel<false>, dim3((unsigned)((1 + tr.strips) * Bn)), dim3(64 * PANEL_WAVES), DIAG2_LDS_BYTES, s, Kb, ld, xm_out, dvec,
-                                   dinv, info, col0, sg, ready, stage, tileq, GemmArgs{}, tr, Bn, CipBatch{cip_tl_bz.stride, cip_tl_bz.mask});
-        else cip_launch_b(k_ldlt_panel<false>, dim3((unsigned)(1 + tr.strips)), dim3(64 * PANEL_WAVES), DIAG2_LDS_BYTES, s, Kb, ld, xm_out, dvec, dinv,
-                          info, col0, sg, ready, stage, tileq, GemmArgs{}, tr, 0);
+        auto kern = Cin ? k_ldlt_panel<false, true> : k_ldlt_panel<false, false>;
+        if (transposed) cip_launch(kern, dim3((unsigned)((1 + tr.strips) * Bn)), dim3(64 * PANEL_WAVES), DIAG2_LDS_BYTES, s, Kb, ld, xm_out, dvec,
+                                   dinv, info, col0, sg, ready, stage, tileq, gl, tr, Bn, CipBatch{cip_tl_bz.stride, cip_tl_bz.mask});
+        else cip_launch_b(kern, dim3((unsigned)(1 + tr.strips)), dim3(64 * PANEL_WAVES), DIAG2_LDS_BYTES, s, Kb, ld, xm_out, dvec, dinv,
+                          info, col0, sg, ready, stage, tileq, gl, tr, 0);
     }
     CIP_HIP_CHECK(hipGetLastError());
     return 0;
diff --git a/conicip.jl_amd/csrc/ldlt.hip b/conicip.jl_amd/csrc/ldlt.hip
--- a/conicip.jl_amd/csrc/ldlt.hip
+++ b/conicip.jl_amd/csrc/ldlt.hip
@@ -145,6 +145,7 @@
 }
 
 int cip_ldlt_fused_for(int Npad) { return solve_fused_for(Npad, cip_solve_block(Npad)); }
+int cip_ldlt_info_words(int Npad) { return 16 + 3 * (Npad / CIP_NB); }
 static size_t ldlt_ws_layout(CipLayout L, int Npad, LdltWorkspace *ws, int fused) {
     const size_t nblk = Npad / CIP_NB;
     ws->Bs = cip_solve_block(Npad);
@@ -155,7 +156,7 @@
     ws->X = L.take<double>(blk); ws->XT = L.take<double>(blk);
     ws->Tt = L.take<double>(nbk * half * half + 32);
     ws->zbuf = L.take<double>(Npad); ws->dinv = L.take<double>(Npad); ws->dvec = L.take<double>(Npad); ws->tmp = L.take<double>(Npad);
-    ws->info = L.take<int>(16 + 3 * nblk);
+    ws->info = L.take<int>(cip_ldlt_info_words(Npad));
     ws->fused = (fused != 0 && nbk >= 2) ? 1 : 0;
     ws->MT = ws->fused ? L.take<double>(blk) : nullptr; ws->PT = ws->fused ? L.take<double>(blk) : nullptr;
     return L.bytes();
@@ -164,7 +165,7 @@
 void cip_ldlt_ws_carve(void *base, int Npad, LdltWorkspace *ws, int fused) {
     ldlt_ws_layout(base, Npad, ws, fused);
     ws->prof = nullptr;
-    ws->lazyC = nullptr; ws->lazy_ld = 0; ws->lazy_diag = nullptr;
+    ws->lazyC = nullptr; ws->lazy_ld = 0; ws->lazy_diag = nullptr; ws->info_zeroed = 0; ws->lazy_first = 0;
     ws->signs = PivotSigns{-1, 0, 0};
     ws->x_zeroed = nullptr;
     ws->side = nullptr;
@@ -177,7 +178,8 @@
 int cip_launch_diag_inverse(hipStream_t s, const double *K, long ld, int nblk, const double *xm_all, double *Linv,
                             double *LinvT, int Bs);
 int cip_launch_panel(hipStream_t s, double *Kb, long ld, double *xm_out, double *dvec, double *dinv, int *info, int col0,
-                     PivotSigns sg, unsigned *ready, unsigned *stage, unsigned *tileq, const GemmArgs *g, int rows, double *W, long ldw);
+                     PivotSigns sg, unsigned *ready, unsigned *stage, unsigned *tileq, const GemmArgs *g, int rows, double *W, long ldw,
+                     const double *Cin, long ldcin, const double *Cdiag);
 int cip_launch_trsm_subst(hipStream_t s, double *Ap, long ld, int rows, const double *L11, const double *xm,
                           const double *dinv, double *W, long ldw);
 
@@ -197,6 +199,22 @@
 int cip_ldlt_set_fused_chain(int on) { fuse_env(); const int prev = g_fuse_diag; if (on == 0 || on == 3) g_fuse_diag = on; return prev; }
 
 static thread_local bool tl_ran_fused = false;
+
+bool cip_ldlt_chain_fused(const LdltWorkspace &ws, int Npad) {
+    fuse_env();
+    static const int lsmax = cip_env_int("CIP_LOCKSTEP_PANEL_MAX", 32);
+    static const int lscus = [] {
+        if (cip_env_set("CIP_LOCKSTEP_PANEL_CUS")) return cip_env_int("CIP_LOCKSTEP_PANEL_CUS", 0);
+        int dev = 0, cus = 256;
+        if (hipGetDevice(&dev) == hipSuccess) (void)hipDeviceGetAttribute(&cus, hipDeviceAttributeMultiprocessorCount, dev);
+        return 4 * cus;
+    }();
+    const bool small_group = cip_in_batch() && cip_tl_bz.B <= lsmax && (long)cip_tl_bz.B * (10 + Npad / 64) <= lscus;
+    return g_fuse_diag && !ws.unfused && (!cip_in_batch() || small_group);
+}
+bool cip_ldlt_lazy_first_for(const LdltWorkspace &ws, int Npad) {
+    return cip_ldlt_chain_fused(ws, Npad) && outer_block_width(Npad, 0) >= 2 * CIP_NB && outer_block_width(Npad, 0) < Npad;
+}
 
 static int factor_outer_panels(hipStream_t s, double *K, int Npad, long ld, const LdltWorkspace &ws, double *Wb, int C0,
                                int wblk, int t0 = 0, int t1 = -1) {
@@ -207,28 +225,23 @@
         const int jb = c0 / CIP_NB;
         const int r = Npad - c0 - CIP_NB;
         GemmArgs gu;
-        fuse_env();
-        static const int lsmax = cip_env_int("CIP_LOCKSTEP_PANEL_MAX", 32);
-        static const int lscus = [] {
-            if (cip_env_set("CIP_LOCKSTEP_PANEL_CUS")) return cip_env_int("CIP_LOCKSTEP_PANEL_CUS", 0);
-            int dev = 0, cus = 256;
-            if (hipGetDevice(&dev) == hipSuccess) (void)hipDeviceGetAttribute(&cus, hipDeviceAttributeMultiprocessorCount, dev);
-            return 4 * cus;
-        }();
-        const bool small_group = cip_in_batch() && cip_tl_bz.B <= lsmax && (long)cip_tl_bz.B * (10 + Npad / 64) <= lscus;
-        const bool fuse = g_fuse_diag && !ws.unfused && (!cip_in_batch() || small_group);
+        const bool fuse = cip_ldlt_chain_fused(ws, Npad);
         if (fuse) {
             tl_ran_fused = true;
             RestOfBlock rb;
             const bool upd = t > 0 && rest_of_block(K, Npad, ld, Wb, C0, wblk, t - 1, rb);
             if (upd) gu = GemmArgs{rb.A, Npad, rb.B, ld, rb.C, ld, rb.M, rb.N, CIP_NB, -1.0};
+            const long lz = (ws.lazy_first && C0 == 0 && t <= 1) ? (long)c0 : -1L;
+            if (lz >= 0 && (!ws.lazyC || (t == 1 && !(upd && rb.C == K + c0 + (long)c0 * ld)))) { cip_set_error("ldlt: the first outer block is lazy without its source"); return -1; }
             unsigned *ctr = (unsigned *)(ws.info + 16);
             if ((rc = cip_launch_panel(s, K + c0 + (long)c0 * ld, ld, ws.Xm + (size_t)jb * 2048, ws.dvec + c0, ws.dinv + c0, ws.info, c0,
                                        ws.signs, ctr + jb, ctr + Npad / CIP_NB + jb, ctr + 2 * (Npad / CIP_NB) + jb, upd ? &gu : nullptr, r,
-                                       Wb + (c0 + CIP_NB) + (long)(t * CIP_NB) * Npad, Npad)))
+                                       Wb + (c0 + CIP_NB) + (long)(t * CIP_NB) * Npad, Npad,
+                                       lz >= 0 ? ws.lazyC + lz + lz * ws.lazy_ld : nullptr, ws.lazy_ld, lz >= 0 ? ws.lazy_diag + lz : nullptr)))
                 return rc;
             continue;
         }
+        if (ws.lazy_first) { cip_set_error("ldlt: only the fused panel chain reads an uncopied first outer block"); return -1; }
         if ((rc = cip_launch_diag_v2(s, K + c0 + (long)c0 * ld, ld, ws.Xm + (size_t)jb * 2048, ws.dvec + c0,
                                      ws.dinv + c0, ws.info, c0, ws.signs)))
             return rc;
@@ -469,7 +482,7 @@
 static int ldlt_factor_body(hipStream_t s, double *K, int Npad, long ld, const LdltWorkspace &ws) {
     if (Npad % CIP_NB) { cip_set_error("ldlt: N must be a multiple of 128"); return -1; }
     int rc;
-    if ((rc = zero_fill(s, ws.info, 64 + 12 * (size_t)(Npad / CIP_NB)))) return rc;
+    if (!ws.info_zeroed && (rc = zero_fill(s, ws.info, sizeof(int) * (size_t)cip_ldlt_info_words(Npad)))) return rc;
     if ((rc = ensure_x_zeroed(s, Npad, ws))) return rc;
     const int Bs = ws.Bs;
     LdltProfile *prof_this = ws.prof ? ws.prof : (cip_tl_builder ? nullptr : g_tl_prof);
diff --git a/conicip.jl_amd/csrc/sdp_large.hip b/conicip.jl_amd/csrc/sdp_large.hip
--- a/conicip.jl_amd/csrc/sdp_large.hip
+++ b/conicip.jl_amd/csrc/sdp_large.hip
@@ -1252,7 +1252,7 @@
     int *gate = (int *)(w->ctr + LG_C_GATE + side);
     hipLaunchKernelGGL(k_lg_cert_build, lg_grid(n2), dim3(256), 0, s, M3, rp, dscale, r, rp, want_max, cert, M2, M1);
     LdltWorkspace wc = wx;
-    wc.no_prep = 1; wc.lazyC = nullptr; wc.prof = nullptr;
+    wc.no_prep = 1; wc.lazyC = nullptr; wc.lazy_first = 0; wc.info_zeroed = 0; wc.prof = nullptr;
     if ((rc = cip_ldlt_factor(s, M2, rp, rp, wc))) return rc;
     hipLaunchKernelGGL(k_lg_cert_check, dim3(1), dim3(64), 0, s, (const int *)wc.info, gate, w->fallbacks());
     double *dg = w->dg(side), *of = w->of(side);
diff --git a/include/cipkkt.h b/include/cipkkt.h
--- a/include/cipkkt.h
+++ b/include/cipkkt.h
@@ -177,6 +177,7 @@
 int cip_get_chain_fallbacks(cip_handle *h);
 int cip_set_ldlt_side_prep(int on);
 int cip_set_lazy_copy(int on);
+int cip_set_lazy_first(int on);
 int cip_set_sdp_lanczos(int on);
 int cip_sdp_lanczos_fallbacks(cip_handle *h, int *count);
 int cip_profile_trailing(cip_handle *h, int enabled);
```
